# qiskit-community/aqc-research

Hardware: AMD Instinct MI355X
Metric: objective+gradient evals/sec (higher is better)
Workload: dtype f64; 1 GPU; 16-qubit, 40-block cx spin ansatz, state-vector objective+gradient; n_qubits=16, num_thetas=208, gate_groups=56, batch_per_gpu=1024, columns=1, transport=none, records_gathered=1024, launcher=none

## Files before the change

aqc_research_amd/csrc/aqc_api.cpp:

```cpp
#include "aqc_ws.h"

using namespace aqc;

namespace {
thread_local std::string g_error;
}

namespace aqc {

int fail(const char* fmt, ...) {
    char buf[1024];
    va_list ap;
    va_start(ap, fmt);
    vsnprintf(buf, sizeof buf, fmt, ap);
    va_end(ap);
    g_error = buf;
    return 1;
}
int set_error(const std::string& msg) { g_error = msg; return 1; }

int check_buf(const aqc_ws* ws, int buf) {
    if (!ws) return fail("null workspace");
    if (buf < 0 || buf >= AQC_NUM_BUFS) return fail("invalid buffer id %d", buf);
    return 0;
}

int check_block_range(const aqc_ws* ws, int block_from, int block_to) {
    const int nb = ws->ctx->prog.num_blocks;
    if (block_from < 0 || nb == 0) return 0;
    if (!(block_from < block_to && block_to <= nb)) return fail("invalid block_range [%d, %d)", block_from, block_to);
    return 0;
}

int ensure_coef(aqc_ws* ws) {
    if (ws->coef_valid) return 0;
    return fail("thetas have not been uploaded (aqc_ws_set_thetas)");
}

int copy_in(aqc_ws* ws, double2* dst, const double* src, size_t rows) {
    if (ws->pitch == ws->ncols) {
        HIP_OK(hipMemcpyAsync(dst, src, rows * ws->ncols * sizeof(double2), hipMemcpyHostToDevice, ws->stream));
    } else {
        HIP_OK(hipMemsetAsync(dst, 0, rows * ws->pitch * sizeof(double2), ws->stream));
        HIP_OK(hipMemcpy2DAsync(dst, (size_t)ws->pitch * sizeof(double2), src, (size_t)ws->ncols * sizeof(double2),
                                (size_t)ws->ncols * sizeof(double2), rows, hipMemcpyHostToDevice, ws->stream));
    }
    HIP_OK(hipStreamSynchronize(ws->stream));
    return 0;
}
int copy_out(aqc_ws* ws, double* dst, const double2* src, size_t rows) {
    if (ws->pitch == ws->ncols) {
        HIP_OK(hipMemcpyAsync(dst, src, rows * ws->ncols * sizeof(double2), hipMemcpyDeviceToHost, ws->stream));
    } else {
        HIP_OK(hipMemcpy2DAsync(dst, (size_t)ws->ncols * sizeof(double2), src, (size_t)ws->pitch * sizeof(double2),
                                (size_t)ws->ncols * sizeof(double2), rows, hipMemcpyDeviceToHost, ws->stream));
    }
    HIP_OK(hipStreamSynchronize(ws->stream));
    return 0;
}

int results_guard(aqc_ws* ws) {
    if (ws->copy_pending && !ws->capturing) {
        HIP_OK(hipStreamWaitEvent(ws->stream, ws->ev_copied, 0));
        ws->copy_pending = false;
    }
    return 0;
}


}

extern "C" {

const char* aqc_version(void) { return "aqc_hip 0.1.0 (gfx950)"; }
const char* aqc_last_error(void) { return g_error.c_str(); }

int aqc_live_buffers(int64_t* device, int64_t* pinned) {
    if (device) *device = g_live_device.load();
    if (pinned) *pinned = g_live_pinned.load();
    return 0;
}

int aqc_device_count(void) {
    int ndev = 0;
    return hipGetDeviceCount(&ndev) == hipSuccess ? ndev : 0;
}

int aqc_create(int num_qubits, int entangler, const int32_t* blocks, int num_blocks, int trotter, int second_order,
               aqc_ctx** out) {
    if (!out) return fail("out pointer is null");
    *out = nullptr;
    aqc_ctx* ctx = new aqc_ctx();
    const std::string err = build_program(num_qubits, entangler, blocks, num_blocks, trotter != 0, second_order != 0, ctx->prog);
    if (!err.empty()) {
        delete ctx;
        return fail("%s", err.c_str());
    }
    *out = ctx;
    return 0;
}

int aqc_destroy(aqc_ctx* ctx) {
    if (!ctx) return 0;
    for (auto& kv : ctx->oneshot) aqc_ws_destroy(kv.second);
    delete ctx;
    return 0;
}

int aqc_num_thetas(const aqc_ctx* ctx) { return ctx ? ctx->prog.num_thetas() : -1; }
int aqc_num_gate_groups(const aqc_ctx* ctx) { return ctx ? (int)ctx->prog.groups.size() : -1; }

int aqc_plan_query(aqc_ctx* ctx, int ncols, int which, int tile_bits, int low_bits, int stage, int* num_stages,
                   int* bits_out, int* num_bits, int* ops_out, int* num_ops) {
    if (!ctx) return fail("null context");
    if (ncols < 1) return fail("ncols must be positive");
    const int col_bits = ceil_log2(ncols);
    if (tile_bits <= 0) tile_bits = which == 1 ? 12 : 13;
    if (low_bits < 0) low_bits = 3;
    Plan plan = make_plan(ctx->prog, col_bits, tile_bits, low_bits, which == 0);
    if (which == 3) {
        split_substages(ctx->prog, plan, 4, 1 << 20);
        plan = mirror_plan(plan);
    }
    const std::string err = check_plan(ctx->prog, plan);
    if (!err.empty()) return fail("planner produced an invalid plan: %s", err.c_str());
    if (num_stages) *num_stages = (int)plan.stages.size();
    if (stage >= 0) {
        if (stage >= (int)plan.stages.size()) return fail("stage index out of range");
        const Stage& st = plan.stages[stage];
        if (num_bits) *num_bits = (int)st.bits.size();
        if (num_ops) *num_ops = (int)st.ops.size();
        if (bits_out) for (size_t i = 0; i < st.bits.size(); ++i) bits_out[i] = st.bits[i];
        if (ops_out) for (size_t i = 0; i < st.ops.size(); ++i) ops_out[i] = st.ops[i];
    }
    return 0;
}

int aqc_plan_projected(aqc_ctx* ctx, int tile_bits, int low_bits, int32_t* info) {
    if (!ctx || !info) return fail("null argument");
    if (tile_bits <= 0) tile_bits = 12;
    if (low_bits < 0) low_bits = 3;
    const Program& prog = ctx->prog;
    tile_bits = std::min(std::max(tile_bits, 8), std::min(12, prog.n));
    aqc_ws tmp;
    tmp.ctx = ctx;
    tmp.ncols = 1; tmp.col_bits = 0; tmp.nbits = prog.n;
    Plan best = make_plan(prog, 0, tile_bits, low_bits, false);
    for (int lb = low_bits - 1; lb >= 2; --lb) {
        Plan cand = make_plan(prog, 0, tile_bits, lb, false);
        if (cand.stages.size() < best.stages.size()) best = cand;
    }
    lower_plan(prog, best, tmp.sweep, 4, true, true);
    tmp.sparse_enabled = true;
    tmp.inv_mirrored = tmp.sweep.v3 && tmp.sweep.plan.stages.size() >= 2;
    proj_plan(&tmp, low_bits);
    const int rc = aqc_ws_projected_info(&tmp, info);
    tmp.ctx = nullptr;
    return rc;
}

int aqc_plan_substages(aqc_ctx* ctx, int ncols, int which, int tile_bits, int low_bits, int stage, int* num_subs, int* subs_out, int max_subs) {
    if (!ctx || !num_subs) return fail("null argument");
    if (ncols < 1) return fail("ncols must be positive");
    const int col_bits = ceil_log2(ncols);
    if (tile_bits <= 0) tile_bits = 12;
    if (low_bits < 0) low_bits = 3;
    Plan plan = make_plan(ctx->prog, col_bits, tile_bits, low_bits, which == 0);
    split_substages(ctx->prog, plan, 4, 1 << 20);
    if (which == 3) plan = mirror_plan(plan);
    const std::string err = check_plan(ctx->prog, plan);
    if (!err.empty()) return fail("planner produced an invalid plan: %s", err.c_str());
    if (stage < 0 || stage >= (int)plan.stages.size()) return fail("stage index out of range");
    const Stage& st = plan.stages[stage];
    *num_subs = (int)st.subs.size();
    if (subs_out)
        for (int i = 0; i < (int)st.subs.size() && i < max_subs; ++i) {
            for (int j = 0; j < 4; ++j) subs_out[5 * i + j] = j < (int)st.subs[i].bits.size() ? st.subs[i].bits[j] : -1;
            subs_out[5 * i + 4] = (int)st.subs[i].ops.size();
        }
    return 0;
}


static int ws_decide(aqc_ws* ws, int tile_bits_apply, int tile_bits_sweep) {
    aqc_ctx* ctx = ws->ctx;
    const Program& prog = ctx->prog;
    const int batch = ws->batch;
    const int low_bits = env_int("AQC_LOW_BITS", 3);
    int ka = tile_bits_apply > 0 ? tile_bits_apply : env_int("AQC_TILE_BITS_APPLY", 0);
    int ks = tile_bits_sweep > 0 ? tile_bits_sweep : env_int("AQC_TILE_BITS_SWEEP", 0);
    const int family = env_int("AQC_KERNEL_FAMILY", env_int("AQC_KERNEL_V2", -1) >= 0 ? env_int("AQC_KERNEL_V2", -1) + 1 : 0);
    if (family < 0 || family > 3) return fail("AQC_KERNEL_FAMILY must be 1 (per-group), 2 (register-blocked) or 3 (matrix cores)");
    const bool want_v3 = (family == 3 || family == 0) && ws->nbits >= 8;
    const int force_v2 = family == 3 ? 0 : (family ? family - 1 : -1);
    const size_t big_tiles = (size_t)batch << std::max(0, ws->nbits - 12);
    const bool want_v2 = force_v2 >= 0 ? force_v2 != 0 : big_tiles >= 512;
    auto pick = [&](int kmax) {
        if (want_v3) {
            int k = std::min(12, ws->nbits);
            while (k > 10 && ((size_t)batch << (ws->nbits - k)) < 256) --k;
            const int kmin = std::max(8, prog.n + std::min(ws->col_bits, 3));
            while (ws->col_bits > 0 && k > kmin && ((size_t)batch << (ws->nbits - k)) < 256) --k;
            return k;
        }
        if (want_v2) return std::min(kmax, ws->nbits);
        int k = std::min(11, ws->nbits);
        while (k > 10 && ((size_t)batch << (ws->nbits - k)) < 512) --k;
        return k;
    };
    if (ka <= 0) ka = pick(13);
    if (ks <= 0) ks = pick(12);
    ka = std::min(std::min(ka, 13), ws->nbits);
    ks = std::min(std::min(ks, 12), ws->nbits);
    ws->threads = env_int("AQC_THREADS", 0);
    if (ws->threads <= 0) ws->threads = std::min(256, std::max(64, 1 << (std::min(ka, ks) - 2)));
    if (ws->threads < 64 || ws->threads > 512 || ws->threads % 64) return fail("AQC_THREADS must be a multiple of 64 in [64, 512]");

    auto best_plan = [&](int k, bool inverse) {
        Plan best = make_plan(prog, ws->col_bits, k, low_bits, inverse);
        for (int lb = low_bits - 1; lb >= 2; --lb) {
            Plan cand = make_plan(prog, ws->col_bits, k, lb, inverse);
            if (cand.stages.size() < best.stages.size()) best = cand;
        }
        return best;
    };
    if (want_v3) { ka = std::min(std::max(ka, 8), 12); ks = std::max(ks, 8); }
    auto cached = [&](const std::vector<int>& key, DevPlan& out, const std::function<void(HostPlan&)>& lower) {
        std::lock_guard<std::recursive_mutex> lock(ctx->mu);
        auto it = ctx->plan_cache.find(key);
        if (it == ctx->plan_cache.end()) {
            HostPlan fresh;
            lower(fresh);
            it = ctx->plan_cache.emplace(key, std::move(fresh)).first;
        }
        out = it->second;
    };
    auto cached_plan = [&](int which, int k, bool inverse, int reg_bits, bool dots, DevPlan& out) {
        cached({which, ws->col_bits, k, low_bits, reg_bits, (int)dots, (int)want_v3}, out,
               [&](HostPlan& fresh) { lower_plan(prog, best_plan(k, inverse), fresh, reg_bits, dots, want_v3); });
    };
    cached_plan(2, ka, false, (want_v2 || want_v3) ? 4 : 0, false, ws->fwd);
    cached_plan(1, ks, false, want_v3 ? 4 : (want_v2 ? (env_int("AQC_SWEEP_REG_BITS", 4) == 3 ? 3 : 4) : 0), true, ws->sweep);
    ws->inv_mirrored = want_v3 && ka == ks && ws->sweep.v3 && ws->sweep.plan.stages.size() >= 2 && env_int("AQC_MIRROR_PLAN", 1) != 0;
    if (ws->inv_mirrored)
        cached({3, ws->col_bits, ks, low_bits, 4, 0, 1}, ws->inv,
               [&](HostPlan& fresh) { lower_plan(prog, mirror_plan(ws->sweep.plan), fresh, 4, false, true, true); });
    else
        cached_plan(0, ka, true, (want_v2 || want_v3) ? 4 : 0, false, ws->inv);
    ws->sparse_enabled = env_int("AQC_SPARSE_SWEEP", 1) != 0;
    ws->sparse_min_items = env_int("AQC_SPARSE_MIN_ITEMS", 512);
    ws->lazy_z_enabled = env_int("AQC_LAZY_Z", 1) != 0;
    ws->r_only_enabled = env_int("AQC_R_ONLY_LAST", 1) != 0;
    ws->r_only_max_subs = env_int("AQC_R_ONLY_MAX_SUBS", 12);
    ws->proj_vdag_enabled = env_int("AQC_PROJECTED_VDAG", 1) != 0;
    ws->proj_fused_enabled = env_int("AQC_PROJECTED_FUSED", 1) != 0;
    ws->proj_pairs_enabled = env_int("AQC_PROJECTED_PAIRS", 1) != 0;
    ws->proj_vdag_min_elems = (long long)env_int("AQC_PROJECTED_VDAG_MIN_ELEMS", 1 << 24);
    ws->skipw_enabled = env_int("AQC_SKIP_ZERO_W", 0) != 0;
    for (DevPlan* p : {&ws->fwd, &ws->inv, &ws->sweep}) {
        const std::string err = check_plan(prog, p->plan);
        if (!err.empty()) return fail("planner produced an invalid plan: %s", err.c_str());
    }
    proj_plan(ws, low_bits);
    if (env_int("AQC_VERBOSE", 0) && want_v3)
        fprintf(stderr, "aqc_hip: matrix-core kernels, tiles 2^%d (V / V^H, %d workgroups per CU) / 2^%d (sweep, %d per CU), sub-stages %zu / %zu / %zu\n",
                ws->inv.k, mfma_occupancy(ws->inv.k, false), ws->sweep.k, mfma_occupancy(ws->sweep.k, true), ws->fwd.h_subs3.size(),
                ws->inv.h_subs3.size(), ws->sweep.h_subs3.size());
    return 0;
}

struct SlotTables {
    std::vector<int> theta_slots, slot_theta, slot_ntiles;
    int partial_tiles = 1;
};
static SlotTables ws_slot_tables(aqc_ws* ws) {
    const Program& prog = ws->ctx->prog;
    const int T = prog.num_thetas();
    const int G = (int)prog.groups.size();
    ws->nslots = G * kSlotsPerGroup;
    SlotTables t;
    t.partial_tiles = ws->sweep.v3 ? 1 : ws->sweep.ntiles;
    t.theta_slots.assign(2 * (size_t)std::max(T, 1), -1);
    t.slot_ntiles.assign((size_t)std::max(ws->nslots, 1), t.partial_tiles);
    auto feed = [&](int theta, int slot) {
        if (t.theta_slots[2 * theta] < 0) t.theta_slots[2 * theta] = slot; else t.theta_slots[2 * theta + 1] = slot;
    };
    for (int gi = 0; gi < G; ++gi) {
        const GateGroup& g = prog.groups[gi];
        if (g.type == GROUP_FRONT) {
            feed(g.theta0 + 2, gi * kSlotsPerGroup + 0);
            feed(g.theta0 + 1, gi * kSlotsPerGroup + 1);
            feed(g.theta0 + 0, gi * kSlotsPerGroup + 2);
        } else {
            for (int d = 0; d < prog.tpb; ++d) feed(g.theta0 + d, gi * kSlotsPerGroup + d);
        }
    }
    t.slot_theta.assign((size_t)std::max(ws->nslots, 1), -1);
    ws->grads_direct = ws->sweep.v3 && T > 0 && env_int("AQC_GRADS_DIRECT", 1) != 0;
    for (int th = 0; th < T; ++th) {
        if (t.theta_slots[2 * th] < 0 || t.theta_slots[2 * th + 1] >= 0) { ws->grads_direct = false; break; }
        t.slot_theta[t.theta_slots[2 * th]] = th;
    }
    return t;
}

static int ws_upload_ujobs(aqc_ws* ws) {
    const Program& prog = ws->ctx->prog;
    std::vector<UJob> jobs, route_jobs;
    size_t n_vdag_sweep = 0;
    DevPlan* vsw = ws->proj.ok ? &ws->proj.vsw : nullptr;
    const int nsw = ws->sweep.v3 ? (int)ws->sweep.h_subs3.size() : 0;
    ws->ujobs_mirror = ws->inv_mirrored && ws->inv.v3 && (int)ws->inv.h_subs3.size() == nsw && env_int("AQC_UBUILD_MIRROR", 1) != 0;
    for (DevPlan* p : {&ws->inv, &ws->sweep, vsw, &ws->fwd})
        if (p && p->v3)
            for (size_t i = 0; i < p->h_subs3.size(); ++i) {
                if (p == &ws->inv && ws->ujobs_mirror) continue;
                UJob j{p->d_subs3 + i, p->d_grps, p->d_umat, (int)i, (int)p->h_subs3.size(), p->plan.inverse ? 1 : 0, prog.entangler, nullptr, 0, 0};
                if (p == &ws->sweep && ws->ujobs_mirror) { j.umat_mirror = ws->inv.d_umat; j.mirror_index = nsw - 1 - (int)i; j.mirror_nsubs = nsw; }
                if (p == vsw) {
                    const int nvs = (int)vsw->h_subs3.size();
                    j.umat_mirror = ws->proj.vinv.d_umat; j.mirror_index = nvs - 1 - (int)i; j.mirror_nsubs = nvs;
                }
                jobs.push_back(j);
                if (p != &ws->fwd) ++n_vdag_sweep;
                if (vsw && ((p == &ws->inv && (int)i >= p->h_stages.back().sub_begin) || (p == &ws->sweep && (int)i < p->h_stages[0].nsubs) || p == vsw))
                    route_jobs.push_back(j);
            }
    if (vsw && !route_jobs.empty() && route_jobs.size() < n_vdag_sweep && env_int("AQC_UBUILD_SUBSET", 1) != 0) {
        if (ws->d_ujobs_route.upload(route_jobs)) return 1;
        ws->n_ujobs_route = (int)route_jobs.size();
    }
    if (!jobs.empty() && ws->d_ujobs.upload(jobs)) return 1;
    return 0;
}

static int ws_device_side(aqc_ws* ws, const SlotTables& t) {
    const Program& prog = ws->ctx->prog;
    const size_t B = (size_t)ws->batch, T1 = (size_t)std::max(prog.num_thetas(), 1), lanes = B * ws->lane_elems;
    HIP_OK(hipStreamCreateWithFlags(&ws->stream, hipStreamNonBlocking));
    HIP_OK(hipEventCreate(&ws->ev0)); HIP_OK(hipEventCreate(&ws->ev1));
    HIP_OK(hipEventCreate(&ws->pev0)); HIP_OK(hipEventCreate(&ws->pev1));
    if (upload_plan(ws->fwd) || upload_plan(ws->inv) || upload_plan(ws->sweep) || proj_alloc(ws)) return 1;
    if (ws->d_thetas_own.alloc(B * T1)) return 1;
    ws->d_thetas = ws->d_thetas_own;
    if (ws->d_coef.alloc(B * (prog.n + prog.num_blocks + 1) * kCoefStride)) return 1;
    for (auto& buf : ws->bufs) {
        if (buf.alloc(lanes)) return 1;
        HIP_OK(hipMemsetAsync(buf, 0, sizeof(double2) * lanes, ws->stream));
    }
    if (ws->d_partial.alloc(B * std::max(ws->nslots, 1) * t.partial_tiles)) return 1;
    for (DevPlan* p : {&ws->fwd, &ws->inv, &ws->sweep})
        if (p->v3 && p->d_umat.alloc(B * std::max<size_t>(p->h_subs3.size(), 1) * 12 * 64)) return 1;
    if (ws_upload_ujobs(ws)) return 1;
    if (ws->sweep.v3 && ws->sweep.d_rpart.alloc(B * std::max<size_t>(ws->sweep.h_subs3.size(), 1) *
                                                sweep3_nparts(ws->sweep.ntiles, ws->batch, ws->sweep.k) * 256)) return 1;
    if (ws->d_grads.alloc(B * T1)) return 1;
    if (ws->d_theta_slots.upload(t.theta_slots) || ws->d_slot_ntiles.upload(t.slot_ntiles) || ws->d_slot_theta.upload(t.slot_theta)) return 1;
    ws->pin_thetas = B * T1;
    ws->pin_grads = 2 * B * T1;
    ws->pin_small = 2 * B * 64;
    if (ws->h_pin.alloc(ws->pin_thetas + ws->pin_grads + ws->pin_small)) return 1;
    ws->vdot_parts = (int)std::min<size_t>(1024, std::max<size_t>(1, ws->lane_elems / 1024));
    if (ws->d_vdot_part.alloc(B * ws->vdot_parts)) return 1;
    HIP_OK(hipStreamSynchronize(ws->stream));
    return 0;
}

int aqc_ws_create(aqc_ctx* ctx, int device, int batch, int ncols, int tile_bits_apply, int tile_bits_sweep, aqc_ws** out) {
    if (!out) return fail("out pointer is null");
    *out = nullptr;
    if (!ctx) return fail("null context");
    if (batch < 1 || batch > 65535) return fail("batch must be in [1, 65535] (lanes are the y dimension of the launch grid)");
    if (ncols < 1) return fail("ncols must be >= 1");
    const Program& prog = ctx->prog;
    int ndev = 0;
    hipError_t e = hipGetDeviceCount(&ndev);
    if (e != hipSuccess || ndev <= 0)
        return fail("no HIP device available (%s): the aqc_hip path needs an AMD GPU and has no CPU fallback",
                    e == hipSuccess ? "device count is 0" : hipGetErrorString(e));
    if (device < 0 || device >= ndev) return fail("device %d out of range (%d visible)", device, ndev);
    HIP_OK(hipSetDevice(device));
    HIP_OK(init_kernels());
    HIP_OK(init_kernels2());
    HIP_OK(init_kernels3());

    struct Destroy { void operator()(aqc_ws* w) const { aqc_ws_destroy(w); } };
    std::unique_ptr<aqc_ws, Destroy> ws(new aqc_ws());
    ws->ctx = ctx;
    ws->device = device;
    ws->batch = batch;
    ws->ncols = ncols;
    ws->col_bits = ceil_log2(ncols);
    ws->pitch = 1 << ws->col_bits;
    ws->nbits = ws->col_bits + prog.n;
    if (ws->nbits > kMaxBits) return fail("2^%d elements per lane is beyond this build's limit", ws->nbits);
    ws->lane_elems = (size_t)1 << ws->nbits;
    if (ws_decide(ws.get(), tile_bits_apply, tile_bits_sweep)) return 1;
    if (ws_device_side(ws.get(), ws_slot_tables(ws.get()))) return 1;
    *out = ws.release();
    return 0;
}

int aqc_ws_destroy(aqc_ws* ws) {
    if (!ws) return 0;
    (void)hipSetDevice(ws->device);
    for (hipStream_t s : {ws->stream, ws->copy_stream, ws->mps_stream}) if (s) (void)hipStreamSynchronize(s);
    drop_graphs(ws);
    for (hipEvent_t ev : {ws->ev0, ws->ev1, ws->pev0, ws->pev1, ws->ev_ready, ws->ev_copied, ws->ev_mps_fork, ws->ev_mps_join})
        if (ev) (void)hipEventDestroy(ev);
    for (hipStream_t s : {ws->copy_stream, ws->mps_stream, ws->stream}) if (s) (void)hipStreamDestroy(s);
    delete ws;
    return 0;
}

int aqc_ws_set_thetas(aqc_ws* ws, const double* thetas) {
    if (!ws || !thetas) return fail("null argument");
    HIP_OK(hipSetDevice(ws->device));
    const Program& prog = ws->ctx->prog;
    const int T = prog.num_thetas();
    HIP_OK(hipMemcpyAsync(ws->d_thetas_own, thetas, sizeof(double) * (size_t)ws->batch * T, hipMemcpyHostToDevice, ws->stream));
    HIP_OK(hipStreamSynchronize(ws->stream));
    return run_coef(ws, ws->d_thetas_own);
}

int aqc_ws_upload(aqc_ws* ws, int buf, const double* src) {
    if (check_buf(ws, buf) || before_write(ws, buf)) return 1;
    if (!src) return fail("null source");
    HIP_OK(hipSetDevice(ws->device));
    return copy_in(ws, ws->bufs[buf], src, (size_t)ws->batch << ws->ctx->prog.n);
}

int aqc_ws_upload_lane(aqc_ws* ws, int buf, int lane, const double* src) {
    if (check_buf(ws, buf)) return 1;
    if (!src) return fail("null source");
    if (lane < 0 || lane >= ws->batch) return fail("lane out of range");
    HIP_OK(hipSetDevice(ws->device));
    if (before_write(ws, buf, true)) return 1;
    return copy_in(ws, ws->bufs[buf] + (size_t)lane * ws->lane_elems, src, (size_t)1 << ws->ctx->prog.n);
}

int aqc_ws_broadcast(aqc_ws* ws, int buf, const double* src) {
    if (check_buf(ws, buf) || before_write(ws, buf)) return 1;
    if (!src) return fail("null source");
    HIP_OK(hipSetDevice(ws->device));
    if (copy_in(ws, ws->bufs[buf], src, (size_t)1 << ws->ctx->prog.n)) return 1;
    for (int b = 1; b < ws->batch; ++b)
        HIP_OK(hipMemcpyAsync(ws->bufs[buf] + (size_t)b * ws->lane_elems, ws->bufs[buf], ws->lane_elems * sizeof(double2),
                              hipMemcpyDeviceToDevice, ws->stream));
    return 0;
}

int aqc_ws_copy_lane(aqc_ws* dst_ws, int dst_buf, int dst_lane, aqc_ws* src_ws, int src_buf, int src_lane) {
    if (check_buf(dst_ws, dst_buf) || check_buf(src_ws, src_buf)) return 1;
    if (dst_ws->device != src_ws->device) return fail("copy_lane: the two workspaces live on different devices");
    if (dst_ws->lane_elems != src_ws->lane_elems) return fail("copy_lane: lane sizes differ");
    if (dst_lane < 0 || dst_lane >= dst_ws->batch || src_lane < 0 || src_lane >= src_ws->batch) return fail("lane out of range");
    if (before_read(src_ws, src_buf) || before_write(dst_ws, dst_buf, true)) return 1;
    HIP_OK(hipSetDevice(dst_ws->device));
    if (src_ws->stream != dst_ws->stream) HIP_OK(hipStreamSynchronize(src_ws->stream));
    HIP_OK(hipMemcpyAsync(dst_ws->bufs[dst_buf] + (size_t)dst_lane * dst_ws->lane_elems, src_ws->bufs[src_buf] + (size_t)src_lane * src_ws->lane_elems,
                          sizeof(double2) * dst_ws->lane_elems, hipMemcpyDeviceToDevice, dst_ws->stream));
    return 0;
}

int aqc_ws_download(aqc_ws* ws, int buf, double* dst) {
    if (check_buf(ws, buf)) return 1;
    if (!dst) return fail("null destination");
    HIP_OK(hipSetDevice(ws->device));
    if (before_read(ws, buf)) return 1;
    return copy_out(ws, dst, ws->bufs[buf], (size_t)ws->batch << ws->ctx->prog.n);
}

int aqc_ws_download_lane(aqc_ws* ws, int buf, int lane, double* dst) {
    if (check_buf(ws, buf)) return 1;
    if (!dst) return fail("null destination");
    if (lane < 0 || lane >= ws->batch) return fail("lane out of range");
    HIP_OK(hipSetDevice(ws->device));
    if (before_read(ws, buf)) return 1;
    return copy_out(ws, dst, ws->bufs[buf] + (size_t)lane * ws->lane_elems, (size_t)1 << ws->ctx->prog.n);
}

int aqc_ws_set_basis(aqc_ws* ws, int buf, const int64_t* index) {
    if (check_buf(ws, buf) || before_write(ws, buf)) return 1;
    if (!index) return fail("null index");
    HIP_OK(hipSetDevice(ws->device));
    const int64_t dim = (int64_t)1 << ws->ctx->prog.n;
    std::vector<long long> elem(ws->batch);
    for (int b = 0; b < ws->batch; ++b) {
        if (index[b] < 0 || index[b] >= dim) return fail("basis index out of range");
        elem[b] = (long long)index[b] << ws->col_bits;
    }
    if (ws->d_basis_index.reserve(ws->batch)) return 1;
    HIP_OK(hipMemcpyAsync(ws->d_basis_index, elem.data(), sizeof(long long) * ws->batch, hipMemcpyHostToDevice, ws->stream));
    HIP_OK(hipStreamSynchronize(ws->stream));
    HIP_OK(hipMemsetAsync(ws->bufs[buf], 0, sizeof(double2) * (size_t)ws->batch * ws->lane_elems, ws->stream));
    {
        ProfScope ps(ws, AQC_K_MISC);
        HIP_OK(launch_scatter_one(ws->bufs[buf], ws->lane_elems, ws->batch, ws->d_basis_index, ws->stream));
    }
    std::vector<long long> supp(2 * (size_t)ws->batch, -1);
    for (int b = 0; b < ws->batch; ++b) supp[2 * (size_t)b] = elem[b];
    if (ws->d_combo_prev[buf].reserve(2 * (size_t)ws->batch)) return 1;
    HIP_OK(hipMemcpyAsync(ws->d_combo_prev[buf], supp.data(), sizeof(long long) * supp.size(), hipMemcpyHostToDevice, ws->stream));
    HIP_OK(hipStreamSynchronize(ws->stream));
    std::vector<double> coef(4 * (size_t)ws->batch, 0.0);
    for (int b = 0; b < ws->batch; ++b) coef[4 * (size_t)b] = 1.0;
    lhs_support_changed(ws, buf, std::move(supp), std::move(coef));
    return 0;
}

int aqc_ws_set_identity(aqc_ws* ws, int buf) {
    if (check_buf(ws, buf) || before_write(ws, buf)) return 1;
    const int dim = 1 << ws->ctx->prog.n;
    if (ws->ncols != dim) return fail("identity needs a square workspace (ncols == 2^n)");
    HIP_OK(hipSetDevice(ws->device));
    HIP_OK(hipMemsetAsync(ws->bufs[buf], 0, sizeof(double2) * (size_t)ws->batch * ws->lane_elems, ws->stream));
    ProfScope ps(ws, AQC_K_MISC);
    HIP_OK(launch_set_identity(ws->bufs[buf], ws->lane_elems, dim, ws->pitch, ws->batch, ws->stream));
    return 0;
}

int aqc_ws_set_combo(aqc_ws* ws, int buf, const int64_t* index, const double* coef) {
    if (check_buf(ws, buf)) return 1;
    if (!index || !coef) return fail("null argument");
    if (buf == AQC_BUF_W || buf == AQC_BUF_ZW || buf == AQC_BUF_Z) return fail("set_combo targets an lhs buffer (X, X2) or Y");
    HIP_OK(hipSetDevice(ws->device));
    const int64_t dim = (int64_t)1 << ws->ctx->prog.n;
    const int B = ws->batch;
    std::vector<long long> elem(2 * (size_t)B);
    for (int b = 0; b < B; ++b) {
        const int64_t i0 = index[2 * b], i1 = index[2 * b + 1];
        if (i0 < 0 || i0 >= dim || i1 >= dim) return fail("basis index out of range");
        if (i1 == i0) return fail("the two basis states of a lane must differ");
        elem[2 * b] = (long long)i0 << ws->col_bits;
        elem[2 * b + 1] = i1 < 0 ? -1 : (long long)i1 << ws->col_bits;
    }
    std::vector<double> cf(coef, coef + 4 * (size_t)B);
    if (ws->combo_valid[buf] && ws->combo_last_elem[buf] == elem && ws->combo_last_coef[buf] == cf) return 0;
    if (ws->d_combo_index.reserve(2 * (size_t)B) || ws->d_combo_coef.reserve(2 * (size_t)B)) return 1;
    if (ws->d_combo_prev[buf].reserve(2 * (size_t)B)) return 1;
    HIP_OK(hipMemcpyAsync(ws->d_combo_index, elem.data(), sizeof(long long) * 2 * B, hipMemcpyHostToDevice, ws->stream));
    HIP_OK(hipMemcpyAsync(ws->d_combo_coef, coef, sizeof(double2) * 2 * B, hipMemcpyHostToDevice, ws->stream));
    HIP_OK(hipStreamSynchronize(ws->stream));
    if (!ws->combo_valid[buf]) {
        HIP_OK(hipMemsetAsync(ws->bufs[buf], 0, sizeof(double2) * (size_t)B * ws->lane_elems, ws->stream));
        HIP_OK(hipMemsetAsync(ws->d_combo_prev[buf], 0xff, sizeof(long long) * 2 * B, ws->stream));
    }
    ProfScope ps(ws, AQC_K_MISC);
    HIP_OK(launch_scatter_two(ws->bufs[buf], ws->lane_elems, B, ws->d_combo_index, ws->d_combo_coef, ws->d_combo_prev[buf], ws->stream));
    lhs_support_changed(ws, buf, std::move(elem), std::move(cf));
    return 0;
}

int aqc_ws_get_grads(aqc_ws* ws, double* grads) {
    if (!ws || !grads) return fail("null argument");
    HIP_OK(hipSetDevice(ws->device));
    HIP_OK(hipMemcpyAsync(grads, ws->d_grads, sizeof(double2) * (size_t)ws->batch * ws->ctx->prog.num_thetas(),
                          hipMemcpyDeviceToHost, ws->stream));
    HIP_OK(hipStreamSynchronize(ws->stream));
    return 0;
}

int aqc_ws_gather(aqc_ws* ws, int buf, const int64_t* index, int count, double* out) {
    if (check_buf(ws, buf)) return 1;
    if (!index || !out || count < 1) return fail("invalid gather arguments");
    HIP_OK(hipSetDevice(ws->device));
    if (before_read(ws, buf)) return 1;
    const int64_t dim = (int64_t)1 << ws->ctx->prog.n;
    std::vector<long long> elem(count);
    for (int i = 0; i < count; ++i) {
        if (index[i] < 0 || index[i] >= dim) return fail("gather index out of range");
        elem[i] = (long long)index[i] << ws->col_bits;
    }
    HIP_OK(hipStreamSynchronize(ws->stream));
    if (ws->d_tmp_index.reserve(count) || ws->d_tmp_small.reserve((size_t)ws->batch * count)) return 1;
    HIP_OK(hipMemcpyAsync(ws->d_tmp_index, elem.data(), sizeof(long long) * count, hipMemcpyHostToDevice, ws->stream));
    HIP_OK(hipStreamSynchronize(ws->stream));
    {
        ProfScope ps(ws, AQC_K_MISC);
        HIP_OK(launch_gather(ws->bufs[buf], ws->lane_elems, ws->d_tmp_index, count, ws->batch, ws->d_tmp_small, ws->stream));
    }
    HIP_OK(hipMemcpyAsync(out, ws->d_tmp_small, sizeof(double2) * (size_t)ws->batch * count, hipMemcpyDeviceToHost, ws->stream));
    HIP_OK(hipStreamSynchronize(ws->stream));
    return 0;
}

int aqc_ws_vdot(aqc_ws* ws, int buf_a, int buf_b, double* out) {
    if (check_buf(ws, buf_a) || check_buf(ws, buf_b)) return 1;
    if (!out) return fail("null output");
    HIP_OK(hipSetDevice(ws->device));
    if (before_read(ws, buf_a) || before_read(ws, buf_b)) return 1;
    HIP_OK(hipStreamSynchronize(ws->stream));
    if (ws->d_tmp_small.reserve(ws->batch)) return 1;
    {
        ProfScope ps(ws, AQC_K_MISC);
        HIP_OK(launch_vdot(ws->bufs[buf_a], ws->bufs[buf_b], ws->lane_elems, ws->lane_elems, ws->batch, ws->d_vdot_part,
                           ws->vdot_parts, ws->d_tmp_small, ws->stream));
    }
    HIP_OK(hipMemcpyAsync(out, ws->d_tmp_small, sizeof(double2) * (size_t)ws->batch, hipMemcpyDeviceToHost, ws->stream));
    HIP_OK(hipStreamSynchronize(ws->stream));
    return 0;
}

int aqc_ws_theta_bank(aqc_ws* ws, const double* thetas, int nsets) {
    if (!ws || !thetas || nsets < 1) return fail("invalid theta bank arguments");
    HIP_OK(hipSetDevice(ws->device));
    const size_t count = (size_t)nsets * ws->batch * std::max(ws->ctx->prog.num_thetas(), 1), bytes = sizeof(double) * count;
    HIP_OK(hipStreamSynchronize(ws->stream));
    if (ws->d_theta_bank.release()) return 1;
    ws->bank_sets = 0;
    ws->d_thetas = ws->d_thetas_own;
    if (ws->d_theta_bank.alloc(count)) return 1;
    HIP_OK(hipMemcpyAsync(ws->d_theta_bank, thetas, bytes, hipMemcpyHostToDevice, ws->stream));
    HIP_OK(hipStreamSynchronize(ws->stream));
    ws->bank_sets = nsets;
    return 0;
}

int aqc_ws_use_theta_set(aqc_ws* ws, int set_index) {
    if (!ws) return fail("null workspace");
    if (set_index < 0 || set_index >= ws->bank_sets) return fail("theta set %d out of range (%d loaded)", set_index, ws->bank_sets);
    HIP_OK(hipSetDevice(ws->device));
    return run_coef(ws, ws->d_theta_bank + (size_t)set_index * ws->batch * ws->ctx->prog.num_thetas());
}

int aqc_ws_gather_setup(aqc_ws* ws, const int64_t* index, int count) {
    if (!ws || !index || count < 1) return fail("invalid gather arguments");
    HIP_OK(hipSetDevice(ws->device));
    const int64_t dim = (int64_t)1 << ws->ctx->prog.n;
    std::vector<long long> elem(count);
    for (int i = 0; i < count; ++i) {
        if (index[i] < 0 || index[i] >= dim) return fail("gather index out of range");
        elem[i] = (long long)index[i] << ws->col_bits;
    }
    HIP_OK(hipStreamSynchronize(ws->stream));
    drop_graphs(ws);
    if (ws->d_index.reserve(count) || ws->d_small.reserve((size_t)ws->batch * count)) return 1;
    if (2 * (size_t)ws->batch * count > ws->pin_small) {
        const size_t want = 2 * (size_t)ws->batch * count;
        PinBuf<double> pin;
        if (pin.alloc(ws->pin_thetas + ws->pin_grads + want)) return 1;
        ws->h_pin = std::move(pin);
        ws->pin_small = want;
    }
    HIP_OK(hipMemcpyAsync(ws->d_index, elem.data(), sizeof(long long) * count, hipMemcpyHostToDevice, ws->stream));
    HIP_OK(hipStreamSynchronize(ws->stream));
    ws->gather_count = count;
    ws->h_gather = elem;
    ++ws->gather_gen;
    return 0;
}

int aqc_ws_gather_launch(aqc_ws* ws, int buf) {
    if (check_buf(ws, buf)) return 1;
    if (ws->gather_count < 1) return fail("aqc_ws_gather_setup has not been called");
// ... 265 lines not shown
```

aqc_research_amd/csrc/aqc_kernels3.hip:

```cpp
#include <hip/hip_runtime.h>

#include <cstring>

#include <type_traits>

#include "aqc_device.h"
#include "aqc_launch.h"
#include "aqc_math.h"

namespace aqc {

typedef double double4_t __attribute__((ext_vector_type(4)));

__host__ __device__ __forceinline__ unsigned swz3(unsigned l) { return l ^ ((l >> 4) & 15u) ^ ((l >> 8) & 15u); }

__device__ __forceinline__ double4_t mfma(double a, double b, double4_t c) {
    return __builtin_amdgcn_mfma_f64_16x16x4f64(a, b, c, 0, 0, 0);
}

struct Acc3 { double4_t k1, k2, k3; };
__device__ __forceinline__ void u_mfma(const cplx (&v)[4], const double (&u0)[4], const double (&u1)[4], const double (&u2)[4], Acc3& t) {
    t.k1 = double4_t{0.0, 0.0, 0.0, 0.0}; t.k2 = t.k1; t.k3 = t.k1;
#pragma unroll
    for (int s = 0; s < 4; ++s) {
        t.k1 = mfma(v[s].x + v[s].y, u0[s], t.k1);
        t.k2 = mfma(v[s].x, u1[s], t.k2);
        t.k3 = mfma(v[s].y, u2[s], t.k3);
    }
}
__device__ __forceinline__ void u_combine(const Acc3& t, cplx (&o)[4]) {
#pragma unroll
    for (int r = 0; r < 4; ++r) {
        o[r].x = t.k1[r] - t.k3[r];
        o[r].y = t.k1[r] + t.k2[r];
    }
}

#ifdef AQC_TUNING
#define AQC_STAMP(slot) do { if (a.stamps && threadIdx.x == 0 && (slot) < kStampSlots) \
    a.stamps[((size_t)blockIdx.y * gridDim.x + blockIdx.x) * kStampSlots + (slot)] = __builtin_amdgcn_s_memtime(); } while (0)
#ifdef AQC_TUNING_NODBG
#define AQC_DBG_AND(x)
#define AQC_DBG_TEST(x) false
#else
#define AQC_DBG_AND(x) && (x)
#define AQC_DBG_TEST(x) (x)
#endif
#else
#define AQC_STAMP(slot) do { } while (0)
#define AQC_DBG_AND(x)
#define AQC_DBG_TEST(x) false
#endif

__host__ __device__ constexpr bool sweep_scratch_double(int k) { return k >= 12 || k <= 9; }
#ifndef AQC_SWEEP_SPREAD
#define AQC_SWEEP_SPREAD 1
#endif
#ifndef AQC_APPLY_SPREAD
#define AQC_APPLY_SPREAD 1
#endif
#ifndef AQC_EXP_APPLY_SKIP
#define AQC_EXP_APPLY_SKIP 0
#endif
constexpr int kApplySkip = AQC_EXP_APPLY_SKIP;
#ifndef AQC_EXP_SWEEP_SKIP
#define AQC_EXP_SWEEP_SKIP 0
#endif
constexpr int kSweepSkip = AQC_EXP_SWEEP_SKIP;
#ifndef AQC_EXP_UBUILD_SKIP
#define AQC_EXP_UBUILD_SKIP 0
#endif
constexpr int kUbuildSkip = AQC_EXP_UBUILD_SKIP;

constexpr int kSweepSpread = AQC_SWEEP_SPREAD, kApplySpread = AQC_APPLY_SPREAD;
template <int K, bool SWEEP = false> struct TileShape {
    static constexpr int kSweepWaves12 = 4;
    static constexpr int kWaves = (SWEEP && K == 12) ? kSweepWaves12 : (K >= 10 ? 4 : (1 << (K - 8)));
    static constexpr int kGroups = 1 << (K - 8);
    static constexpr int kGpw = kGroups / kWaves;
    static constexpr int kLoads = (1 << (K - 6)) / kWaves;
};

struct SubRegs {
    double u0[4], u1[4], u2[4];
    unsigned lane12;
};

template <int GPW>
__device__ __forceinline__ void fetch_sub(SubRegs& x, const DevSub3* subs, const double* umat, int sub_index, int lane, int wave,
                                          int nwaves) {
    const DevSub3* sub = subs + sub_index;
    const double* up = umat + (size_t)sub_index * 12 * 64;
#pragma unroll
    for (int s = 0; s < 4; ++s) {
        x.u0[s] = up[(0 * 4 + s) * 64 + lane];
        x.u1[s] = up[(1 * 4 + s) * 64 + lane];
        x.u2[s] = up[(2 * 4 + s) * 64 + lane];
    }
    x.lane12 = sub->lane12[lane];
}

template <int GPW>
struct SubAddr {
    unsigned a1, a2;
    unsigned k1[GPW][4], k2[GPW][4];
};
typedef unsigned uint8v_t __attribute__((ext_vector_type(8)));
template <int GPW>
__device__ __forceinline__ void fetch_k(SubAddr<GPW>& x, const DevSub3* subs, int sub_index, int wave, int nwaves) {
#pragma unroll
    for (int j = 0; j < GPW; ++j) {
        const uint8v_t kv = *reinterpret_cast<const __attribute__((address_space(4))) uint8v_t*>(
            (const __attribute__((address_space(4))) void*)(const void*)&subs[sub_index].kk[wave + j * nwaves][0]);
#pragma unroll
        for (int s = 0; s < 4; ++s) { x.k1[j][s] = kv[s]; x.k2[j][s] = kv[4 + s]; }
    }
}
template <int GPW>
__device__ __forceinline__ void sub_addr(SubAddr<GPW>& x, const SubRegs& c, unsigned lds_base) {
    x.a1 = ((c.lane12 & 0xffffu) << 4) + lds_base;
    x.a2 = ((c.lane12 >> 16) << 4) + lds_base;
}
typedef double dbl2_t __attribute__((ext_vector_type(2)));
typedef __attribute__((address_space(3))) dbl2_t* lds_cplx_ptr;
__device__ __forceinline__ cplx lds_get(unsigned addr) {
    const dbl2_t v = *reinterpret_cast<lds_cplx_ptr>(addr);
    return make_double2(v.x, v.y);
}
__device__ __forceinline__ void lds_put(unsigned addr, cplx v) { *reinterpret_cast<lds_cplx_ptr>(addr) = dbl2_t{v.x, v.y}; }
__device__ __forceinline__ unsigned lds_address(const void* p) {
    return (unsigned)reinterpret_cast<size_t>((__attribute__((address_space(3))) const char*)p);
}

__device__ __forceinline__ const void* uniform_ptr(const void* p) {
    const unsigned long long v = (unsigned long long)p;
    const unsigned lo = __builtin_amdgcn_readfirstlane((unsigned)v), hi = __builtin_amdgcn_readfirstlane((unsigned)(v >> 32));
    return (const void*)(((unsigned long long)hi << 32) | lo);
}

template <int K, int NV>
__device__ __forceinline__ void load_tiles3(cplx* t0, cplx* t1, const cplx* s0, const cplx* s1, const DevStage& st, unsigned lo, int wave) {
    constexpr int NL = TileShape<K, NV == 2>::kLoads, NW = TileShape<K, NV == 2>::kWaves;
    cplx v0[NL], v1[NL];
#pragma unroll
    for (int i = 0; i < NL; ++i) {
        const unsigned off = lo + st.dhi[wave + i * NW];
        v0[i] = s0[off];
        if (NV == 2) v1[i] = s1[off];
    }
#pragma unroll
    for (int i = 0; i < NL; ++i) {
        const unsigned slot = swz3((unsigned)((wave + i * NW) << 6) | (threadIdx.x & 63u));
        t0[slot] = v0[i];
        if (NV == 2) t1[slot] = v1[i];
    }
}
template <int K, bool SWEEP>
__device__ __forceinline__ void store_tile3(const cplx* tile, cplx* dst, const DevStage& st, unsigned lo, int wave) {
    constexpr int NL = TileShape<K, SWEEP>::kLoads, NW = TileShape<K, SWEEP>::kWaves;
#pragma unroll
    for (int i = 0; i < NL; ++i) {
        const unsigned slot = swz3((unsigned)((wave + i * NW) << 6) | (threadIdx.x & 63u));
        dst[lo + st.dhi[wave + i * NW]] = tile[slot];
    }
}
__device__ __forceinline__ size_t tile_base3(const DevStage& st, unsigned tile) {
    size_t base = 0;
    for (int i0 = 0; i0 < st.nub; i0 += 4) {
        int ub[4];
#pragma unroll
        for (int u = 0; u < 4; ++u) ub[u] = st.ubits[i0 + u];
#pragma unroll
        for (int u = 0; u < 4; ++u)
            if (i0 + u < st.nub) base |= (size_t)((tile >> (i0 + u)) & 1u) << ub[u];
    }
    return base;
}

__device__ __forceinline__ int uniform_load(const int* p) { return __builtin_amdgcn_readfirstlane(*p); }
struct ItemAt { int bl, tile, slot; };
template <bool LIST>
__device__ __forceinline__ ItemAt item_at(const Stage3Args& a, int wi) {
    if (LIST) {
        const TileItem* it = a.items + wi;
        return ItemAt{uniform_load(&it->lane), uniform_load(&it->tile), uniform_load(&it->slot)};
    }
    const int bl = wi / a.ntiles;
    return ItemAt{bl, wi - bl * a.ntiles, 0};
}
template <int K, bool LIST, bool PAIR = false>
__device__ __forceinline__ void apply_mfma_body(const Stage3Args& a0, const Stage3Args& b0, const int wg, const int nwg) {
    using TS = TileShape<K>;
    static_assert(!PAIR || (LIST && K >= 12), "the pair form walks two lists with persistent workgroups");
    extern __shared__ __attribute__((aligned(16))) char smem[];
    const Stage3Args* ca = &a0;
#define a (*ca)
#define st (ca->stage)
    cplx* tw = reinterpret_cast<cplx*>(smem);
    const unsigned lds_base = lds_address(smem);
    if (lds_base & ((16u << K) - 1)) __builtin_trap();
    const int lane = threadIdx.x & 63;
    const int wave = __builtin_amdgcn_readfirstlane((int)(threadIdx.x >> 6));
    constexpr int NL = TS::kLoads, NW = TS::kWaves;
    constexpr bool kPersist = K >= 12;
    int nwork = LIST ? uniform_load(a.nitems) : a.ntiles * a.batch;
    bool second = false;
    if (PAIR && wg >= nwork) { ca = &b0; second = true; nwork = uniform_load(b0.nitems); }
    unsigned lo = st.dlo[lane];
    unsigned lo16 = lo << 4;
    (void)lo16;
    SubRegs cur, nxt;
    SubAddr<TS::kGpw> ad;
    dbl2_t pw[NL];
    int wi = wg + ((kPersist || LIST) ? 0 : (int)blockIdx.y * a.ntiles);
    if (LIST && wi >= nwork) return;
    ItemAt it = item_at<LIST>(a, wi);
    {
        const int bl = it.bl;
        if (st.nsubs > 0) {
            fetch_sub<TS::kGpw>(cur, a.subs, a.umat + (size_t)bl * a.nsubs_total * 12 * 64, st.sub_begin, lane, wave, NW);
            fetch_k<TS::kGpw>(ad, a.subs, st.sub_begin, wave, NW);
        }
        AQC_STAMP(0);
        if (!(kApplySkip & 64)) load_tiles3<K, 1>(tw, nullptr, a.in0 + (size_t)bl * a.lane_stride + tile_base3(st, it.tile), nullptr, st, lo, wave);
    }
    __builtin_amdgcn_s_waitcnt(0x0F70);
    AQC_STAMP(1);
    for (;;) {
    const int bl = it.bl;
    const size_t lane_off = (size_t)bl * a.lane_stride + tile_base3(st, it.tile);
    const double* umat = a.umat + (size_t)bl * a.nsubs_total * 12 * 64;
    int nwi = wi + nwg;
    bool more = kPersist && st.nsubs > 0 && nwi < nwork;
    const Stage3Args* na = ca;
    int nnwork = nwork;
    if (PAIR && !more && !second) {
        na = &b0; nwi = wg; nnwork = uniform_load(b0.nitems);
        more = nwi < nnwork;
    }
    const bool change = PAIR && na != ca;
    const ItemAt nit = more ? item_at<LIST>(*na, nwi) : ItemAt{0, 0, 0};
    const int nbl = nit.bl;
    const size_t next_off = more ? (size_t)nbl * na->lane_stride + tile_base3(na->stage, nit.tile) : 0;
    const unsigned nlo = change ? na->stage.dlo[lane] : lo;
    const unsigned nlo16 = nlo << 4;
    for (int si = 0; si < st.nsubs; ++si) {
        AQC_STAMP(4 + si);
        if (!(kApplySkip & 512)) __syncthreads();
        if (si + 1 < st.nsubs) fetch_sub<TS::kGpw>(nxt, a.subs, umat, st.sub_begin + si + 1, lane, wave, NW);
        else if (more) fetch_sub<TS::kGpw>(nxt, na->subs, na->umat + (size_t)nbl * na->nsubs_total * 12 * 64, na->stage.sub_begin, lane, wave, NW);
        if (kPersist && more && !(kApplySkip & 64)) {
#pragma unroll
            for (int c = 0; c < 4; ++c) {
                if (si == (c < st.nsubs ? c : st.nsubs - 1)) {
#pragma unroll
                    for (int i = c * (NL / 4); i < (c + 1) * (NL / 4); ++i) {
                        const size_t ub = next_off + na->stage.dhi[wave + i * NW];
                        asm volatile("s_nop 4\n\tglobal_load_dwordx4 %0, %1, %2" : "=a"(pw[i]) : "v"(nlo16), "s"(uniform_ptr(na->in0 + ub)) : "memory");
                    }
                }
            }
        }
        sub_addr(ad, cur, lds_base);
        cplx v[2][4];
        Acc3 acc;
#pragma unroll
        for (int s = 0; s < 4; ++s) v[0][s] = lds_get(ad.a1 ^ ad.k1[0][s]);
#pragma unroll
        for (int j = 0; j <= TS::kGpw; ++j) {
            if (j + 1 < TS::kGpw && !(kApplySkip & 2)) {
#pragma unroll
                for (int s = 0; s < 4; ++s) v[(j + 1) & 1][s] = lds_get((kApplySkip & 32) ? ad.a1 : (ad.a1 ^ ad.k1[j + 1][s]));
            }
            __builtin_amdgcn_sched_barrier(0);
            double sv[4];
            cplx o[4];
            if (j < TS::kGpw) {
#pragma unroll
                for (int s = 0; s < 4; ++s) sv[s] = (kApplySkip & (16 | 128)) ? v[j & 1][s].x : v[j & 1][s].x + v[j & 1][s].y;
            }
            if (j > 0) {
                if (kApplySkip & (16 | 256)) {
#pragma unroll
                    for (int r = 0; r < 4; ++r) o[r] = make_double2(acc.k1[r], acc.k2[r]);
                } else u_combine(acc, o);
            }
            unsigned wa[4];
            if (j < TS::kGpw) {
#pragma unroll
                for (int s = 0; s < 4; ++s) asm volatile("" : "+v"(sv[s]));
            }
            if (j > 0) {
#pragma unroll
                for (int r = 0; r < 4; ++r) { wa[r] = (kApplySkip & 32) ? ad.a2 : (ad.a2 ^ ad.k2[j - 1][r]); asm volatile("" : "+v"(wa[r])); }
            }
            __builtin_amdgcn_sched_barrier(0);
            if (j < TS::kGpw) {
                acc.k1 = double4_t{0.0, 0.0, 0.0, 0.0}; acc.k2 = acc.k1; acc.k3 = acc.k1;
#pragma unroll
                for (int s = 0; s < 4; ++s) {
                    if (kApplySkip & 8) continue;
                    acc.k1 = mfma(sv[s], cur.u0[s], acc.k1);
                    acc.k2 = mfma(v[j & 1][s].x, cur.u1[s], acc.k2);
                    acc.k3 = mfma(v[j & 1][s].y, cur.u2[s], acc.k3);
                }
            }
            if (j > 0 && !(kApplySkip & 1)) {
#pragma unroll
                for (int r = 0; r < 4; ++r) lds_put(wa[r], o[r]);
                if (j < TS::kGpw) {
#pragma unroll
                    for (int i = 0; i < 4; ++i) {
                        __builtin_amdgcn_sched_group_barrier(0x008, kApplySpread, 0);
                        __builtin_amdgcn_sched_group_barrier(0x200, 1, 0);
                    }
                }
            }
            __builtin_amdgcn_sched_barrier(0);
        }
        if (si + 1 < st.nsubs || more) {
            cur = nxt;
            if (si + 1 < st.nsubs) fetch_k<TS::kGpw>(ad, a.subs, st.sub_begin + si + 1, wave, NW);
            else fetch_k<TS::kGpw>(ad, na->subs, na->stage.sub_begin, wave, NW);
        }
    }
    AQC_STAMP(4 + st.nsubs);
    __syncthreads();
    AQC_STAMP(2);
    if (!(kApplySkip & 64)) store_tile3<K, false>(tw, a.out0 + lane_off, st, lo, wave);
    AQC_STAMP(3);
    if (!more) break;
    __syncthreads();
    __builtin_amdgcn_s_waitcnt(0x0F70);
#pragma unroll
    for (int i = 0; i < NL; ++i) {
        const unsigned slot = swz3((unsigned)((wave + i * NW) << 6) | (threadIdx.x & 63u));
        asm volatile("ds_write_b128 %0, %1" : : "v"(lds_base + (slot << 4)), "a"(pw[i]) : "memory");
    }
    __builtin_amdgcn_s_waitcnt(0xC07F);
    wi = nwi;
    it = nit;
    if (PAIR) { ca = na; second = second || change; nwork = nnwork; lo = nlo; lo16 = nlo16; }
    }
#undef a
#undef st
}
template <int K, bool LIST = false>
__global__ __launch_bounds__(TileShape<K>::kWaves * 64, 2) void apply_mfma_kernel(const Stage3Args a) {
    apply_mfma_body<K, LIST>(a, a, (int)blockIdx.x, (int)gridDim.x);
}
#ifndef AQC_PAIR_PLAIN_BOUNDARY
#define AQC_PAIR_PLAIN_BOUNDARY 0
#endif
template <int K>
__global__ __launch_bounds__(TileShape<K>::kWaves * 64, 2) void apply_pair_kernel(const Stage3Args a, const Stage3Args b, const int grid_a) {
    if constexpr (K >= 12 && !AQC_PAIR_PLAIN_BOUNDARY) {
        static_assert(sizeof(Stage3Args) % 8 == 0 && alignof(Stage3Args) == 8, "b follows a in the kernel-argument segment without padding");
        const __attribute__((address_space(4))) char* kp = (const __attribute__((address_space(4))) char*)__builtin_amdgcn_kernarg_segment_ptr();
        const Stage3Args* pa = (const Stage3Args*)(const void*)kp;
        const Stage3Args* pb = (const Stage3Args*)(const void*)(kp + sizeof(Stage3Args));
        apply_mfma_body<K, true, true>(*pa, *pb, (int)blockIdx.x, (int)gridDim.x);
    } else if (K >= 12) {
        apply_mfma_body<K, true>(a, a, (int)blockIdx.x, (int)gridDim.x);
        __syncthreads();
        apply_mfma_body<K, true>(b, b, (int)blockIdx.x, (int)gridDim.x);
    } else if ((int)blockIdx.x < grid_a) {
        apply_mfma_body<K, true>(a, a, (int)blockIdx.x, grid_a);
    } else {
        apply_mfma_body<K, true>(b, b, (int)blockIdx.x - grid_a, (int)gridDim.x - grid_a);
    }
}

template <int N>
__device__ __forceinline__ void wait_prefetched(dbl2_t (&pw)[N], dbl2_t (&pz)[N]) {
    asm volatile("s_waitcnt vmcnt(0)" : : : "memory");
#pragma unroll
    for (int i = 0; i < N; ++i) asm volatile("" : "+a"(pw[i]), "+a"(pz[i]));
}
__device__ __forceinline__ unsigned tile_offset3(const DevStage& st, unsigned local) { return st.dlo[local & 63u] | st.dhi[local >> 6]; }
template <int K> struct SweepShape : TileShape<K, true> {};
__device__ __forceinline__ unsigned elem_bit(const DevStage& st, long long e, unsigned local_pos) {
    const unsigned m = local_pos < 6 ? st.dlo[1u << local_pos] : st.dhi[1u << (local_pos - 6)];
    return ((unsigned long long)e & m) ? 1u : 0u;
}
template <int GPW, int NW>
__device__ __forceinline__ void skip_masks(const DevStage& st, unsigned info, long long e0, long long e1, int wave, unsigned& nzmask, unsigned& kneed) {
    nzmask = 0; kneed = 0;
    const unsigned gfresh = info & 15u, kfresh = (info >> 6) & 3u;
#pragma unroll
    for (int k = 0; k < 2; ++k) {
        const long long e = k ? e1 : e0;
        if (e < 0) continue;
        unsigned gb = 0;
#pragma unroll
        for (int i = 0; i < 4; ++i)
            if (gfresh >> i & 1) gb |= elem_bit(st, e, (info >> (8 + 4 * i)) & 15u) << i;
        unsigned kb = 0;
        if (kfresh & 1) kb |= elem_bit(st, e, (info >> 24) & 15u);
        if (kfresh & 2) kb |= elem_bit(st, e, (info >> 28) & 15u) << 1;
#pragma unroll
        for (int j = 0; j < GPW; ++j)
            if ((((unsigned)(wave + j * NW) ^ gb) & gfresh) == 0) nzmask |= 1u << j;
#pragma unroll
        for (unsigned s2 = 0; s2 < 4; ++s2)
            if (((s2 ^ kb) & kfresh) == 0) kneed |= 1u << s2;
    }
}
template <int K, bool LIST, bool SKIPW, bool RLAST>
__device__ __forceinline__ void sweep_mfma_body(const Stage3Args& a, const int wg, const int nwg) {
    using TS = TileShape<K, true>;
    constexpr int kSlots = TS::kWaves > 4 ? 4 : TS::kWaves;
    constexpr unsigned tsize = 1u << K;
    extern __shared__ __attribute__((aligned(16))) char smem[];
    const DevStage& st = a.stage;
    cplx* tw = reinterpret_cast<cplx*>(smem);
    cplx* tz = tw + tsize;
    cplx* scratch = tz + tsize;
    constexpr bool kDouble = sweep_scratch_double(K);
    const unsigned lds_base = lds_address(smem);
    if (lds_base & ((32u << K) - 1)) __builtin_trap();
    const int lane = threadIdx.x & 63;
    const int wave = __builtin_amdgcn_readfirstlane((int)(threadIdx.x >> 6));
    constexpr bool kPersist = K >= 12;
    constexpr int NL = TS::kLoads, NW = TS::kWaves;
    const int nwork = LIST ? uniform_load(a.nitems) : a.ntiles * a.batch;
    const unsigned lo = st.dlo[lane];
    SubRegs cur, nxt;
    SubAddr<TS::kGpw> ad;
    dbl2_t pw[NL], pz[NL];
    unsigned parity = 0;
    AQC_STAMP(0);
    const int chunk = kPersist ? (LIST ? (nwork + nwg - 1) / nwg : a.chunk) : 0;
    const int wi_first = kPersist ? wg * chunk : wg;
    const int wi_end = kPersist ? (wi_first + chunk < nwork ? wi_first + chunk : nwork) : wi_first + 1;
    int wi = wi_first;
    if (wi >= nwork) return;
    const unsigned e16 = threadIdx.x << 4;
    dbl2_t racc;
    static_assert(!kPersist || NL == 4 * TS::kGpw, "the prefetch registers are the first sub-stage's operands");
    const bool reg_first = kPersist && st.nsubs > 0;
    unsigned flo16 = 0;
    ItemAt it = item_at<LIST>(a, wi);
    size_t item_off = (size_t)it.bl * a.lane_stride + tile_base3(st, it.tile);
    {
        const size_t off0 = item_off;
        if (st.nsubs > 0) {
            fetch_sub<TS::kGpw>(cur, a.subs, a.umat + (size_t)it.bl * a.nsubs_total * 12 * 64, st.sub_begin, lane, wave, NW);
            fetch_k<TS::kGpw>(ad, a.subs, st.sub_begin, wave, NW);
        }
        if (reg_first) {
            flo16 = tile_offset3(st, swz3(cur.lane12 & 0xffffu)) << 4;
#pragma unroll
            for (int i = 0; i < ((kSweepSkip & 64) ? 0 : NL); ++i) {
                const size_t ub = off0 + a.first_hi[wave + (i / 4) * NW][i % 4];
                asm volatile("s_nop 4\n\tglobal_load_dwordx4 %0, %1, %2" : "=a"(pw[i]) : "v"(flo16), "s"(uniform_ptr(a.in0 + ub)) : "memory");
                asm volatile("s_nop 4\n\tglobal_load_dwordx4 %0, %1, %2" : "=a"(pz[i]) : "v"(flo16), "s"(uniform_ptr(a.in1 + ub)) : "memory");
            }
        } else {
            load_tiles3<K, 2>(tw, tz, a.in0 + off0, a.in1 + off0, st, lo, wave);
        }
    }
    __builtin_amdgcn_s_waitcnt(0x0F70);
    if (reg_first) wait_prefetched<NL>(pw, pz);
    __syncthreads();
    AQC_STAMP(1);
    for (;;) {
    const int bl = it.bl, tile = it.tile;
    const size_t lane_off = item_off;
    long long se0 = -1, se1 = -1;
    if (SKIPW) {
        const unsigned long long toff = (unsigned long long)tile_base3(st, tile);
        const long long c0 = a.supp[2 * (size_t)bl], c1 = a.supp[2 * (size_t)bl + 1];
        const unsigned lo0 = __builtin_amdgcn_readfirstlane((unsigned)c0), hi0 = __builtin_amdgcn_readfirstlane((unsigned)(c0 >> 32));
        const unsigned lo1 = __builtin_amdgcn_readfirstlane((unsigned)c1), hi1 = __builtin_amdgcn_readfirstlane((unsigned)(c1 >> 32));
        const long long u0 = (long long)(((unsigned long long)hi0 << 32) | lo0), u1 = (long long)(((unsigned long long)hi1 << 32) | lo1);
        if (u0 >= 0 && (((unsigned long long)u0 ^ toff) & st.fresh_nonlocal) == 0) se0 = u0;
        if (u1 >= 0 && (((unsigned long long)u1 ^ toff) & st.fresh_nonlocal) == 0) se1 = u1;
    }
    const double* umat = a.umat + (size_t)bl * a.nsubs_total * 12 * 64;
    const int part = LIST ? it.slot : (kPersist ? wg - (bl * a.ntiles) / chunk : tile);
    const bool seg_first = LIST || !kPersist || wi == wi_first || tile == 0;
    cplx* rpart = a.rpart + (((size_t)bl * a.nsubs_total + st.sub_begin) * a.nparts + part) * 256;
    const int nwi = wi + 1;
    const bool more = reg_first && nwi < wi_end;
    const ItemAt nit = more ? item_at<LIST>(a, nwi) : ItemAt{0, 0, 0};
    const int nbl = nit.bl;
    const size_t next_off = more ? (size_t)nbl * a.lane_stride + tile_base3(st, nit.tile) : 0;
    constexpr unsigned ZOFF = tsize * 16;
    cplx vw[2][4], vz[2][4];
    constexpr bool kEarly = K >= 11;
    if (reg_first) {
        sub_addr(ad, cur, lds_base);
#pragma unroll
        for (int s = 0; s < 4; ++s) { vw[0][s] = make_double2(pw[s].x, pw[s].y); vz[0][s] = make_double2(pz[s].x, pz[s].y); }
    } else if (kEarly && st.nsubs > 0) {
        sub_addr(ad, cur, lds_base);
#pragma unroll
        for (int s = 0; s < 4; ++s) { vw[0][s] = lds_get(ad.a1 ^ ad.k1[0][s]); vz[0][s] = lds_get((ad.a1 | ZOFF) ^ ad.k1[0][s]); }
    }
    auto prefetch = [&](int c) __attribute__((always_inline)) {
#pragma unroll
        for (int i = 0; i < ((kSweepSkip & 64) ? 0 : NL); ++i)
            if (i / (NL / 4) == c) {
                const size_t ub = next_off + a.first_hi[wave + (i / 4) * NW][i % 4];
                asm volatile("s_nop 4\n\tglobal_load_dwordx4 %0, %1, %2" : "=a"(pw[i]) : "v"(flo16), "s"(uniform_ptr(a.in0 + ub)) : "memory");
                asm volatile("s_nop 4\n\tglobal_load_dwordx4 %0, %1, %2" : "=a"(pz[i]) : "v"(flo16), "s"(uniform_ptr(a.in1 + ub)) : "memory");
            }
    };
    const int nmain = RLAST && a.r_only_last && st.nsubs >= 1 && !(kPersist && st.nsubs == 1) ? st.nsubs - 1 : st.nsubs;
    if (!RLAST) {
        for (int si = 0; si < st.nsubs; ++si) {
#define AQC_SS_FROM_REGS (reg_first && si == 0)
#define AQC_SS_RONLY false
#include "aqc_sweep_substage.inc"
#undef AQC_SS_FROM_REGS
#undef AQC_SS_RONLY
        }
    } else {
        if (nmain > 0) {
            const int si = 0;
#define AQC_SS_FROM_REGS reg_first
#define AQC_SS_RONLY false
#include "aqc_sweep_substage.inc"
#undef AQC_SS_FROM_REGS
#undef AQC_SS_RONLY
        }
        for (int si = 1; si < nmain; ++si) {
#define AQC_SS_FROM_REGS false
#define AQC_SS_RONLY false
#include "aqc_sweep_substage.inc"
#undef AQC_SS_FROM_REGS
#undef AQC_SS_RONLY
        }
        if (nmain < st.nsubs) {
            const int si = nmain;
#define AQC_SS_FROM_REGS false
#define AQC_SS_RONLY true
#include "aqc_sweep_substage.inc"
#undef AQC_SS_FROM_REGS
#undef AQC_SS_RONLY
        }
    }
    AQC_STAMP(kStampSlots - 2);
    if (more) wait_prefetched<NL>(pw, pz);
    if (!(kSweepSkip & 64)) {
        if (a.store_out & 1) store_tile3<K, true>(tw, a.out0 + lane_off, st, lo, wave);
        if (a.store_out & 2) store_tile3<K, true>(tz, a.out1 + lane_off, st, lo, wave);
    }
    AQC_STAMP(kStampSlots - 1);
    if (!more) break;
    AQC_STAMP(kStampSlots - 6);
    __syncthreads();
    AQC_STAMP(kStampSlots - 5);
    wi = nwi;
    it = nit;
    item_off = next_off;
    }
    AQC_STAMP(kStampSlots - 4);
}
template <int K, bool LIST = false, bool SKIPW = false, bool RLAST = false>
__global__ __launch_bounds__(SweepShape<K>::kWaves * 64, K >= 12 ? 1 : 2) void sweep_mfma_kernel(const Stage3Args a) {
    sweep_mfma_body<K, LIST, SKIPW, RLAST>(a, (int)blockIdx.x, (int)gridDim.x);
}
template <int K, bool RLAST_A, bool RLAST_B>
__global__ __launch_bounds__(SweepShape<K>::kWaves * 64, K >= 12 ? 1 : 2) void sweep_pair_kernel(const Stage3Args a, const Stage3Args b, const int grid_a) {
    if (K >= 12) {
        sweep_mfma_body<K, true, false, RLAST_A>(a, (int)blockIdx.x, (int)gridDim.x);
        __syncthreads();
        sweep_mfma_body<K, true, false, RLAST_B>(b, (int)blockIdx.x, (int)gridDim.x);
    } else if ((int)blockIdx.x < grid_a) {
        sweep_mfma_body<K, true, false, RLAST_A>(a, (int)blockIdx.x, grid_a);
    } else {
        sweep_mfma_body<K, true, false, RLAST_B>(b, (int)blockIdx.x - grid_a, (int)gridDim.x - grid_a);
    }
}

constexpr int kGrpChunk = 16;
struct Gm {
    cplx c[4], t[4];
    double ec, es;
    double rc[4], rs[4];
    int type, pc, pt, flags, slot0, jblock, o0, o1;
};
__device__ __forceinline__ void m2_mul(const cplx (&a)[4], const cplx (&b)[4], cplx (&o)[4]) {
#pragma unroll
    for (int i = 0; i < 2; ++i)
#pragma unroll
        for (int j = 0; j < 2; ++j) {
            const cplx x = a[2 * i], y = b[j], u = a[2 * i + 1], v = b[2 + j];
            o[2 * i + j] = make_double2(x.x * y.x - x.y * y.y + u.x * v.x - u.y * v.y, x.x * y.y + x.y * y.x + u.x * v.y + u.y * v.x);
        }
}
__device__ __forceinline__ void m2_ry(double c, double s, cplx (&o)[4]) {
    o[0] = make_double2(c, 0.0); o[1] = make_double2(-s, 0.0); o[2] = make_double2(s, 0.0); o[3] = make_double2(c, 0.0);
}
__device__ __forceinline__ void m2_rz(double c, double s, cplx (&o)[4]) {
    o[0] = make_double2(c, -s); o[1] = make_double2(0.0, 0.0); o[2] = make_double2(0.0, 0.0); o[3] = make_double2(c, s);
}
__device__ __forceinline__ void m2_rx(double c, double s, cplx (&o)[4]) {
    o[0] = make_double2(c, 0.0); o[1] = make_double2(0.0, -s); o[2] = make_double2(0.0, -s); o[3] = make_double2(c, 0.0);
}
template <bool DAG, bool TR>
__device__ __forceinline__ void m2_apply(const cplx (&m)[4], cplx& a0, cplx& a1) {
    const cplx m00 = m[0], m01 = (DAG || TR) ? m[2] : m[1], m10 = (DAG || TR) ? m[1] : m[2], m11 = m[3];
    const double sg = DAG ? -1.0 : 1.0;
    const cplx x = a0, y = a1;
    a0 = make_double2(m00.x * x.x - sg * m00.y * x.y + m01.x * y.x - sg * m01.y * y.y, m00.x * x.y + sg * m00.y * x.x + m01.x * y.y + sg * m01.y * y.x);
    a1 = make_double2(m10.x * x.x - sg * m10.y * x.y + m11.x * y.x - sg * m11.y * y.y, m10.x * x.y + sg * m10.y * x.x + m11.x * y.y + sg * m11.y * y.x);
}
__device__ __forceinline__ void stage_groups(Gm* gm, const DevGrp* grps, int begin, int count, const double* th, int ent, int lane) {
    {
        const int gi = lane >> 2, k = lane & 3;
        if (gi < count) {
            const DevGrp d = grps[begin + gi];
            double c = 1.0, s = 0.0;
            if (k < (d.type == 0 ? 3 : 4)) sincos(0.5 * th[d.theta0 + k], &s, &c);
            gm[gi].rc[k] = c; gm[gi].rs[k] = s;
            if (k == 0) {
                double ec = 1.0, es = 0.0;
                if (ent == 2 && d.type != 0) sincos(th[d.theta0 + 4], &es, &ec);
                gm[gi].ec = ec; gm[gi].es = es;
            }
        }
    }
    __builtin_amdgcn_fence(__ATOMIC_SEQ_CST, "wavefront");
    __builtin_amdgcn_wave_barrier();
    if (lane >= count) return;
    const DevGrp d = grps[begin + lane];
    Gm g;
    g.type = d.type; g.pc = d.pc; g.pt = d.pt; g.flags = d.flags; g.slot0 = d.slot0; g.jblock = d.jblock;
    const int mask = 0xF & ~(1 << d.pc) & ~(1 << d.pt);
    g.o0 = __ffs(mask) - 1; g.o1 = __ffs(mask & (mask - 1)) - 1;
    g.ec = gm[lane].ec; g.es = gm[lane].es;
#pragma unroll
    for (int k = 0; k < 4; ++k) { g.rc[k] = gm[lane].rc[k]; g.rs[k] = gm[lane].rs[k]; }
    cplx a[4], b[4], m[4];
    if (d.type == 0) {
        m2_rz(g.rc[0], g.rs[0], a); m2_ry(g.rc[1], g.rs[1], b); m2_mul(a, b, m);
        m2_rz(g.rc[2], g.rs[2], b); m2_mul(m, b, g.c);
        g.t[0] = make_double2(1.0, 0.0); g.t[1] = make_double2(0.0, 0.0); g.t[2] = g.t[1]; g.t[3] = g.t[0];
    } else {
        m2_rz(g.rc[1], g.rs[1], a); m2_ry(g.rc[0], g.rs[0], b); m2_mul(a, b, g.c);
        if (d.flags & 1) { m2_rz(kR, -kR, b); m2_mul(g.c, b, m); g.c[0] = m[0]; g.c[1] = m[1]; g.c[2] = m[2]; g.c[3] = m[3]; }
        if (ent == 0) m2_rx(g.rc[3], g.rs[3], a); else m2_rz(g.rc[3], g.rs[3], a);
        m2_ry(g.rc[2], g.rs[2], b); m2_mul(a, b, g.t);
        if (d.flags & 2) { m2_rz(kR, kR, a); m2_mul(a, g.t, m); g.t[0] = m[0]; g.t[1] = m[1]; g.t[2] = m[2]; g.t[3] = m[3]; }
    }
    gm[lane] = g;
}
__device__ __forceinline__ int grp_index(const Gm& g, int l, int rest) {
    return ((l >> 1) << g.pc) | ((l & 1) << g.pt) | ((rest & 1) << g.o0) | ((rest >> 1) << g.o1);
}
template <int MODE>
__device__ __forceinline__ void grp_apply(const Gm& g, int ent, cplx (&x)[4]) {
    auto entangle = [&](double es) {
        if (g.type == 0) return;
        if (ent == 0) { const cplx t = x[2]; x[2] = x[3]; x[3] = t; }
        else if (ent == 1) x[3] = make_double2(-x[3].x, -x[3].y);
        else x[3] = cmul(x[3], g.ec, es);
    };
    if (MODE == 0) {
        entangle(g.es);
        m2_apply<false, false>(g.t, x[0], x[1]); m2_apply<false, false>(g.t, x[2], x[3]);
        m2_apply<false, false>(g.c, x[0], x[2]); m2_apply<false, false>(g.c, x[1], x[3]);
    } else {
        m2_apply<MODE == 1, MODE == 2>(g.c, x[0], x[2]); m2_apply<MODE == 1, MODE == 2>(g.c, x[1], x[3]);
        m2_apply<MODE == 1, MODE == 2>(g.t, x[0], x[1]); m2_apply<MODE == 1, MODE == 2>(g.t, x[2], x[3]);
        entangle(MODE == 1 ? -g.es : g.es);
    }
}

__global__ __launch_bounds__(64) void ubuild_kernel(const UJob* jobs, const double* thetas, int T, double* thetas_copy) {
    __shared__ cplx u[256];
    __shared__ Gm gm[kGrpChunk];
    const int lane = threadIdx.x, b = blockIdx.y;
    const UJob job = jobs[blockIdx.x];
    const DevSub3 sub = *job.sub;
    const double* th = thetas + (size_t)b * T;
    if (thetas_copy && blockIdx.x == 0)
        for (int i = lane; i < T; i += 64) thetas_copy[(size_t)b * T + i] = th[i];
#pragma unroll
    for (int m = 0; m < 4; ++m) {
        const int e = lane + 64 * m;
        u[e] = make_double2((e >> 4) == (e & 15) ? 1.0 : 0.0, 0.0);
    }
    const int col = lane & 15, rest = lane >> 4;
    for (int base = 0; base < sub.ngrp; base += kGrpChunk) {
        const int count = min(kGrpChunk, sub.ngrp - base);
        __syncthreads();
        stage_groups(gm, job.grps, sub.grp_begin + base, count, th, job.entangler, lane);
        __syncthreads();
        for (int i = 0; i < count; ++i) {
            const Gm& g = gm[i];
            cplx x[4];
            int idx[4];
#pragma unroll
            for (int l = 0; l < 4; ++l) { idx[l] = grp_index(g, l, rest) * 16 + col; x[l] = u[idx[l]]; }
            if (job.inverse) grp_apply<1>(g, job.entangler, x); else grp_apply<0>(g, job.entangler, x);
#pragma unroll
            for (int l = 0; l < 4; ++l) u[idx[l]] = x[l];
            __syncthreads();
        }
    }
    __syncthreads();
    double* out = job.umat + ((size_t)b * job.nsubs + job.index) * 12 * 64;
    if (kUbuildSkip) {
        double acc = 0.0;
        for (int m = 0; m < 4; ++m) acc += u[lane + 64 * m].x * u[lane + 64 * m].y;
        if (acc == 1.0e300) out[lane] = acc;
    }
    if (kUbuildSkip & 1) return;
#pragma unroll
    for (int s = 0; s < 4; ++s) {
        const cplx v = u[(lane & 15) * 16 + 4 * s + (lane >> 4)];
        out[(0 * 4 + s) * 64 + lane] = v.x;
        out[(1 * 4 + s) * 64 + lane] = v.y - v.x;
        out[(2 * 4 + s) * 64 + lane] = v.x + v.y;
    }
    if (job.umat_mirror && !(kUbuildSkip & 2)) {
        double* om = job.umat_mirror + ((size_t)b * job.mirror_nsubs + job.mirror_index) * 12 * 64;
#pragma unroll
        for (int s = 0; s < 4; ++s) {
            const cplx t = u[(4 * s + (lane >> 4)) * 16 + (lane & 15)];
            const double re = t.x, im = -t.y;
            om[(0 * 4 + s) * 64 + lane] = re;
            om[(1 * 4 + s) * 64 + lane] = im - re;
            om[(2 * 4 + s) * 64 + lane] = re + im;
        }
    }
}

template <int LB>
__device__ __forceinline__ void rho_unapply(cplx (&rho)[16], int kind, double c, double s) {
    constexpr int st = LB == 0 ? 1 : 2, other = LB == 0 ? 2 : 1;
#pragma unroll
    for (int q = 0; q < 2; ++q)
#pragma unroll
        for (int b = 0; b < 4; ++b) {
            const int a0 = q * other;
            if (kind == MOP_RY) ry2(rho[a0 * 4 + b], rho[(a0 + st) * 4 + b], c, -s);
            else if (kind == MOP_RZ) rz2(rho[a0 * 4 + b], rho[(a0 + st) * 4 + b], c, -s);
            else rx2(rho[a0 * 4 + b], rho[(a0 + st) * 4 + b], c, -s);
        }
#pragma unroll
    for (int q = 0; q < 2; ++q)
#pragma unroll
        for (int a = 0; a < 4; ++a) {
            const int b0 = q * other;
            if (kind == MOP_RY) ry2(rho[a * 4 + b0], rho[a * 4 + b0 + st], c, -s);
            else if (kind == MOP_RZ) rz2(rho[a * 4 + b0], rho[a * 4 + b0 + st], c, s);
            else rx2(rho[a * 4 + b0], rho[a * 4 + b0 + st], c, s);
        }
}
template <int LB>
__device__ __forceinline__ cplx rho_dot(const cplx (&rho)[16], int kind) {
    constexpr int st = LB == 0 ? 1 : 2, other = LB == 0 ? 2 : 1;
    double re = 0.0, im = 0.0;
#pragma unroll
    for (int q = 0; q < 2; ++q) {
        const int i0 = q * other, i1 = i0 + st;
        if (kind == MOP_RY) { re += rho[i1 * 4 + i0].x - rho[i0 * 4 + i1].x; im += rho[i1 * 4 + i0].y - rho[i0 * 4 + i1].y; }
        else if (kind == MOP_RZ) { re += rho[i0 * 4 + i0].x - rho[i1 * 4 + i1].x; im += rho[i0 * 4 + i0].y - rho[i1 * 4 + i1].y; }
        else { re += rho[i0 * 4 + i1].x + rho[i1 * 4 + i0].x; im += rho[i0 * 4 + i1].y + rho[i1 * 4 + i0].y; }
    }
    return kind == MOP_RY ? make_double2(0.5 * re, 0.5 * im) : make_double2(-0.5 * im, 0.5 * re);
}

#ifdef AQC_TUNING
__device__ unsigned long long g_rgrad_stamps[32 * 8];
#define RG_STAMP(slot) do { if (blockIdx.y == 0 && blockIdx.x < 32 && threadIdx.x == 0) g_rgrad_stamps[blockIdx.x * 8 + (slot)] = __builtin_amdgcn_s_memtime(); } while (0)
#else
#define RG_STAMP(slot) do { } while (0)
#endif
template <int WAVES>
__global__ __launch_bounds__(64 * WAVES) void rgrad_kernel(const DevSub3* subs, const DevGrp* grps, int ent, const double* thetas, int T,
                                                           const cplx* rpart, int ntiles, int nsubs_total, cplx* partial, int nslots,
                                                           int from, int to, int front, const int* slot_theta, cplx* grads, cplx* mirror,
                                                           const GatherJob gj, int tiles_per_lane, int chunk, int sparse_subs,
                                                           const int* lane_parts, int conj_sub, const double* umat, int nsubs_run,
                                                           const RgradSecond second) {
    if ((int)blockIdx.x == nsubs_run + second.count) {
        const cplx* src = static_cast<const cplx*>(gj.buf) + (size_t)blockIdx.y * gj.lane_stride;
        for (int i = threadIdx.x; i < gj.count; i += 64 * WAVES) {
            const cplx v = src[(size_t)gj.elem[i]];
            static_cast<cplx*>(gj.out)[(size_t)blockIdx.y * gj.count + i] = v;
            if (gj.mirror) static_cast<cplx*>(gj.mirror)[(size_t)blockIdx.y * gj.count + i] = v;
        }
        return;
    }
    __shared__ cplx R[16 * 17];
    __shared__ Gm gm[kGrpChunk];
    __shared__ cplx rho_s[kGrpChunk][16];
    __shared__ cplx psum[WAVES > 1 ? WAVES - 1 : 1][WAVES > 1 ? 256 : 1];
    const int lane = threadIdx.x & 63, wave = threadIdx.x >> 6, b = blockIdx.y;
    int si = blockIdx.x;
    if (si >= nsubs_run) {
        si -= nsubs_run;
        subs = second.subs; grps = second.grps; rpart = second.rpart; ntiles = second.nparts; nsubs_total = second.nsubs_total;
        tiles_per_lane = second.nparts; chunk = 0; sparse_subs = second.nsubs_total; lane_parts = second.lane_parts; conj_sub = -1; umat = second.umat;
    }
    RG_STAMP(0);
    const DevSub3 sub = subs[si];
    const double* th = thetas + (size_t)b * T;
    const int nparts_stride = ntiles;
    if (chunk > 0) ntiles = ((b + 1) * tiles_per_lane - 1) / chunk - (b * tiles_per_lane) / chunk + 1;
    if (si < sparse_subs) ntiles = lane_parts[b];
    const cplx* rp = rpart + ((size_t)b * nsubs_total + si) * nparts_stride * 256;
    {
        cplx acc[4] = {make_double2(0.0, 0.0), make_double2(0.0, 0.0), make_double2(0.0, 0.0), make_double2(0.0, 0.0)};
        constexpr int TB = 8;
        for (int t0 = wave; t0 < ntiles; t0 += TB * WAVES) {
            cplx v[TB][4];
#pragma unroll
            for (int u = 0; u < TB; ++u)
#pragma unroll
                for (int r = 0; r < 4; ++r)
                    v[u][r] = t0 + u * WAVES < ntiles ? rp[(size_t)(t0 + u * WAVES) * 256 + 64 * r + lane] : make_double2(0.0, 0.0);
            if (WAVES > 1 && t0 == wave && wave == 0 && sub.ngrp > 0)
                stage_groups(gm, grps, sub.grp_begin + max(0, sub.ngrp - kGrpChunk), min(sub.ngrp, kGrpChunk), th, ent, lane);
#pragma unroll
            for (int u = 0; u < TB; ++u)
#pragma unroll
                for (int r = 0; r < 4; ++r) { acc[r].x += v[u][r].x; acc[r].y += v[u][r].y; }
        }
        if (WAVES > 1) {
            if (wave > 0) {
#pragma unroll
                for (int r = 0; r < 4; ++r) psum[wave - 1][64 * r + lane] = acc[r];
            }
            __syncthreads();
            if (wave > 0) return;
#pragma unroll
            for (int w = 0; w < WAVES - 1; ++w)
#pragma unroll
                for (int r = 0; r < 4; ++r) { const cplx p = psum[w][64 * r + lane]; acc[r].x += p.x; acc[r].y += p.y; }
        }
#pragma unroll
        for (int r = 0; r < 4; ++r)
            R[(4 * r + (lane >> 4)) * 17 + (lane & 15)] = acc[r];
    }
    if (si == conj_sub) {
        cplx* const Us = &rho_s[0][0];
        const double* up = umat + ((size_t)b * nsubs_total + si) * 12 * 64;
        __syncthreads();
#pragma unroll
        for (int s2 = 0; s2 < 4; ++s2) {
            const double re = up[(0 * 4 + s2) * 64 + lane], im = up[(1 * 4 + s2) * 64 + lane] + re;
            Us[(lane & 15) * 16 + 4 * s2 + (lane >> 4)] = make_double2(re, im);
        }
        __syncthreads();
        const int i0 = lane & 15, j0 = lane >> 4;
        cplx acc[4];
#pragma unroll
        for (int m = 0; m < 4; ++m) {
            const int j = j0 + 4 * m;
            double re = 0.0, im = 0.0;
            for (int k = 0; k < 16; ++k) {
                const cplx u = Us[j * 16 + k], r = R[k * 17 + i0];
                re += u.x * r.x - u.y * r.y; im += u.x * r.y + u.y * r.x;
            }
            acc[m] = make_double2(re, im);
        }
        __syncthreads();
#pragma unroll
        for (int m = 0; m < 4; ++m) R[(j0 + 4 * m) * 17 + i0] = acc[m];
        __syncthreads();
#pragma unroll
        for (int m = 0; m < 4; ++m) {
            const int j = j0 + 4 * m;
            double re = 0.0, im = 0.0;
            for (int k = 0; k < 16; ++k) {
                const cplx t = R[j * 17 + k], u = Us[i0 * 16 + k];
                re += t.x * u.x + t.y * u.y; im += t.y * u.x - t.x * u.y;
            }
            acc[m] = make_double2(re, im);
        }
        __syncthreads();
#pragma unroll
        for (int m = 0; m < 4; ++m) R[(j0 + 4 * m) * 17 + i0] = acc[m];
        __syncthreads();
    }
    RG_STAMP(1);
    cplx* out = partial + (size_t)b * nslots;
    auto put = [&](int slot, cplx v) {
        out[slot] = v;
        if (slot_theta) {
            const int t = slot_theta[slot];
            if (t >= 0) {
                grads[(size_t)b * T + t] = v;
                if (mirror) mirror[(size_t)b * T + t] = v;
            }
        }
    };
    const int lo = lane & 15, hi = lane >> 4;
    for (int top = sub.ngrp; top > 0; top -= kGrpChunk) {
        const int base = max(0, top - kGrpChunk), count = top - base;
        __syncthreads();
        if (WAVES == 1 || top != sub.ngrp) stage_groups(gm, grps, sub.grp_begin + base, count, th, ent, lane);
        __syncthreads();
        RG_STAMP(2);
        for (int i = count - 1; i >= 0; --i) {
            const Gm& g = gm[i];
            {
                const int a = lane >> 4, bb = (lane >> 2) & 3, o = lane & 3;
                cplx v = R[grp_index(g, a, o) * 17 + grp_index(g, bb, o)];
                v.x += dpp_mov<0xB1, 0xf>(v.x); v.y += dpp_mov<0xB1, 0xf>(v.y);
                v.x += dpp_mov<0x4E, 0xf>(v.x); v.y += dpp_mov<0x4E, 0xf>(v.y);
                if (o == 0) rho_s[i][a * 4 + bb] = v;
            }
            cplx x[4];
            int idx[4];
#pragma unroll
            for (int l = 0; l < 4; ++l) { idx[l] = grp_index(g, l, hi) * 17 + lo; x[l] = R[idx[l]]; }
            grp_apply<1>(g, ent, x);
#pragma unroll
            for (int l = 0; l < 4; ++l) R[idx[l]] = x[l];
            __syncthreads();
#pragma unroll
            for (int l = 0; l < 4; ++l) { idx[l] = lo * 17 + grp_index(g, l, hi); x[l] = R[idx[l]]; }
            grp_apply<2>(g, ent, x);
#pragma unroll
            for (int l = 0; l < 4; ++l) R[idx[l]] = x[l];
            __syncthreads();
        }
        RG_STAMP(3);
        if (lane < count) {
            const Gm& g = gm[lane];
            const bool on = g.jblock < 0 ? (front != 0) : (g.jblock >= from && g.jblock < to);
            if (on && g.slot0 >= 0) {
                cplx rho[16];
#pragma unroll
                for (int e = 0; e < 16; ++e) rho[e] = rho_s[lane][e];
                if (g.type == 0) {
                    put(g.slot0 + 2, rho_dot<1>(rho, MOP_RZ));
                    rho_unapply<1>(rho, MOP_RZ, g.rc[0], g.rs[0]);
                    put(g.slot0 + 1, rho_dot<1>(rho, MOP_RY));
                    rho_unapply<1>(rho, MOP_RY, g.rc[1], g.rs[1]);
                    put(g.slot0 + 0, rho_dot<1>(rho, MOP_RZ));
                } else {
                    const int ks = ent == 0 ? MOP_RX : MOP_RZ;
                    if (g.flags & 2) rho_unapply<0>(rho, MOP_RZ, kR, kR);
                    put(g.slot0 + 3, rho_dot<0>(rho, ks));
                    rho_unapply<0>(rho, ks, g.rc[3], g.rs[3]);
                    put(g.slot0 + 2, rho_dot<0>(rho, MOP_RY));
                    put(g.slot0 + 1, rho_dot<1>(rho, MOP_RZ));
                    rho_unapply<1>(rho, MOP_RZ, g.rc[1], g.rs[1]);
                    put(g.slot0 + 0, rho_dot<1>(rho, MOP_RY));
                    if (ent == 2) {
                        rho_unapply<0>(rho, MOP_RY, g.rc[2], g.rs[2]);
                        rho_unapply<1>(rho, MOP_RY, g.rc[0], g.rs[0]);
                        put(g.slot0 + 4, make_double2(rho[15].y, -rho[15].x));
                    }
                }
            } else if (slot_theta && g.slot0 >= 0) {
                for (int k = 0; k < 5; ++k) put(g.slot0 + k, make_double2(0.0, 0.0));
            }
        }
        RG_STAMP(4);
    }
}
#ifdef AQC_TUNING
void rgrad_print_stamps(int nsubs) {
    unsigned long long h[32 * 8];
    if (hipMemcpyFromSymbol(h, HIP_SYMBOL(g_rgrad_stamps), sizeof h) != hipSuccess) return;
    double a = 0, b = 0, c = 0, d = 0;
    const int n = nsubs < 32 ? nsubs : 32;
    for (int i = 0; i < n; ++i) { a += h[i * 8 + 1] - h[i * 8]; b += h[i * 8 + 2] - h[i * 8 + 1]; c += h[i * 8 + 3] - h[i * 8 + 2]; d += h[i * 8 + 4] - h[i * 8 + 3]; }
    fprintf(stderr, "aqc_hip stamps: gradient walk (lane 0, %d sub-stages): tile sum %.0f + group decode %.0f + R walk %.0f + rho walk %.0f cycles\n", n, a / n, b / n, c / n, d / n);
}
#endif

void stage3_first_offsets(Stage3Args& a, const DevSub3& first_sub) {
    for (int g = 0; g < 16; ++g)
        for (int s = 0; s < 4; ++s) {
            const unsigned local = swz3(first_sub.kk[g][s] >> 4);
            a.first_hi[g][s] = a.stage.dlo[local & 63u] | a.stage.dhi[local >> 6];
        }
}

int mfma_threads(int k, bool sweep) { return (sweep && k == 12) ? 64 * SweepShape<12>::kWaves : 64 * std::min(4, 1 << std::max(0, k - 8)); }
size_t apply3_lds_bytes(int k) { return (size_t)16 << k; }
size_t sweep3_lds_bytes(int k) {
    return ((size_t)32 << k) + (size_t)(sweep_scratch_double(k) ? 2 : 1) * std::min(4, mfma_threads(k, true) / 64) * 256 * sizeof(cplx);
}

template <typename F>
static hipError_t with_tile_size(int k, F&& f) {
    switch (k) {
        case 8: return f(std::integral_constant<int, 8>{});
        case 9: return f(std::integral_constant<int, 9>{});
        case 10: return f(std::integral_constant<int, 10>{});
        case 11: return f(std::integral_constant<int, 11>{});
        case 12: return f(std::integral_constant<int, 12>{});
        default: return hipErrorInvalidValue;
    }
}
using Stage3Kernel = void (*)(Stage3Args);
using Pair3Kernel = void (*)(Stage3Args, Stage3Args, int);
template <int K> static Stage3Kernel apply_variant(bool list) { return list ? apply_mfma_kernel<K, true> : apply_mfma_kernel<K, false>; }
template <int K> static Stage3Kernel sweep_variant(bool list, bool skipw, bool rlast) {
    if (list) return rlast ? sweep_mfma_kernel<K, true, false, true> : sweep_mfma_kernel<K, true, false, false>;
    if (skipw) return sweep_mfma_kernel<K, false, true, false>;
    return rlast ? sweep_mfma_kernel<K, false, false, true> : sweep_mfma_kernel<K, false, false, false>;
}
template <int K> static Pair3Kernel apply_pair_variant() { return apply_pair_kernel<K>; }
template <int K> static Pair3Kernel sweep_pair_variant(bool rlast_a) { return rlast_a ? sweep_pair_kernel<K, true, false> : sweep_pair_kernel<K, false, false>; }

template <typename F>
static hipError_t big_lds(F kernel) {
    return hipFuncSetAttribute(reinterpret_cast<const void*>(kernel), hipFuncAttributeMaxDynamicSharedMemorySize, 160 * 1024);
}
hipError_t init_kernels3() {
    hipError_t e = hipSuccess;
    for (int k = 8; k <= 12 && e == hipSuccess; ++k)
        e = with_tile_size(k, [](auto kk) {
            constexpr int K = decltype(kk)::value;
            hipError_t e = big_lds(apply_pair_variant<K>());
            for (int f = 0; f < 2 && e == hipSuccess; ++f) e = big_lds(apply_variant<K>(f));
            for (int f = 0; f < 2 && e == hipSuccess; ++f) e = big_lds(sweep_pair_variant<K>(f));
            for (int f = 0; f < 8 && e == hipSuccess; ++f) e = big_lds(sweep_variant<K>(f & 1, f & 2, f & 4));
            return e;
        });
    return e;
}
template <typename... Args>
static hipError_t launch3(void (*kernel)(Args...), dim3 grid, int k, bool sweep, hipStream_t s, const Args&... args) {
    kernel<<<grid, mfma_threads(k, sweep), sweep ? sweep3_lds_bytes(k) : apply3_lds_bytes(k), s>>>(args...);
    return hipGetLastError();
}
int mfma_occupancy(int k, bool sweep) {
    int n = 0;
    const hipError_t e = with_tile_size(k, [&](auto kk) {
        constexpr int K = decltype(kk)::value;
        return sweep ? hipOccupancyMaxActiveBlocksPerMultiprocessor(&n, sweep_variant<K>(false, false, false), mfma_threads(k, true), sweep3_lds_bytes(k))
                     : hipOccupancyMaxActiveBlocksPerMultiprocessor(&n, apply_variant<K>(false), mfma_threads(k, false), apply3_lds_bytes(k));
    });
    return e == hipSuccess ? n : -1;
}
static long persistent_sweep_grid() {
    static int cus[64] = {0};
    int dev = 0;
    if (hipGetDevice(&dev) != hipSuccess || dev < 0 || dev >= 64) return 256;
    if (cus[dev] == 0) {
        int n = 0;
        cus[dev] = (hipDeviceGetAttribute(&n, hipDeviceAttributeMultiprocessorCount, dev) == hipSuccess && n > 0) ? n : 256;
    }
    if (const char* e = getenv("AQC_SWEEP_GRID")) { const long v = atol(e); if (v > 0) return v; }
    return cus[dev];
}
static long apply_persist() {
    static const long persist = []() { const char* e = getenv("AQC_APPLY_PERSIST"); return e ? atol(e) : 2L; }();
    return persist;
}
static bool stage3_launchable(int k, const Stage3Args& a, bool need_list, bool need_subs) {
    if (a.items ? (!a.nitems || a.max_items < 1) : need_list) return false;
    if (k < 12) return true;
    if (need_subs && a.stage.nsubs <= 0) return false;
    for (int l = 0; l < 64; ++l)
        if (a.stage.dlo[l] >= (1u << 28)) return false;
    return true;
}
hipError_t launch_apply3(int k, hipStream_t s, const Stage3Args& a) {
    const bool list = a.items != nullptr;
    const long persist = apply_persist();
    if (!stage3_launchable(k, a, false, list) || (list && k >= 12 && persist <= 0)) return hipErrorInvalidValue;
    const long nwork = list ? (long)a.max_items : (long)a.ntiles * a.batch;
    const dim3 grid = (k >= 12 && persist > 0 && a.stage.nsubs > 0) ? dim3((unsigned)std::min<long>(nwork, persist * persistent_sweep_grid()))
                                                                     : ((k >= 12 || list) ? dim3((unsigned)nwork) : dim3(a.ntiles, a.batch));
    return with_tile_size(k, [&](auto kk) { return launch3(apply_variant<decltype(kk)::value>(list), grid, k, false, s, a); });
}
static_assert(2 * sizeof(Stage3Args) + 16 <= 3840, "two argument blocks must fit the kernel-argument segment");
hipError_t launch_apply3_pair(int k, hipStream_t s, const Stage3Args& a, const Stage3Args& b) {
    const long persist = apply_persist();
    if (!stage3_launchable(k, a, true, true) || !stage3_launchable(k, b, true, true) || (k >= 12 && persist <= 0)) return hipErrorInvalidValue;
    const long longer = std::max(a.max_items, b.max_items);
    const dim3 grid((unsigned)(k >= 12 ? std::min<long>(longer, persist * persistent_sweep_grid()) : (long)a.max_items + b.max_items));
    return with_tile_size(k, [&](auto kk) { return launch3(apply_pair_variant<decltype(kk)::value>(), grid, k, false, s, a, b, a.max_items); });
}
int sweep3_chunk(int ntiles, int batch, int k) {
    if (k < 12) return 0;
    const long nwork = (long)ntiles * batch, g = std::min<long>(nwork, persistent_sweep_grid());
    return (int)((nwork + g - 1) / g);
}
int sweep3_nparts(int ntiles, int batch, int k) {
    const int chunk = sweep3_chunk(ntiles, batch, k);
    return chunk > 0 ? std::min(ntiles, (ntiles + chunk - 1) / chunk + 1) : ntiles;
}
hipError_t launch_sweep3(int k, hipStream_t s, const Stage3Args& a) {
    const bool list = a.items != nullptr;
    if (!stage3_launchable(k, a, false, true)) return hipErrorInvalidValue;
    if (a.nparts < 1 || (!list && (a.nparts != sweep3_nparts(a.ntiles, a.batch, k) || a.chunk != sweep3_chunk(a.ntiles, a.batch, k)))) return hipErrorInvalidValue;
    const long nwork = list ? (long)a.max_items : (long)a.ntiles * a.batch;
    const dim3 grid((unsigned)(k >= 12 ? (list ? std::min<long>(nwork, persistent_sweep_grid()) : (nwork + a.chunk - 1) / a.chunk) : nwork));
    const bool skipw = !list && a.supp != nullptr;
    const bool rlast = !skipw && a.r_only_last != 0;
    return with_tile_size(k, [&](auto kk) { return launch3(sweep_variant<decltype(kk)::value>(list, skipw, rlast), grid, k, true, s, a); });
}

hipError_t launch_sweep3_pair(int k, hipStream_t s, const Stage3Args& a, const Stage3Args& b) {
    if (!stage3_launchable(k, a, true, true) || !stage3_launchable(k, b, true, true)) return hipErrorInvalidValue;
    if (a.nparts < 1 || b.nparts < 1 || a.supp || b.supp || b.r_only_last) return hipErrorInvalidValue;
    const long longer = std::max(a.max_items, b.max_items);
    const dim3 grid((unsigned)(k >= 12 ? std::min<long>(longer, persistent_sweep_grid()) : (long)a.max_items + b.max_items));
    return with_tile_size(k, [&](auto kk) { return launch3(sweep_pair_variant<decltype(kk)::value>(a.r_only_last != 0), grid, k, true, s, a, b, a.max_items); });
}

__device__ __forceinline__ int tile_of_elem(const DevStage& st, long long e) {
    int t = 0;
    for (int i = 0; i < st.nub; ++i) t |= (int)((e >> st.ubits[i]) & 1) << i;
    return t;
}
__device__ __forceinline__ int lane_tiles(const DevStage& st, const long long* supp, int per_lane, const long long* extra, int nextra, int b,
                                          int (&tiles)[kMaxTileCands]) {
    int n = 0;
    auto add = [&](long long e) {
        if (e < 0) return;
        const int t = tile_of_elem(st, e);
        for (int i = 0; i < n; ++i)
            if (tiles[i] == t) return;
        tiles[n++] = t;
    };
    for (int k = 0; supp && k < per_lane; ++k) add(supp[(size_t)b * per_lane + k]);
    for (int k = 0; extra && k < nextra; ++k) add(extra[k]);
    return n;
}
__global__ __launch_bounds__(1024) void tile_items_kernel(const DevStage st, const long long* supp, int per_lane, const long long* extra, int nextra,
                                                          int batch, TileItem* items, int* nitems, int* lane_parts, int* prev_tiles,
                                                          TileItem* clear_items, int* nclear) {
    __shared__ int scan_a[1024], scan_b[1024];
    const int tid = threadIdx.x, per = (batch + 1023) / 1024;
    const int b0 = tid * per, b1 = min(batch, b0 + per);
    int tiles[kMaxTileCands];
    int mine = 0, mine_clear = 0;
    for (int b = b0; b < b1; ++b) {
        const int n = lane_tiles(st, supp, per_lane, extra, nextra, b, tiles);
        mine += n;
        if (prev_tiles)
            for (int k = 0; k < 2; ++k) {
                const int pt = prev_tiles[2 * b + k];
                bool stale = pt >= 0;
                for (int i = 0; i < n; ++i) stale = stale && tiles[i] != pt;
                mine_clear += stale ? 1 : 0;
            }
    }
    scan_a[tid] = mine; scan_b[tid] = mine_clear;
    __syncthreads();
    for (int d = 1; d < 1024; d <<= 1) {
        const int va = tid >= d ? scan_a[tid - d] : 0, vb = tid >= d ? scan_b[tid - d] : 0;
        __syncthreads();
        scan_a[tid] += va; scan_b[tid] += vb;
        __syncthreads();
    }
    int at = scan_a[tid] - mine, at_clear = scan_b[tid] - mine_clear;
    if (tid == 1023) { *nitems = scan_a[tid]; if (nclear) *nclear = scan_b[tid]; }
    for (int b = b0; b < b1; ++b) {
        const int n = lane_tiles(st, supp, per_lane, extra, nextra, b, tiles);
        if (lane_parts) lane_parts[b] = n;
        if (prev_tiles) {
            for (int k = 0; k < 2; ++k) {
                const int pt = prev_tiles[2 * b + k];
                bool stale = pt >= 0;
                for (int i = 0; i < n; ++i) stale = stale && tiles[i] != pt;
                if (stale) clear_items[at_clear++] = TileItem{b, pt, 0, 0};
            }
            prev_tiles[2 * b] = n > 0 ? tiles[0] : -1;
            prev_tiles[2 * b + 1] = n > 1 ? tiles[1] : -1;
        }
        for (int i = 0; i < n; ++i) items[at++] = TileItem{b, tiles[i], i, 0};
    }
}
hipError_t launch_tile_items(const DevStage& stage, const long long* supp, int per_lane, const long long* extra, int nextra, int batch,
                             TileItem* items, int* nitems, int* lane_parts, int* prev_tiles, TileItem* clear_items, int* nclear, hipStream_t s) {
    if ((supp ? per_lane : 0) + (extra ? nextra : 0) > kMaxTileCands || batch < 1) return hipErrorInvalidValue;
    if (prev_tiles && ((supp ? per_lane : 0) > 2 || (extra && nextra > 0) || !clear_items || !nclear)) return hipErrorInvalidValue;
    tile_items_kernel<<<1, 1024, 0, s>>>(stage, supp, per_lane, extra, nextra, batch, items, nitems, lane_parts, prev_tiles, clear_items, nclear);
    return hipGetLastError();
}
__global__ __launch_bounds__(256) void clear_tiles_kernel(const DevStage st, cplx* buf, size_t lane_stride, const TileItem* clear_items, const int* nclear) {
    if ((int)blockIdx.x >= *nclear) return;
    const TileItem it = clear_items[blockIdx.x];
    cplx* dst = buf + (size_t)it.lane * lane_stride + tile_base3(st, (unsigned)it.tile);
    for (unsigned l = threadIdx.x; l < (1u << st.k); l += 256) dst[tile_offset3(st, l)] = make_double2(0.0, 0.0);
}
hipError_t launch_clear_tiles(const DevStage& stage, void* buf, size_t lane_stride, const TileItem* clear_items, const int* nclear, int max_items,
                              hipStream_t s) {
    if (max_items < 1) return hipSuccess;
    clear_tiles_kernel<<<max_items, 256, 0, s>>>(stage, static_cast<cplx*>(buf), lane_stride, clear_items, nclear);
    return hipGetLastError();
}
hipError_t launch_ubuild(const UJob* jobs, int njobs, const double* thetas, int T, int batch, hipStream_t s, double* thetas_copy) {
    if (njobs < 1) return hipSuccess;
    ubuild_kernel<<<dim3(njobs, batch), 64, 0, s>>>(jobs, thetas, T, thetas_copy);
    return hipGetLastError();
}
hipError_t launch_rgrad(const DevSub3* subs, const DevGrp* grps, int entangler, const double* thetas, int T, const void* rpart,
                        int ntiles, int nsubs_total, void* partial, int nslots, int from, int to, int front, int batch, hipStream_t s,
                        const int* slot_theta, void* grads, void* mirror, GatherJob gather, int nparts, int chunk, int sparse_subs,
                        const int* lane_parts, int conj_sub, const double* umat, int nsubs_run, const RgradSecond* second_plan) {
    if (nsubs_total < 1) return hipSuccess;
    if (nsubs_run < 0 || nsubs_run > nsubs_total) nsubs_run = nsubs_total;
    RgradSecond second;
    memset(&second, 0, sizeof second);
    if (second_plan) second = *second_plan;
    const int extra = (gather.count > 0 && gather.buf ? 1 : 0) + second.count;
    if (nsubs_run + extra < 1) return hipSuccess;
    const int tiles_per_lane = ntiles;
    if (nparts <= 0) nparts = ntiles;
    ntiles = nparts;
    if (nparts >= 32 && second.count == 0)
        rgrad_kernel<4><<<dim3(nsubs_run + extra, batch), 256, 0, s>>>(subs, grps, entangler, thetas, T, static_cast<const cplx*>(rpart), ntiles,
                                                                  nsubs_total, static_cast<cplx*>(partial), nslots, from, to, front, slot_theta,
                                                                  static_cast<cplx*>(grads), static_cast<cplx*>(mirror), gather, tiles_per_lane, chunk, sparse_subs, lane_parts, conj_sub, umat, nsubs_run, second);
    else
        rgrad_kernel<1><<<dim3(nsubs_run + extra, batch), 64, 0, s>>>(subs, grps, entangler, thetas, T, static_cast<const cplx*>(rpart), ntiles,
                                                                 nsubs_total, static_cast<cplx*>(partial), nslots, from, to, front, slot_theta,
                                                                 static_cast<cplx*>(grads), static_cast<cplx*>(mirror), gather, tiles_per_lane, chunk, sparse_subs, lane_parts, conj_sub, umat, nsubs_run, second);
    return hipGetLastError();
}

}
```

aqc_research_amd/csrc/aqc_launch.h:

```cpp
#pragma once
#include <string>
#include <hip/hip_runtime.h>

#include <algorithm>
#include <cstddef>

#include "aqc_device.h"
#include "aqc_mps_walk.h"

namespace aqc {

struct StageArgs {
    const DevStage* stage;
    const DevOp* ops;
    const DevSub* subs;
    const DevMop* mops;
    const double* coef;
    int ncoef;
    const double2* in0;
    const double2* in1;
    double2* out0;
    double2* out1;
    size_t lane_stride;
    double2* partial;
    int nslots, ntiles_max;
    int from, to, front;
    int final_stage;
    int debug;
};

size_t apply_lds_bytes(int k);
size_t sweep_lds_bytes(int k, int threads);
hipError_t init_kernels();
hipError_t launch_apply(int ent, bool inverse, int ntiles, int batch, int threads, int k, hipStream_t s, const StageArgs& a);
hipError_t launch_sweep(int ent, int ntiles, int batch, int threads, int k, hipStream_t s, const StageArgs& a);
hipError_t launch_coef(const double* thetas, double* coef, int n, int nblocks, int tpb, int tail, int batch, hipStream_t s);
hipError_t launch_finalize(const void* partial, const int* theta_slots, const int* slot_ntiles, void* grads, int T,
                           int nslots, int ntiles_max, int n, int tpb, int from, int to, int front, int batch,
                           hipStream_t s, void* mirror = nullptr);
hipError_t launch_scatter_one(void* buf, size_t lane_stride, int batch, const long long* elem, hipStream_t s);
hipError_t launch_scatter_two(void* buf, size_t lane_stride, int batch, const long long* elem, const void* coef, long long* prev, hipStream_t s);
hipError_t launch_set_identity(void* buf, size_t lane_stride, int dim, int pitch, int batch, hipStream_t s);
hipError_t launch_gather(const void* buf, size_t lane_stride, const long long* elem, int count, int batch, void* out,
                         hipStream_t s, void* mirror = nullptr);
hipError_t launch_vdot(const void* a, const void* b, size_t lane_stride, size_t count, int batch, void* part, int nparts,
                       void* out, hipStream_t s);

hipError_t init_kernels2();
hipError_t launch_apply2(int ent, int ntiles, int batch, int k, hipStream_t s, const StageArgs& a);
hipError_t launch_sweep2(int ent, int ntiles, int batch, int k, int reg_bits, hipStream_t s, const StageArgs& a);

struct TileItem { int lane, tile, slot, pad; };
struct Stage3Args {
    DevStage stage;
    const DevSub3* subs;
    const double* umat;
    int nsubs_total;
    const double2* in0;
    const double2* in1;
    double2* out0;
    double2* out1;
    size_t lane_stride;
    double2* rpart;
    int ntiles;
    int batch;
    int chunk, nparts;
    int store_out;
    int r_only_last;
    const long long* supp;
    const TileItem* items;
    const int* nitems;
    int max_items;
    unsigned first_hi[16][4];
    int debug;
    unsigned long long* stamps;
};
constexpr int kStampSlots = 40;
void stage3_first_offsets(Stage3Args& a, const DevSub3& first_sub);
hipError_t init_kernels3();
int mfma_threads(int k, bool sweep);
int mfma_occupancy(int k, bool sweep);
hipError_t launch_apply3(int k, hipStream_t s, const Stage3Args& a);
hipError_t launch_sweep3(int k, hipStream_t s, const Stage3Args& a);
hipError_t launch_apply3_pair(int k, hipStream_t s, const Stage3Args& a, const Stage3Args& b);
hipError_t launch_sweep3_pair(int k, hipStream_t s, const Stage3Args& a, const Stage3Args& b);
void rgrad_print_stamps(int nsubs);
int sweep3_chunk(int ntiles, int batch, int k);
int sweep3_nparts(int ntiles, int batch, int k);
struct ProjMap { const unsigned* tab; int shift; };
struct ProjArgs {
    const double2* y;
    const double2* s;
    double2* out;
    int s_virtual, out_virtual;
    int staged;
    int keep_bits, k_bits, cb;
    ProjMap y_keep, y_k, s_k, s_c, o_keep, o_c;
    size_t lane_stride;
    const TileItem* items;
    const int* nitems;
    const int* lane_parts;
    int nub0, ubits0[32];
    unsigned ff_mask, cb_mask, tf_mask;
    int nvp;
    const unsigned* off_t;
    const unsigned* off_cb;
    const unsigned* it_of_c;
    const unsigned* off_us;
    int us_bits;
    size_t part_stride;
    double2* cpart;
    int cpart_shares;
    int t, ntiles_v;
    double2* vm;
    TileItem* vitems;
    int* vcount;
    int* vlane_parts;
    int batch;
};
hipError_t launch_project_init(const ProjArgs& a, hipStream_t s);
hipError_t launch_project_fused(const ProjArgs& a, const void* mend, void* ctile, void* yout, hipStream_t s);
hipError_t launch_project_amps(const ProjArgs& a, const long long* gather, int ngather, const long long* supp, void* small, const void* vy, const void* z,
                               hipStream_t s);
hipError_t launch_project(const ProjArgs& a, hipStream_t s);
struct UJob {
    const DevSub3* sub;
    const DevGrp* grps;
    double* umat;
    int index, nsubs;
    int inverse, entangler;
    double* umat_mirror;
    int mirror_index, mirror_nsubs;
};
hipError_t launch_ubuild(const UJob* jobs, int njobs, const double* thetas, int T, int batch, hipStream_t s, double* thetas_copy = nullptr);
struct GatherJob {
    const void* buf; size_t lane_stride; const long long* elem; int count; void* out; void* mirror;
};
struct RgradSecond {
    const DevSub3* subs;
    const DevGrp* grps;
    const double2* rpart;
    const int* lane_parts;
    const double* umat;
    int nparts, nsubs_total, count;
};
hipError_t launch_rgrad(const DevSub3* subs, const DevGrp* grps, int entangler, const double* thetas, int T, const void* rpart,
                        int ntiles, int nsubs_total, void* partial, int nslots, int from, int to, int front, int batch, hipStream_t s,
                        const int* slot_theta = nullptr, void* grads = nullptr, void* mirror = nullptr,
                        GatherJob gather = GatherJob{nullptr, 0, nullptr, 0, nullptr, nullptr},
                        int nparts = 0, int chunk = 0,
                        int sparse_subs = 0, const int* lane_parts = nullptr,
                        int conj_sub = -1, const double* umat = nullptr,
                        int nsubs_run = -1,
                        const RgradSecond* second_plan = nullptr);
constexpr int kMaxTileCands = 72;
hipError_t launch_tile_items(const DevStage& stage, const long long* supp, int per_lane, const long long* extra, int nextra, int batch,
                             TileItem* items, int* nitems, int* lane_parts, int* prev_tiles, TileItem* clear_items, int* nclear, hipStream_t s);
hipError_t launch_clear_tiles(const DevStage& stage, void* buf, size_t lane_stride, const TileItem* clear_items, const int* nclear, int max_items,
                              hipStream_t s);

struct LbState {
    int B, T, S, memory;
    double *x, *g, *f;
    double *d, *slope, *step;
    double *x_new;
    double *Smem, *Ymem, *rho;
    int *active, *done;
    long long* nit;
    double *weight, *fidelity;
    int* max_no;
    double2 *cur_hs, *cur_g0;
    double2 *acc_hs, *acc_g0;
};
hipError_t lb_prepare(const LbState& st, const void* hs, int update, double* f_out, void* raw_hs, void* x2, size_t lane_stride,
                      const long long* index, long long* prev, hipStream_t s);
hipError_t lb_take(const LbState& st, const void* grads, double* g_out, void* raw_g, hipStream_t s);
hipError_t lb_probe(const LbState& st, const void* hs, int* flags, hipStream_t s);
hipError_t lb_commit0(const LbState& st, const void* hs, const void* raw_g, double* f_out, double* g_out, hipStream_t s);
hipError_t lb_active(const LbState& st, double gtol, double fid_thr, int* flags, hipStream_t s);
hipError_t lb_direction(const LbState& st, int count, hipStream_t s);
hipError_t lb_trial(const LbState& st, double* thetas, hipStream_t s);
hipError_t lb_armijo(const LbState& st, double c1, const double* thetas, const double* ft, const void* raw_hs_t, const void* raw_g0_t,
                     int* flags, hipStream_t s);
hipError_t lb_copy_raw(const LbState& st, hipStream_t s);
hipError_t lb_history(const LbState& st, int count, double ftol, const double* f_acc, const double* g_acc, hipStream_t s);
struct LbMat {
    int k;
    double gtol, fobj_thr, fid_thr;
    double *gmax;
    double *ft, *gt, *gmax_t, *fid_t;
    double *f_acc, *g_acc, *gmax_acc, *fid_acc;
    int* status;
    int* flags;
};
enum { kLbNotDone = 1, kLbAnyActive = 2 };
enum { kLbNonFinite = 1 };
hipError_t lb_mat_value(const LbState& st, const LbMat& m, const void* trace, const void* grads, int init, hipStream_t s);
hipError_t lb_mat_direction(const LbState& st, const LbMat& m, int count, hipStream_t s);
hipError_t lb_mat_armijo(const LbState& st, const LbMat& m, double c1, const double* thetas, hipStream_t s);
hipError_t lb_mat_history(const LbState& st, const LbMat& m, int count, double ftol, int last, hipStream_t s);

hipError_t launch_mps_scale(void* g, const double* lam, int rows, int cols, hipStream_t s);
hipError_t launch_zgemm(bool conj_t, bool accum, int M, int N, int K, const void* A, int lda, const void* B, int ldb,
                        void* C, int ldc, hipStream_t s);
hipError_t launch_zgemm_bh(bool conj_t, bool accum, int M, int N, int K, const void* A, int lda, const void* B, int ldb,
                           void* C, int ldc, hipStream_t s);
hipError_t launch_mps_env_dot(const void* e, const void* rc, size_t count, void* out, hipStream_t s);
hipError_t launch_zgemm_batched(bool conj_t, bool accum, int M, int N, int K, const void* A, int lda, const void* B, int ldb,
                                void* C, int ldc, size_t stride_a, size_t stride_b, size_t stride_c, int nbatch, hipStream_t s);
hipError_t launch_zgemm_tables(int M, int N, int K, const void* const* a_tab, int lda, const void* const* b_tab, int ldb, void* const* c_tab, int ldc,
                               size_t stride_a, size_t stride_b, size_t stride_c, int outer, int inner, hipStream_t s, int b_transposed = 0);
hipError_t launch_mps_product(const void* const* t_tab, void* const* out_tab, int n, int count, hipStream_t s);
struct MpsSites {
    int n;
    size_t total;
    size_t offset[65];
    int lam_offset[64];
    int cols[64];
};
hipError_t launch_mps_scale_all(void* t, const double* lam, const MpsSites& sites, hipStream_t s);

int cd_num_parts(size_t npairs);
hipError_t launch_cd_dot(const void* w, const void* z, size_t npairs, int hbit, int kind, void* part, hipStream_t s);
hipError_t launch_cd_update(void* w, void* z, size_t npairs, int hbit, int kind, const void* part, int nparts,
                            const double* theta_in, double* theta_out, int tindex, double dim, hipStream_t s);
hipError_t launch_cd_entangle(void* w, void* z, size_t ngroups, int cbit, int tbit, int ent, hipStream_t s);
struct CdSegHost { int32_t ha, hb, ent, nrot, kind[4], on_b[4], tindex[4]; };
size_t cd_persistent_lds_bytes(int nbits, int T);
struct CdRule {
    int* status;
    int* nit;
    double* best_f;
    double* best_thetas;
    double* profile;
    double fobj_thr, dtheta_thr;
    int maxiter;
};
hipError_t launch_cd_persistent(const void* prog, int nsegs, int nbits, int col_bits, const void* target, size_t lane_stride, double* thetas,
                                int T, double* fobj, int nsweeps, int max_steps, int batch, hipStream_t s, const CdRule* rule = nullptr);
struct CdWide {
    void* w; void* z;
    size_t lane_stride;
    int ngroups, nparts;
    int ha, hb, ent;
    int kind, on_b, tindex;
    int next_kind, next_on_b;
    int T;
    const double* theta_in;
    double* theta_out;
    double* dmax;
    const int* status;
    const double* part_in;
    double* part_out;
    double inv_d2n;
};
int cd_wide_parts(size_t lane_elems);
hipError_t launch_cd_wide_open(const CdWide& a, int batch, hipStream_t s);
hipError_t launch_cd_wide_step(const CdWide& a, int batch, hipStream_t s);
struct CdClose {
    CdRule rule;
    const double2* trace;
    double* dmax;
    double* theta_own;
    const double* theta_cur;
    int T;
    double inv_d2n;
};
hipError_t launch_cd_close(const CdClose& a, int batch, hipStream_t s);
hipError_t launch_cd_count(int* status, int batch, int mark, int* running, hipStream_t s);


hipError_t launch_gate1q(const void* src, void* dst, int n, size_t ncols, int q, const double* g, hipStream_t s);
hipError_t launch_gate2q(const void* src, void* dst, int n, size_t ncols, int qc, int qt, const double* g, hipStream_t s);
int gate_dot_parts(int n, size_t ncols, int kind);
hipError_t launch_gate_dot(const void* w, const void* z, int n, size_t ncols, int kind, int q0, int q1, void* partial, void* out,
                           hipStream_t s);


int set_error(const std::string& msg);

hipError_t launch_svd_identity(void* V, int cols, hipStream_t s);
hipError_t launch_jacobi_round(void* W, int rows, void* V, int cols, const void* pairs, int npairs, double tol, const double* fro2, int* rotations,
                               hipStream_t s);
hipError_t launch_svd_fro2(const void* W, size_t n, double* out, hipStream_t s);
hipError_t launch_svd_load(const void* a, int m, int n, int mode, void* work, hipStream_t s);
hipError_t launch_svd_assemble(const void* W, const void* V, const int* ord, const double* sigma, int m, int n, int k, int mode, void* u, void* vh,
                               double* s_sorted, hipStream_t s);
bool svd_fits_small(int rows, int cols);
hipError_t launch_jacobi_small(void* W, int rows, void* V, int cols, double tol, int max_sweeps, int* sweeps_out, double* sigma_out,
                               hipStream_t s);
bool svd_fits_block(int rows, int cols);
int svd_block_size();
hipError_t launch_jacobi_block(void* W, int rows, void* V, int cols, const void* bpairs, int rounds, int per_round, double tol, int max_sweeps,
                               const double* fro2, int* rot, unsigned* bar, int* status, hipStream_t s);
hipError_t launch_svd_norms(const void* W, int rows, int cols, double* sigma, hipStream_t s);
hipError_t launch_mps_theta(const void* theta0, const double* lam_left, int chil, int chir, const double* g16, int mode, void* work, hipStream_t s);
size_t svd_batch_work_elems(int count, int m, int n);
size_t svd_batch_v_elems(int count, int m, int n);
hipError_t launch_svd_batch(int count, int m, int n, const int* d_rows, const int* d_cols, const void* d_a, void* d_u, double* d_s, void* d_vh,
                            int* d_sweeps, int* d_status, void* work, void* vmat, hipStream_t s);
constexpr int kLaneCap = 32;
constexpr int kLaneSite = 2 * kLaneCap * kLaneCap;
constexpr int kLaneEnv = kLaneCap * kLaneCap;
constexpr int kLaneNoConv = 1, kLaneOverflow = 2, kLaneZero = 4, kLaneLdsShort = 8;
struct LaneMps { void* T; double* lam; int* dims; double* discarded; int n, pad; };
hipError_t launch_lanes_gate1(const LaneMps& a, const LaneMps* b, const LaneOp1* ops, int nops, const LaneOp1& one, const double* thetas, int T, int lanes,
                              int bond_hint, hipStream_t s);
hipError_t launch_lanes_gate2(const LaneMps& m, const LaneMps* m2, const LaneOp2* ops, int nops, const LaneOp2& one, const double* thetas, int T,
                              double trunc_thr, int max_bond, int* status, int* peak, int lanes, int bond_hint, hipStream_t s,
                              unsigned long long* jstats = nullptr);
hipError_t launch_lanes_env_left(const LaneMps& w, const LaneMps& z, int p, const void* in, size_t in_stride, void* out, size_t out_stride,
                                 const double* gh8, int lanes, hipStream_t s);
hipError_t launch_lanes_env_right(const LaneMps& w, const LaneMps& z, int p, const void* in, size_t in_stride, void* out, size_t out_stride, int lanes,
                                  hipStream_t s);
hipError_t launch_lanes_env_dot(const LaneMps& w, const LaneMps& z, int hi, const void* e, size_t e_stride, const void* rc, size_t rc_stride, void* vals,
                                int nvals, int slot, int lanes, hipStream_t s);
struct LaneSteps { LaneGate1 g[3]; double gh[3][8]; int count, pad; };
hipError_t launch_lanes_grad_step(const LaneMps& w, const LaneMps& z, int q, const LaneSteps& steps, const double* thetas, int T, const void* env_l,
                                  size_t l_stride, const void* env_r, size_t r_stride, void* scratch, void* vals, int nvals, int slot, int lanes, hipStream_t s);
hipError_t launch_lanes_basis(const LaneMps& m, const unsigned char* bits , int lanes, hipStream_t s);
hipError_t launch_lanes_bank_dot(const LaneMps& bank, int count, const LaneMps& vh, int lanes, void* vals, int nvals, int slot0, int* status,
                                 int bond_hint, hipStream_t s);
hipError_t launch_lanes_env_init(void* env_l, size_t l_stride, void* env_r_last, size_t r_stride, int lanes, hipStream_t s);
bool mps_env_fits_small(int xa, int ua, int yb, int vb);
hipError_t launch_mps_env_left(const void* in, const void* A, const void* B, int xa, int ua, int yb, int vb, const double* gh8, void* out, hipStream_t s);
hipError_t launch_mps_env_right(const void* rc, const void* A, const void* B, int xa, int ua, int yb, int vb, void* out, hipStream_t s);
hipError_t launch_mps_theta_fused(const void* tq, const void* tq1, const double* lam_left, int chil, int chim, int chir, const double* g16, int mode,
                                  void* work, hipStream_t s);
hipError_t launch_mps_split(const void* W, const void* V, const int* ord, const double* sigma, const double* lam_left, int chil, int chir,
                            int k, int mode, double rescale, void* tq, void* tq1, const double* lam_new, double* lam_dst, hipStream_t s);
hipError_t launch_mps_colscale(void* t, const double* lam, size_t rows, int cols, int mul, hipStream_t s);

int sk_qr_slabs(int d);
hipError_t launch_sk_qr(void* a, void* scratch, size_t lane_stride, int lda, int d, int k, int batch, double abs_floor, void* partial, void* rinv, int* status,
                        hipStream_t s);
hipError_t launch_sk_alt(void* x, void* y, size_t lane_stride, int pitch, int d, int k, const void* u, size_t u_stride, const int* idx, int batch,
                         hipStream_t s);
hipError_t launch_sk_omega(void* out, size_t lane_stride, int pitch, int d, int k, unsigned long long seed, unsigned long long stream,
                           unsigned long long iteration, int normal, int batch, hipStream_t s);
hipError_t launch_sk_sub(void* a, const void* b, size_t lane_stride, int pitch, int d, int k, int batch, hipStream_t s);
struct SkAdam {
    int B, T, k, profile_stride;
    double* thetas;
    const double2* trace;
    const double2* grads;
    double *m, *v, *best_x;
    double *best_f, *profile;
    const double* lr;
    int *t, *nit, *flag;
    double beta1, beta2, eps, tol;
};
hipError_t launch_sk_adam(const SkAdam& st, int col, int do_update, hipStream_t s);

}
```

aqc_research_amd/csrc/aqc_ws.h:

```cpp
#pragma once
#include <hip/hip_runtime_api.h>

#include <cmath>
#include <cstdarg>
#include <cstdio>
#include <cstdlib>
#include <cstring>
#include <functional>
#include <initializer_list>
#include <map>
#include <memory>
#include <mutex>
#include <string>
#include <type_traits>
#include <vector>

#include "../../include/aqc_hip.h"
#include "aqc_devbuf.h"
#include "aqc_device.h"
#include "aqc_launch.h"
#include "aqc_plan.h"

namespace aqc {

int fail(const char* fmt, ...) __attribute__((format(printf, 1, 2)));

#define HIP_OK(expr)                                                                              \
    do {                                                                                          \
        hipError_t e_ = (expr);                                                                   \
        if (e_ != hipSuccess) return ::aqc::fail("%s failed: %s (%s:%d)", #expr, hipGetErrorString(e_), __FILE__, __LINE__); \
    } while (0)

inline int env_int(const char* name, int dflt) {
    const char* v = getenv(name);
    return (v && *v) ? atoi(v) : dflt;
}

inline int ceil_log2(int v) {
    int b = 0;
    while ((1 << b) < v) ++b;
    return b;
}

enum ULevel { kUNone = 0, kURoute = 1, kUAll = 2 };

struct HostPlan {
    Plan plan;
    std::vector<DevStage> h_stages;
    std::vector<DevOp> h_ops;
    std::vector<DevSub> h_subs;
    std::vector<DevMop> h_mops;
    int k = 0, ntiles = 0, reg_bits = 0;
    bool v2 = false;
    bool v3 = false;
    std::vector<DevSub3> h_subs3;
    std::vector<DevGrp> h_grps;
    int family() const { return v3 ? 3 : (v2 ? 2 : 1); }
};
static_assert(std::is_copy_constructible<HostPlan>::value && std::is_copy_assignable<HostPlan>::value,
              "a cached plan is copied out of the cache: it owns no device memory (a buffer member would make it move-only)");

struct DevPlan : HostPlan {
    DevBuf<DevStage> d_stages;
    DevBuf<DevOp> d_ops;
    DevBuf<DevSub> d_subs;
    DevBuf<DevMop> d_mops;
    DevBuf<DevSub3> d_subs3;
    DevBuf<DevGrp> d_grps;
    DevBuf<double> d_umat;
    DevBuf<double2> d_rpart;
    int u_level = kUNone;
    DevPlan& operator=(const HostPlan& host) { HostPlan::operator=(host); return *this; }
};

struct ListKey {
    static constexpr int kUnknown = -2, kGatherOnly = -1;
    int buf = kUnknown;
    unsigned long long supp = 0, gather = 0;
    bool operator==(const ListKey& o) const { return buf != kUnknown && buf == o.buf && supp == o.supp && gather == o.gather; }
};

struct EvalRoute {
    int x_buf = AQC_BUF_X;
    bool vdag = false;
    bool new_thetas = false;
    bool gather = false;
    bool gather_rides = false;
    bool grads = false;
    bool support_in_gather_set = false;
    bool sparse = false;
    enum VdagKind { kStages, kRestricted, kProjected } vdag_kind = kStages;
    bool skip_zero_w = false;
    int key_bits() const {
        static_assert(AQC_NUM_BUFS <= 8, "x_buf takes the low three bits");
        return x_buf | (vdag ? 8 : 0) | (gather ? 16 : 0) | (gather_rides ? 32 : 0) | (grads ? 64 : 0) | (sparse ? 128 : 0) |
               (support_in_gather_set ? 256 : 0) | (skip_zero_w ? 512 : 0) | ((int)vdag_kind << 10);
    }
};

struct ProjRoute {
    bool ok = false;
    int t = 0, cb = 0, us = 0, nv = 0, nvp = 0, kv = 0, ntiles_v = 0;
    int first_subs = 0;
    Program vprog;
    std::vector<int> rest;
    DevPlan vsw;
    DevPlan vinv;
    DevBuf<double2> vm;
    DevBuf<double2> vy;
    DevBuf<double2> vme;
    DevBuf<double2> cpart;
    int cpart_shares = 0;
    int vy_copies = 1;
    unsigned l0_mask = 0;
    DevBuf<unsigned> d_tab;
    std::vector<unsigned> h_tab;
    unsigned ff_mask = 0, cb_mask = 0, tf_mask = 0;
    DevBuf<TileItem> d_items;
    DevBuf<int> d_count;
    DevBuf<int> d_lane_parts;
    ListKey init_key;
};

void lower_plan(const Program& prog, const Plan& plan, HostPlan& out, int reg_bits, bool with_dots, bool mfma = false, bool presplit = false, int beam_width = 64);
int upload_plan(DevPlan& p);
Plan mirror_plan(const Plan& plan);

}

using aqc::DevBuf; using aqc::DevPlan; using aqc::HostPlan; using aqc::PinBuf; using aqc::Program; using aqc::UJob;

struct aqc_ctx {
    Program prog;
    std::recursive_mutex mu;
    std::map<std::vector<int>, HostPlan> plan_cache;
    std::map<int, aqc_ws*> oneshot;
};

struct aqc_ws {
    aqc_ctx* ctx = nullptr;
    int device = 0, batch = 1, ncols = 1, pitch = 1, col_bits = 0, nbits = 0, threads = 256;
    size_t lane_elems = 0;
    hipStream_t stream = nullptr;
    DevPlan fwd, inv, sweep;
    double* d_thetas = nullptr;
    DevBuf<double> d_thetas_own;
    DevBuf<double> d_theta_bank;
    int bank_sets = 0, gather_count = 0;
    DevBuf<double> d_coef;
    DevBuf<double2> bufs[AQC_NUM_BUFS];
    PinBuf<double> h_pin;
    size_t pin_thetas = 0, pin_grads = 0, pin_small = 0;
    DevBuf<double2> d_partial;
    DevBuf<double2> d_grads;
    double* mirror_grads = nullptr;
    double* mirror_small = nullptr;
    DevBuf<double2> d_small;
    DevBuf<double2> d_vdot_part;
    DevBuf<double2> d_vdot_out;
    DevBuf<long long> d_index;
    DevBuf<long long> d_tmp_index;
    DevBuf<double2> d_tmp_small;
    DevBuf<long long> d_basis_index;
    DevBuf<long long> d_combo_prev[AQC_NUM_BUFS];
    bool combo_valid[AQC_NUM_BUFS] = {false, false, false, false, false, false};
    std::vector<long long> combo_last_elem[AQC_NUM_BUFS];
    std::vector<double> combo_last_coef[AQC_NUM_BUFS];
    DevBuf<char> d_sur;
    PinBuf<char> h_sur;
    int sur_states = 0;
    DevBuf<double> d_sur_real;
    DevBuf<long long> d_combo_index;
    DevBuf<double2> d_combo_coef;
    DevBuf<int> d_theta_slots;
    DevBuf<int> d_slot_theta;
    bool grads_direct = false;
    DevBuf<int> d_slot_ntiles;
    int nslots = 0, vdot_parts = 0;
    bool coef_valid = false;
    bool need_coef = false;
    std::map<std::vector<long long>, hipGraphExec_t> graphs;
    bool capturing = false;
    DevBuf<UJob> d_ujobs;
    bool ujobs_mirror = false;
    DevBuf<UJob> d_ujobs_route;
    int n_ujobs_route = 0;
    struct MpsSlot {
        std::vector<int> dims;
        std::vector<size_t> offset;
        DevBuf<double2> d_t;
    } mps[AQC_MPS_SLOTS];
    DevBuf<double> d_mps_lam;
    DevBuf<double2> d_mps_scratch;
    struct MpsTabs { std::vector<const void*> host; DevBuf<const void*> dev; unsigned long long tick = 0; };
    DevBuf<aqc::CdSegHost> d_cd_prog;
    int cd_nsteps = 0;
    DevBuf<double> d_cd_thetas;
    DevBuf<double> d_cd_fobj;
    DevBuf<double> d_cd_best;
    DevBuf<double> d_cd_real;
    DevBuf<int> d_cd_int;
    DevBuf<double> d_cd_profile;
    DevBuf<double> d_cd_part;
    MpsTabs mps_tabs[32];
    unsigned long long mps_tabs_tick = 0;
    hipEvent_t ev0 = nullptr, ev1 = nullptr, pev0 = nullptr, pev1 = nullptr;
    hipStream_t copy_stream = nullptr;
    hipEvent_t ev_ready = nullptr, ev_copied = nullptr;
    hipStream_t mps_stream = nullptr;
    hipEvent_t ev_mps_fork = nullptr, ev_mps_join = nullptr;
    bool copy_pending = false;
    const double* theta_host = nullptr;
    bool inv_mirrored = false;
    bool ckpt_valid = false;
    bool w_clean = true;
    bool sparse_enabled = true;
    bool r_only_enabled = true;
    int r_only_max_subs = 12;
    bool skipw_enabled = false;
    long sparse_min_items = 512;
    unsigned long long supp_version[AQC_NUM_BUFS] = {0, 0, 0, 0, 0, 0};
    DevBuf<aqc::TileItem> d_sw_items;
    DevBuf<aqc::TileItem> d_sw_clear;
    DevBuf<int> d_sw_counts;
    DevBuf<int> d_sw_lane_parts;
    DevBuf<int> d_sw_prev_tiles;
    int sw_lists_built = 0;
    aqc::ListKey sw_items_key;
    DevBuf<double2> w2;
    DevBuf<double2> zw2;
    bool lazy_z_enabled = true;
    bool z_full = true;
    DevBuf<aqc::TileItem> d_vd_items;
    unsigned long long gather_gen = 0;
    aqc::ListKey vd_key;
    aqc::ListKey z_key;
    aqc::ProjRoute proj;
    bool proj_vdag_enabled = true;
    long long proj_vdag_min_elems = 1ll << 24;
    bool proj_fused_enabled = true;
    bool proj_pairs_enabled = true;
    bool proj_y0_ready = false;
    bool z_from_y = false;
    std::vector<long long> h_gather;
    aqc::ListKey projb_key;
    bool projb_ok = false;
    struct Sketch {
        DevBuf<double2> target;
        bool shared = false;
        DevBuf<double2> qr_part;
        DevBuf<double2> qr_rinv;
        DevBuf<double2> tmp;
        DevBuf<int> status;
        DevBuf<int> idx;
        DevBuf<double> adam;
        DevBuf<int> adam_i;
        DevBuf<double> profile;
        bool adam_started = false;
    } sk;
    bool profile = false;
    int64_t prof_count[AQC_NUM_KINDS] = {};
    double prof_ms[AQC_NUM_KINDS] = {};
    std::vector<std::pair<int, float>> prof_log;
};

namespace aqc {

struct ProfScope {
    aqc_ws* ws;
    int kind;
    ProfScope(aqc_ws* w, int k) : ws(w), kind(k) {
        if (ws->profile) (void)hipEventRecord(ws->pev0, ws->stream);
    }
    ~ProfScope() {
        if (!ws->profile) return;
        float ms = 0.f;
        if (hipEventRecord(ws->pev1, ws->stream) == hipSuccess && hipEventSynchronize(ws->pev1) == hipSuccess &&
            hipEventElapsedTime(&ms, ws->pev0, ws->pev1) == hipSuccess) {
            ws->prof_count[kind] += 1;
            ws->prof_ms[kind] += ms;
            if (ws->prof_log.size() < 100000) ws->prof_log.emplace_back(kind, ms);
        }
    }
};

inline int wait_result_copies(aqc_ws* ws) {
    if (!ws->copy_pending) return 0;
    HIP_OK(hipStreamSynchronize(ws->copy_stream));
    ws->copy_pending = false;
    return 0;
}
struct MirrorScope {
    aqc_ws* w;
    MirrorScope(aqc_ws* w_, double* grads, double* small) : w(w_) { w->mirror_grads = grads; w->mirror_small = small; }
    ~MirrorScope() { w->mirror_grads = nullptr; w->mirror_small = nullptr; w->theta_host = nullptr; }
};
inline bool direct_thetas(const aqc_ws* ws, bool zero_copy) {
    return zero_copy && ws->fwd.v3 && ws->inv.v3 && ws->sweep.v3 && !ws->need_coef;
}

int check_buf(const aqc_ws* ws, int buf);
int check_block_range(const aqc_ws* ws, int block_from, int block_to);
int ensure_coef(aqc_ws* ws);
int copy_in(aqc_ws* ws, double2* dst, const double* src, size_t rows);
int copy_out(aqc_ws* ws, double* dst, const double2* src, size_t rows);
int results_guard(aqc_ws* ws);
int before_read(aqc_ws* ws, int buf);
int before_gather(aqc_ws* ws, int buf);
int before_write(aqc_ws* ws, int buf, bool some_lanes = false);
void lhs_support_changed(aqc_ws* ws, int buf, std::vector<long long> elem = {}, std::vector<double> coef = {});
int run_coef(aqc_ws* ws, double* d_thetas);
void thetas_changed(aqc_ws* ws, double* d_thetas);
ListKey key_of(const aqc_ws* ws, int lhs_buf, bool gather);
bool built_for(const aqc_ws* ws, const ListKey& slot, const ListKey& key);
void record_key(const aqc_ws* ws, ListKey& slot, const ListKey& key);
void replay_state_after(aqc_ws* ws);
int eval_route(aqc_ws* ws, EvalRoute& route);
int enqueue_vdag(aqc_ws* ws, const EvalRoute& route);
int enqueue_gather(aqc_ws* ws, const EvalRoute& route);
void route_state_after(aqc_ws* ws, const EvalRoute& route);
int run_graph(aqc_ws* ws, const EvalRoute& route, std::initializer_list<long long> call, const std::function<int()>& enqueue);
void vdag_projected_state_after(aqc_ws* ws, int x_buf);
int grad_from_impl(aqc_ws* ws, const EvalRoute& route, int block_from, int block_to, int front_layer);
int sweep_r_only_sub(const aqc_ws* ws);
int ensure_umat(aqc_ws* ws, DevPlan& p, int need = kUAll);
int run_apply(aqc_ws* ws, bool inverse, int src_buf, int dst_buf);
Stage3Args stage3_args(aqc_ws* ws, const DevPlan& p, size_t s);
void stage3_first_list(const aqc_ws* ws, Stage3Args& a);
void stage3_sweep_fields(Stage3Args& a, const DevPlan& p, int nparts, int chunk);
void drop_graphs(aqc_ws* ws);
void proj_plan(aqc_ws* ws, int low_bits);
int proj_alloc(aqc_ws* ws);
bool sweep_route_projected(const aqc_ws* ws, bool sparse);
bool projected_pairs(const aqc_ws* ws);
Stage3Args virtual_stage3_args(aqc_ws* ws, const DevPlan& v, size_t s);
Stage3Args projected_sweep_stage(aqc_ws* ws, size_t s);
int run_projected_stages(aqc_ws* ws);
aqc::RgradSecond projected_rgrad_plan(aqc_ws* ws);
bool vdag_route_projected(aqc_ws* ws, int x_buf);
int run_vdag_projected(aqc_ws* ws, int x_buf);
int proj_fix_amplitudes(aqc_ws* ws, int x_buf);
int ensure_sweep_items(aqc_ws* ws, int x_buf);

}
```

aqc_research_amd/csrc/aqc_ws_project.cpp:

```cpp
#include "aqc_ws.h"

#include <algorithm>

using namespace aqc;

namespace aqc {

namespace {
int popc(uint64_t v) { return __builtin_popcountll(v); }
unsigned deposit_bits(unsigned v, const std::vector<int>& bits) {
    unsigned o = 0;
    for (size_t j = 0; j < bits.size(); ++j)
        if (v >> j & 1) o |= 1u << bits[j];
    return o;
}
}

void proj_plan(aqc_ws* ws, int low_bits) {
    ProjRoute& pr = ws->proj;
    pr.ok = false;
    const Program& prog = ws->ctx->prog;
    const DevPlan& p = ws->sweep;
    if (env_int("AQC_PROJECTED", 1) == 0 || !ws->sparse_enabled || !ws->inv_mirrored || !p.v3 || ws->col_bits != 0 || ws->ncols != 1 ||
        p.plan.stages.size() < 2 || prog.n > 30)
        return;
    const int n = prog.n;
    uint64_t L0 = 0, T = 0;
    for (int b : p.plan.stages[0].bits) L0 |= 1ull << b;
    pr.rest.clear();
    for (size_t s = 1; s < p.plan.stages.size(); ++s)
        for (int gi : p.plan.stages[s].ops) {
            const GateGroup& g = prog.groups[gi];
            pr.rest.push_back(gi);
            T |= 1ull << g.q0;
            if (g.q1 >= 0) T |= 1ull << g.q1;
        }
    if (pr.rest.empty()) return;
    const uint64_t all = (1ull << n) - 1, F = all & ~L0, Cb = T & L0, Us = L0 & ~T;
    pr.t = popc(T); pr.cb = popc(Cb); pr.us = popc(Us);
    pr.nv = pr.t + pr.cb;
    if ((Us & 15) != 15 || pr.t < 4 || pr.cb > 6 || pr.nv + 2 > n || pr.nv > 20) return;
    pr.nvp = std::max(pr.nv, 8);
    pr.kv = std::min(pr.nvp, p.k);
    pr.ntiles_v = 1 << (pr.nvp - pr.kv);
    pr.first_subs = p.h_stages[0].nsubs;
    std::vector<int> tbits, cbits, usbits;
    std::vector<int> vq(n, -1);
    for (int b = 0; b < n; ++b) {
        if (T >> b & 1) { vq[b] = (int)tbits.size(); tbits.push_back(b); }
        if (Cb >> b & 1) cbits.push_back(b);
        if (Us >> b & 1) usbits.push_back(b);
    }
    pr.vprog = prog;
    for (int gi : pr.rest) {
        GateGroup& g = pr.vprog.groups[gi];
        g.q0 = vq[g.q0];
        if (g.q1 >= 0) g.q1 = vq[g.q1];
    }
    Plan best;
    for (int lb = std::max(low_bits, 2); lb >= 2; --lb) {
        Plan cand = make_plan(pr.vprog, 0, pr.kv, lb, false, &pr.rest, pr.nvp);
        if (best.stages.empty() || cand.stages.size() < best.stages.size()) best = cand;
    }
    lower_plan(pr.vprog, best, pr.vsw, 4, true, true, false, env_int("AQC_PROJECTED_BEAM", 8));
    if (!pr.vsw.v3 || !check_plan(pr.vprog, pr.vsw.plan, &pr.rest).empty()) return;
    lower_plan(pr.vprog, mirror_plan(pr.vsw.plan), pr.vinv, 4, false, true, true);
    if (!pr.vinv.v3 || pr.vinv.h_subs3.size() != pr.vsw.h_subs3.size()) return;
    for (DevPlan* q : {&pr.vsw, &pr.vinv})
        for (DevStage& ds : q->h_stages) {
            if (ds.nub >= 32) return;
            ds.ubits[ds.nub++] = pr.nvp;
            ds.ntiles *= 2;
        }
    pr.l0_mask = (unsigned)L0;
    pr.ff_mask = (unsigned)(F & ~T);
    pr.cb_mask = (unsigned)Cb;
    pr.tf_mask = (unsigned)(T & F);
    pr.h_tab.clear();
    for (unsigned i = 0; i < (1u << pr.t); ++i) pr.h_tab.push_back(deposit_bits(i, tbits));
    for (unsigned k = 0; k < (1u << pr.us); ++k) pr.h_tab.push_back(deposit_bits(k, usbits));
    for (unsigned c = 0; c < (1u << pr.cb); ++c) pr.h_tab.push_back(deposit_bits(c, cbits));
    for (unsigned c = 0; c < (1u << pr.cb); ++c) {
        const unsigned addr = deposit_bits(c, cbits);
        unsigned it = 0;
        for (size_t j = 0; j < tbits.size(); ++j)
            if (addr >> tbits[j] & 1) it |= 1u << j;
        pr.h_tab.push_back(it);
    }
    pr.ok = true;
    if (env_int("AQC_VERBOSE", 0))
        fprintf(stderr, "aqc_hip: projected route: the sweep's stages after the first run on %d virtual qubits (%d touched, %d shared with the first "
                "stage) instead of %d: %zu stage(s) of 2^%d tiles, %zu sub-stages\n", pr.nv, pr.t, pr.cb, n, pr.vsw.h_stages.size(), pr.kv,
                pr.vsw.h_subs3.size());
}

int proj_alloc(aqc_ws* ws) {
    ProjRoute& pr = ws->proj;
    if (!pr.ok) return 0;
    const size_t B = (size_t)ws->batch;
    if (upload_plan(pr.vsw) || upload_plan(pr.vinv)) return 1;
    const size_t nsubs = std::max<size_t>(pr.vsw.h_subs3.size(), 1);
    if (pr.vsw.d_umat.alloc(B * nsubs * 12 * 64) || pr.vinv.d_umat.alloc(B * nsubs * 12 * 64)) return 1;
    if (pr.vsw.d_rpart.alloc(B * nsubs * (2 * (size_t)pr.ntiles_v) * 256)) return 1;
    const size_t velems = B * (2ull << pr.nvp), vbytes = sizeof(double2) * velems;
    pr.vy_copies = pr.us > 8 && pr.us <= 10 && pr.cb <= 4 ? 1 << (pr.us - 8) : 1;
    if (pr.vm.alloc(velems) || pr.vy.alloc(velems * pr.vy_copies)) return 1;
    HIP_OK(hipMemsetAsync(pr.vm, 0, vbytes, ws->stream));
    HIP_OK(hipMemsetAsync(pr.vy, 0, vbytes * pr.vy_copies, ws->stream));
    pr.cpart_shares = 0;
    const long want_wgs = env_int("AQC_PROJECTED_FUSED_WGS", 512);
    if (pr.us <= 10 && pr.cb <= 4 && (long)B < want_wgs) {
        int shares = 1;
        const int cap = env_int("AQC_PROJECTED_FUSED_MAX_SHARES", 64);
        while ((long)B * pr.vy_copies * shares < want_wgs && 2 * shares <= (1 << (pr.t - 4)) && 2 * shares <= cap) shares *= 2;
        if (shares > 1) {
            if (pr.cpart.alloc((size_t)shares * 2 * B * (16ull << pr.us))) return 1;
            pr.cpart_shares = shares;
        }
    }
    if (pr.vme.alloc(velems)) return 1;
    HIP_OK(hipMemsetAsync(pr.vme, 0, vbytes, ws->stream));
    if (pr.d_tab.upload(pr.h_tab) || pr.d_items.alloc(2 * B * pr.ntiles_v) || pr.d_count.alloc(1) || pr.d_lane_parts.alloc(B)) return 1;
    HIP_OK(hipMemsetAsync(pr.d_count, 0, sizeof(int), ws->stream));
    HIP_OK(hipMemsetAsync(pr.d_lane_parts, 0, sizeof(int) * B, ws->stream));
    return 0;
}

bool sweep_route_projected(const aqc_ws* ws, bool sparse) { return sparse && ws->proj.ok; }

static ProjArgs proj_args(aqc_ws* ws);
static int ensure_pattern(aqc_ws* ws, const ProjArgs& a) {
    ProjRoute& pr = ws->proj;
    if (pr.vsw.h_stages.size() == 1 && built_for(ws, pr.init_key, ws->sw_items_key)) return 0;
    ProfScope ps(ws, AQC_K_MISC);
    HIP_OK(launch_project_init(a, ws->stream));
    record_key(ws, pr.init_key, ws->sw_items_key);
    return 0;
}

static ProjArgs proj_args(aqc_ws* ws) {
    ProjRoute& pr = ws->proj;
    ProjArgs a;
    memset(&a, 0, sizeof a);
    a.lane_stride = ws->lane_elems;
    a.items = ws->d_sw_items;
    a.nitems = ws->d_sw_counts;
    a.lane_parts = ws->d_sw_lane_parts;
    const DevStage& s0 = ws->sweep.h_stages[0];
    a.nub0 = s0.nub;
    for (int i = 0; i < s0.nub; ++i) a.ubits0[i] = s0.ubits[i];
    a.ff_mask = pr.ff_mask; a.cb_mask = pr.cb_mask; a.tf_mask = pr.tf_mask;
    a.nvp = pr.nvp;
    a.off_t = pr.d_tab;
    a.off_cb = pr.d_tab + (1u << pr.t) + (1u << pr.us);
    a.it_of_c = a.off_cb + (1u << pr.cb);
    a.off_us = pr.d_tab + (1u << pr.t);
    a.us_bits = pr.us;
    a.t = pr.t; a.cb = pr.cb; a.ntiles_v = pr.ntiles_v;
    a.vm = pr.vm;
    a.vitems = pr.d_items; a.vcount = pr.d_count; a.vlane_parts = pr.d_lane_parts;
    a.batch = ws->batch;
    return a;
}

static ProjArgs y_product(aqc_ws* ws, ProjArgs a, const double2* y) {
    const ProjRoute& pr = ws->proj;
    a.y = y;
    a.s = ws->bufs[AQC_BUF_W];
    a.out = pr.vy;
    a.s_virtual = 0; a.out_virtual = 1;
    a.staged = 1;
    a.keep_bits = pr.t; a.k_bits = pr.us;
    a.y_keep = ProjMap{a.off_t, 0};
    a.y_k = ProjMap{a.off_us, 0};
    a.s_k = ProjMap{a.off_us, 0};
    a.s_c = ProjMap{a.off_cb, 0};
    a.o_keep = ProjMap{nullptr, 0};
    a.o_c = ProjMap{nullptr, pr.t};
    return a;
}

int run_projected_stages(aqc_ws* ws) {
    ProjRoute& pr = ws->proj;
    if (!ws->proj_y0_ready) {
        const ProjArgs a = proj_args(ws);
        if (ensure_pattern(ws, a)) return 1;
        ProfScope ps(ws, AQC_K_PROJECT);
        HIP_OK(launch_project(y_product(ws, a, ws->bufs[AQC_BUF_ZW]), ws->stream));
    }
    for (size_t s = 0; s < pr.vsw.h_stages.size(); ++s) {
        const Stage3Args a = projected_sweep_stage(ws, s);
        ProfScope ps(ws, AQC_K_SWEEP_VIRTUAL);
        HIP_OK(launch_sweep3(pr.kv, ws->stream, a));
    }
    return 0;
}

Stage3Args virtual_stage3_args(aqc_ws* ws, const DevPlan& v, size_t s) {
    const ProjRoute& pr = ws->proj;
    Stage3Args a = stage3_args(ws, v, s);
    a.lane_stride = 2ull << pr.nvp;
    a.ntiles = 2 * pr.ntiles_v;
    a.items = pr.d_items; a.nitems = pr.d_count; a.max_items = 2 * ws->batch * pr.ntiles_v;
    return a;
}
Stage3Args projected_sweep_stage(aqc_ws* ws, size_t s) {
    const ProjRoute& pr = ws->proj;
    Stage3Args a = virtual_stage3_args(ws, pr.vsw, s);
    a.in0 = pr.vm; a.in1 = pr.vy; a.out0 = pr.vm; a.out1 = pr.vy;
    a.store_out = s + 1 < pr.vsw.h_stages.size() ? 3 : 0;
    stage3_sweep_fields(a, pr.vsw, a.ntiles, 0);
    return a;
}

bool projected_pairs(const aqc_ws* ws) {
    const ProjRoute& pr = ws->proj;
    return pr.ok && ws->proj_pairs_enabled && !ws->capturing && pr.vsw.h_stages.size() == 1 && pr.vinv.h_stages.size() == 1 &&
           ws->sweep.k == pr.kv && ws->inv.k == pr.kv;
}

RgradSecond projected_rgrad_plan(aqc_ws* ws) {
    ProjRoute& pr = ws->proj;
    DevPlan& v = pr.vsw;
    RgradSecond r;
    memset(&r, 0, sizeof r);
    r.subs = v.d_subs3; r.grps = v.d_grps; r.rpart = v.d_rpart; r.lane_parts = pr.d_lane_parts; r.umat = v.d_umat;
    r.nparts = 2 * pr.ntiles_v;
    r.nsubs_total = r.count = (int)v.h_subs3.size();
    return r;
}

bool vdag_route_projected(aqc_ws* ws, int x_buf) {
    ProjRoute& pr = ws->proj;
    if (!pr.ok || !ws->proj_vdag_enabled || ws->capturing || (long long)ws->lane_elems * ws->batch < ws->proj_vdag_min_elems) return false;
    const ListKey key = key_of(ws, x_buf, true);
    if (ws->projb_key == key) return ws->projb_ok;
    ws->projb_key = key;
    ws->projb_ok = false;
    const std::vector<long long>& el = ws->combo_last_elem[x_buf];
    const std::vector<double>& cf = ws->combo_last_coef[x_buf];
    const size_t B = (size_t)ws->batch;
    if (el.size() != 2 * B || cf.size() != 4 * B || (ws->gather_count > 0 && ws->h_gather.size() != (size_t)ws->gather_count)) return false;
    const unsigned fmask = ~pr.l0_mask & (unsigned)((1ull << ws->ctx->prog.n) - 1);
    for (size_t b = 0; b < B; ++b) {
        if (el[2 * b] < 0 || el[2 * b + 1] >= 0 || cf[4 * b] != 1.0 || cf[4 * b + 1] != 0.0) return false;
        const unsigned e = (unsigned)el[2 * b];
        for (long long gl : ws->h_gather) {
            const unsigned d = e ^ (unsigned)gl;
            if ((d & fmask) == 0) continue;
            if ((d & pr.l0_mask) != 0 || (d & pr.ff_mask) != 0) return false;
        }
    }
    ws->projb_ok = true;
    return true;
}

struct VirtualRun { const DevPlan& plan; const double2* src; double2* dst; };
static Stage3Args virtual_apply_stage(aqc_ws* ws, const VirtualRun& v, size_t s) {
    Stage3Args a = virtual_stage3_args(ws, v.plan, s);
    a.in0 = s == 0 ? v.src : v.dst;
    a.out0 = v.dst;
    return a;
}
static int enqueue_couple(aqc_ws* ws, int k, const Stage3Args* real, const VirtualRun* v) {
    if (real && v) {
        ProfScope ps(ws, AQC_K_APPLY_VIRTUAL);
        HIP_OK(launch_apply3_pair(k, ws->stream, *real, virtual_apply_stage(ws, *v, 0)));
    } else if (real) {
        ProfScope ps(ws, AQC_K_APPLY_LIST);
        HIP_OK(launch_apply3(k, ws->stream, *real));
    } else {
        for (size_t s = 0; s < v->plan.h_stages.size(); ++s) {
            ProfScope ps(ws, AQC_K_APPLY_VIRTUAL);
            HIP_OK(launch_apply3(ws->proj.kv, ws->stream, virtual_apply_stage(ws, *v, s)));
        }
    }
    return 0;
}

int run_vdag_projected(aqc_ws* ws, int x_buf) {
    ProjRoute& pr = ws->proj;
    const DevPlan& p = ws->sweep;
    const DevPlan& iv = ws->inv;
    if (ensure_umat(ws, ws->inv, kURoute)) return 1;
    if (!ws->d_sw_items || !ws->w_clean) return fail("objective by projection without the sparse route's preparation");
    if (ensure_sweep_items(ws, x_buf)) return 1;
    Stage3Args psi = stage3_args(ws, p, 0);
    psi.in0 = ws->bufs[x_buf];
    psi.out0 = ws->bufs[AQC_BUF_W];
    stage3_first_list(ws, psi);
    Stage3Args last = stage3_args(ws, iv, iv.h_stages.size() - 1);
    last.in0 = ws->bufs[AQC_BUF_ZW];
    last.out0 = ws->bufs[AQC_BUF_Z];
    stage3_first_list(ws, last);
    const VirtualRun mend{pr.vsw, pr.vm, pr.vme};
    const VirtualRun y0{pr.vinv, pr.vy, pr.vy};
    const ProjArgs a = proj_args(ws);
    const bool pairs = projected_pairs(ws);

    if (!pairs && enqueue_couple(ws, p.k, &psi, nullptr)) return 1;
    if (ensure_pattern(ws, a)) return 1;
    if (enqueue_couple(ws, p.k, pairs ? &psi : nullptr, &mend)) return 1;
    if (ws->proj_fused_enabled && pr.us <= 10 && pr.cb <= 4 && (pr.us <= 8 || pr.vy_copies == 1 << (pr.us - 8))) {
        ProjArgs q = a;
        q.part_stride = (size_t)ws->batch * (2ull << pr.nvp);
        q.cpart = pr.cpart; q.cpart_shares = pr.cpart_shares;
        q.y = ws->bufs[AQC_BUF_Y]; q.s = ws->bufs[AQC_BUF_W];
        ProfScope ps(ws, AQC_K_PROJECT);
        HIP_OK(launch_project_fused(q, pr.vme, ws->bufs[AQC_BUF_ZW], pr.vy, ws->stream));
    } else {
        {
            ProfScope ps(ws, AQC_K_PROJECT);
            HIP_OK(launch_project(y_product(ws, a, ws->bufs[AQC_BUF_Y]), ws->stream));
        }
        ProjArgs q = a;
        q.y = ws->bufs[AQC_BUF_Y]; q.s = pr.vme; q.out = ws->bufs[AQC_BUF_ZW];
        q.s_virtual = 1; q.out_virtual = 0; q.staged = 0;
        q.keep_bits = pr.us; q.k_bits = pr.t;
        q.y_keep = ProjMap{a.off_us, 0}; q.y_k = ProjMap{a.off_t, 0};
        q.s_k = ProjMap{nullptr, 0}; q.s_c = ProjMap{nullptr, pr.t};
        q.o_keep = ProjMap{a.off_us, 0}; q.o_c = ProjMap{a.off_cb, 0};
        ProfScope ps(ws, AQC_K_PROJECT);
        HIP_OK(launch_project(q, ws->stream));
    }
    if (!pairs && enqueue_couple(ws, iv.k, nullptr, &y0)) return 1;
    if (enqueue_couple(ws, iv.k, &last, pairs ? &y0 : nullptr)) return 1;
    vdag_projected_state_after(ws, x_buf);
    return 0;
}

int proj_fix_amplitudes(aqc_ws* ws, int x_buf) {
    ProjRoute& pr = ws->proj;
    if (results_guard(ws)) return 1;
    ProfScope ps(ws, AQC_K_MISC);
    ProjArgs a = proj_args(ws);
    HIP_OK(launch_project_amps(a, ws->d_index, ws->gather_count, ws->d_combo_prev[x_buf], ws->d_small, pr.vy, ws->bufs[AQC_BUF_Z], ws->stream));
    return 0;
}

}
```

aqc_research_amd/csrc/aqc_ws_sweep.cpp:

```cpp
#include "aqc_ws.h"

#include <algorithm>

using namespace aqc;

namespace aqc {


void thetas_changed(aqc_ws* ws, double* d_thetas) {
    ws->d_thetas = d_thetas;
    ws->coef_valid = true;
    ws->fwd.u_level = ws->inv.u_level = ws->sweep.u_level = kUNone;
    ws->ckpt_valid = false;
    ws->z_from_y = false;
    ws->proj_y0_ready = false;
}

static void umat_state_after(aqc_ws* ws, const DevPlan& p, int level = kUAll) {
    if (!p.v3) return;
    if (&p == &ws->fwd) ws->fwd.u_level = kUAll;
    else ws->inv.u_level = ws->sweep.u_level = std::max(ws->sweep.u_level, level);
}
static int route_level(const aqc_ws* ws) { return ws->d_ujobs_route ? kURoute : kUAll; }

// ... 190 lines not shown
            a.out0 = s + 1 == m ? ws->bufs[dst_buf] : ws->bufs[mid];
#ifdef AQC_TUNING
            const size_t nwg = (size_t)p.ntiles * ws->batch;
            if (stamps_begin(ws, a, nwg)) return 1;
#endif
            {
                ProfScope ps(ws, AQC_K_APPLY);
                HIP_OK(launch_apply3(p.k, ws->stream, a));
            }
#ifdef AQC_TUNING
            if (stamps_apply(ws, a, s, nwg)) return 1;
#endif
        }
        apply_state_after(ws, inverse, src_buf, dst_buf);
        return 0;
    }
    for (size_t s = 0; s < p.h_stages.size(); ++s) {
        StageArgs a = stage_args(ws, p, s);
        a.in0 = s == 0 ? ws->bufs[src_buf] : ws->bufs[dst_buf];
        a.out0 = ws->bufs[dst_buf];
        a.final_stage = (s + 1 == p.h_stages.size()) ? 1 : 0;
        ProfScope ps(ws, AQC_K_APPLY);
        if (p.v2) HIP_OK(launch_apply2(prog.entangler, p.ntiles, ws->batch, p.k, ws->stream, a));
        else HIP_OK(launch_apply(prog.entangler, inverse, p.ntiles, ws->batch, ws->threads, p.k, ws->stream, a));
    }
    apply_state_after(ws, inverse, src_buf, dst_buf);
    return 0;
}

static bool vdag_route_restricted(const aqc_ws* ws) {
    return ws->lazy_z_enabled && 2 + ws->gather_count <= kMaxTileCands;
}
static Stage3Args last_vdag_stage(aqc_ws* ws) {
    DevPlan& p = ws->inv;
    Stage3Args a = stage3_args(ws, p, p.h_stages.size() - 1);
    a.in0 = ws->bufs[AQC_BUF_ZW];
    a.out0 = ws->bufs[AQC_BUF_Z];
    return a;
}
static void vdag_restricted_state_after(aqc_ws* ws, int x_buf, int level = kUAll) {
    apply_state_after(ws, true, AQC_BUF_Y, AQC_BUF_Z, level);
    ws->z_full = false;
    ws->z_key = key_of(ws, x_buf, true);
}
void vdag_projected_state_after(aqc_ws* ws, int x_buf) {
    vdag_restricted_state_after(ws, x_buf, route_level(ws));
    ws->z_key.gather = 0;
    ws->ckpt_valid = false;
    ws->z_from_y = true;
    ws->proj_y0_ready = true;
}
static int run_vdag_restricted(aqc_ws* ws, int x_buf, bool support_in_gather_set) {
    DevPlan& p = ws->inv;
    if (ensure_umat(ws, p)) return 1;
    const size_t m = p.h_stages.size();
    const size_t per_lane = 2 + (size_t)ws->gather_count;
    if (ws->d_vd_items.capacity() < per_lane * ws->batch) return fail("objective V^H inside a captured graph without its preparation");
    for (size_t s = 0; s + 1 < m; ++s) {
        Stage3Args a = stage3_args(ws, p, s);
        a.in0 = s == 0 ? ws->bufs[AQC_BUF_Y] : ws->bufs[AQC_BUF_ZW];
        a.out0 = ws->bufs[AQC_BUF_ZW];
        ProfScope ps(ws, AQC_K_APPLY);
        HIP_OK(launch_apply3(p.k, ws->stream, a));
    }
    const bool gather_only = support_in_gather_set && ws->gather_count > 0;
    const ListKey key = key_of(ws, gather_only ? ListKey::kGatherOnly : x_buf, true);
    if (!built_for(ws, ws->vd_key, key)) {
        ProfScope ps(ws, AQC_K_MISC);
        HIP_OK(launch_tile_items(p.h_stages[m - 1], gather_only ? nullptr : ws->d_combo_prev[x_buf], 2, ws->gather_count > 0 ? ws->d_index : nullptr,
                                 ws->gather_count, ws->batch, ws->d_vd_items, ws->d_sw_counts + 2, nullptr, nullptr, nullptr, nullptr, ws->stream));
        record_key(ws, ws->vd_key, key);
    }
    Stage3Args a = last_vdag_stage(ws);
    a.items = ws->d_vd_items;
    a.nitems = ws->d_sw_counts + 2;
    a.max_items = (int)(per_lane * ws->batch);
    ws->sw_lists_built |= 2;
    {
        ProfScope ps(ws, AQC_K_APPLY_LIST);
        HIP_OK(launch_apply3(p.k, ws->stream, a));
    }
    vdag_restricted_state_after(ws, x_buf);
    return 0;
}
static int ensure_z_full(aqc_ws* ws, bool reader) {
    if (ws->z_full) return 0;
    if (ws->capturing) return fail("BUF_Z is partial inside a captured graph");
    if (ws->ckpt_valid && ws->inv.u_level != kUNone) {
        if (ensure_umat(ws, ws->inv)) return 1;
        Stage3Args a = last_vdag_stage(ws);
        ProfScope ps(ws, AQC_K_APPLY);
        HIP_OK(launch_apply3(ws->inv.k, ws->stream, a));
        ws->z_full = true;
        return 0;
    }
    if (!reader) return 0;
    if (ws->z_from_y && ws->inv.u_level != kUNone) {
        ws->z_full = true;
        return run_apply(ws, true, AQC_BUF_Y, AQC_BUF_Z);
    }
    return fail("BUF_Z holds V^H y only on the tiles the last one-call evaluation read, and the thetas (or ZW) have changed since: "
                "run aqc_ws_apply(inverse) for the whole vector");
}

void drop_graphs(aqc_ws* ws) {
    for (auto& kv : ws->graphs) (void)hipGraphExecDestroy(kv.second);
    ws->graphs.clear();
}

static bool sweep_route_sparse(const aqc_ws* ws, int x_buf, bool will_vdag) {
    const DevPlan& p = ws->sweep;
    if (!ws->sparse_enabled || !p.v3 || !ws->inv_mirrored || p.h_stages.size() < 2) return false;
    if (!ws->combo_valid[x_buf] || !ws->d_combo_prev[x_buf]) return false;
    if (!(will_vdag ? keeps_checkpoint(ws, true, AQC_BUF_Y, AQC_BUF_Z) : (ws->ckpt_valid || ws->proj_y0_ready))) return false;
    return (long)p.ntiles * ws->batch >= ws->sparse_min_items;
}
int sweep_r_only_sub(const aqc_ws* ws) {
    const DevPlan& p = ws->sweep;
    if (!p.v3 || !ws->r_only_enabled || p.h_stages.empty()) return -1;
    const DevStage& last = p.h_stages.back();
    if (last.nsubs < 1 || last.nsubs > ws->r_only_max_subs || (p.k >= 12 && last.nsubs == 1)) return -1;
    return last.sub_begin + last.nsubs - 1;
}
static bool sweep_skips_zero_w(const aqc_ws* ws, int x_buf) {
    return ws->skipw_enabled && ws->sweep.v3 && ws->combo_valid[x_buf] && ws->d_combo_prev[x_buf] != nullptr;
}
static int sweep_sparse_prepare(aqc_ws* ws) {
    const DevPlan& p = ws->sweep;
    const int B = ws->batch;
    if (!ws->d_sw_items) {
        if (ws->d_sw_items.alloc(2 * (size_t)B) || ws->d_sw_clear.alloc(2 * (size_t)B) || ws->d_sw_counts.alloc(4)) return 1;
        HIP_OK(hipMemsetAsync(ws->d_sw_counts, 0, sizeof(int) * 4, ws->stream));
        if (ws->d_sw_lane_parts.alloc(B) || ws->d_sw_prev_tiles.alloc(2 * (size_t)B)) return 1;
        ws->w_clean = false;
    }
    if (p.h_stages.size() >= 3 && !ws->w2 && !ws->proj.ok) {
        if (ws->w2.alloc((size_t)B * ws->lane_elems) || ws->zw2.alloc((size_t)B * ws->lane_elems)) return 1;
    }
    const size_t vd_need = (2 + (size_t)ws->gather_count) * B;
    if (ws->lazy_z_enabled && ws->d_vd_items.capacity() < vd_need) {
        HIP_OK(hipStreamSynchronize(ws->stream));
        if (ws->d_vd_items.reserve(vd_need)) return 1;
        ws->vd_key = ListKey{};
    }
    if (!ws->w_clean) {
        HIP_OK(hipMemsetAsync(ws->bufs[AQC_BUF_W], 0, sizeof(double2) * (size_t)B * ws->lane_elems, ws->stream));
        HIP_OK(hipMemsetAsync(ws->d_sw_prev_tiles, 0xff, sizeof(int) * 2 * B, ws->stream));
        ws->w_clean = true;
        ws->sw_items_key = ListKey{};
    }
    return 0;
}
static void sweep_state_after(aqc_ws* ws, bool sparse) {
    umat_state_after(ws, ws->sweep, sweep_route_projected(ws, sparse) ? route_level(ws) : kUAll);
    ws->proj_y0_ready = false;
    if (!sparse) {
        ws->w_clean = false;
        ws->ckpt_valid = false;
    }
}

int eval_route(aqc_ws* ws, EvalRoute& r) {
    r.sparse = r.grads && (r.vdag || !r.new_thetas) && sweep_route_sparse(ws, r.x_buf, r.vdag);
    r.skip_zero_w = r.grads && sweep_skips_zero_w(ws, r.x_buf);
    r.vdag_kind = EvalRoute::kStages;
    if (r.sparse && sweep_sparse_prepare(ws)) return 1;
    if (!(r.sparse && r.vdag && vdag_route_restricted(ws))) return 0;
    const bool projected = !r.gather_rides && !r.support_in_gather_set && vdag_route_projected(ws, r.x_buf);
    r.vdag_kind = projected ? EvalRoute::kProjected : EvalRoute::kRestricted;
    return 0;
}
int enqueue_vdag(aqc_ws* ws, const EvalRoute& r) {
    if (r.vdag_kind == EvalRoute::kProjected) return run_vdag_projected(ws, r.x_buf);
    if (r.vdag_kind == EvalRoute::kRestricted) return run_vdag_restricted(ws, r.x_buf, r.support_in_gather_set);
    return run_apply(ws, true, AQC_BUF_Y, AQC_BUF_Z);
}
int enqueue_gather(aqc_ws* ws, const EvalRoute& r) {
    return r.vdag_kind == EvalRoute::kProjected ? proj_fix_amplitudes(ws, r.x_buf) : aqc_ws_gather_launch(ws, AQC_BUF_Z);
}
void route_state_after(aqc_ws* ws, const EvalRoute& r) {
    if (r.vdag && r.vdag_kind == EvalRoute::kProjected) vdag_projected_state_after(ws, r.x_buf);
    else if (r.vdag && r.vdag_kind == EvalRoute::kRestricted) vdag_restricted_state_after(ws, r.x_buf);
    else if (r.vdag) apply_state_after(ws, true, AQC_BUF_Y, AQC_BUF_Z);
    if (r.support_in_gather_set) lhs_support_changed(ws, r.x_buf);
    if (r.grads) sweep_state_after(ws, r.sparse);
}
static std::vector<long long> graph_key(const aqc_ws* ws, const EvalRoute& r, std::initializer_list<long long> call) {
    std::vector<long long> key;
    key.reserve(call.size() + 5);
    key.insert(key.end(), call.begin(), call.end());
    key.push_back(r.key_bits());
    for (const void* addr : {(const void*)ws->d_small, (const void*)ws->h_pin, (const void*)ws->d_combo_prev[r.x_buf], (const void*)ws->d_vd_items})
        key.push_back((long long)(size_t)addr);
    return key;
}

int run_graph(aqc_ws* ws, const EvalRoute& route, std::initializer_list<long long> call, const std::function<int()>& enqueue) {
    const std::vector<long long> key = graph_key(ws, route, call);
    auto it = ws->graphs.find(key);
    if (it == ws->graphs.end()) {
        hipGraph_t graph = nullptr;
        hipGraphExec_t exec = nullptr;
        HIP_OK(hipStreamSynchronize(ws->stream));
        HIP_OK(hipStreamBeginCapture(ws->stream, hipStreamCaptureModeThreadLocal));
        ws->capturing = true;
        const int rc = enqueue();
        ws->capturing = false;
        const hipError_t e = hipStreamEndCapture(ws->stream, &graph);
        if (rc != 0) { if (graph) (void)hipGraphDestroy(graph); return 1; }
        if (e != hipSuccess || !graph) return fail("hipStreamEndCapture failed: %s", hipGetErrorString(e));
        const hipError_t ei = hipGraphInstantiate(&exec, graph, nullptr, nullptr, 0);
        (void)hipGraphDestroy(graph);
        if (ei != hipSuccess) return fail("hipGraphInstantiate failed: %s", hipGetErrorString(ei));
        if (ws->graphs.size() >= 16) drop_graphs(ws);
        it = ws->graphs.emplace(key, exec).first;
    }
    thetas_changed(ws, ws->d_thetas_own);
    route_state_after(ws, route);
    replay_state_after(ws);
    HIP_OK(hipGraphLaunch(it->second, ws->stream));
    return 0;
}

int ensure_sweep_items(aqc_ws* ws, int x_buf) {
    const DevPlan& p = ws->sweep;
    const ListKey key = key_of(ws, x_buf, false);
    if (!built_for(ws, ws->sw_items_key, key)) {
        ProfScope ps(ws, AQC_K_MISC);
        HIP_OK(launch_tile_items(p.h_stages[0], ws->d_combo_prev[x_buf], 2, nullptr, 0, ws->batch, ws->d_sw_items, ws->d_sw_counts,
                                 ws->d_sw_lane_parts, ws->d_sw_prev_tiles, ws->d_sw_clear, ws->d_sw_counts + 1, ws->stream));
        HIP_OK(launch_clear_tiles(p.h_stages[0], ws->bufs[AQC_BUF_W], ws->lane_elems, ws->d_sw_clear, ws->d_sw_counts + 1, 2 * ws->batch, ws->stream));
        record_key(ws, ws->sw_items_key, key);
        ws->sw_lists_built |= 1;
    }
    return 0;
}

static int sweep_mfma(aqc_ws* ws, const EvalRoute& route, int block_from, int block_to, int front_layer) {
    const Program& prog = ws->ctx->prog;
    DevPlan& p = ws->sweep;
    const int x_buf = route.x_buf;
    const int nsubs = (int)p.h_subs3.size();
    const size_t m = p.h_stages.size();
    const int nparts = sweep3_nparts(p.ntiles, ws->batch, p.k), chunk = sweep3_chunk(p.ntiles, ws->batch, p.k);
    const bool sparse = route.sparse, skipw = route.skip_zero_w;
    const bool projected = sweep_route_projected(ws, sparse);
    if (ensure_umat(ws, p, projected ? kURoute : kUAll)) return 1;
    int r_only_sub = skipw || projected ? -1 : sweep_r_only_sub(ws);
    const bool first_stage_r_only = projected && ws->proj_y0_ready && ws->r_only_enabled && p.h_stages[0].nsubs >= 2 &&
                                    p.h_stages[0].nsubs <= ws->r_only_max_subs;
    if (first_stage_r_only) r_only_sub = p.h_stages[0].sub_begin + p.h_stages[0].nsubs - 1;
    bool pair_virtual = projected && ws->proj_y0_ready && projected_pairs(ws);
#ifdef AQC_TUNING
    if (env_int("AQC_STAMPS", 0) != 0) pair_virtual = false;
#endif
    if (!ws->z_full && !(sparse && ((route.support_in_gather_set && ws->z_key.gather == ws->gather_gen) ||
                                    (ws->z_key.buf == x_buf && ws->z_key.supp == ws->supp_version[x_buf]))) && ensure_z_full(ws, true))
        return 1;
    if (sparse) {
        if (!ws->d_sw_items || !ws->w_clean || (m >= 3 && !ws->w2 && !projected)) return fail("sparse sweep inside a captured graph without its preparation");
        if (ensure_sweep_items(ws, x_buf)) return 1;
    }
    for (size_t s = 0; s < (projected ? 1 : m); ++s) {
        Stage3Args a = stage3_args(ws, p, s);
        if (sparse) {
            double2* w2 = m >= 3 ? ws->w2 : nullptr;
            double2* z2 = m >= 3 ? ws->zw2 : nullptr;
            a.in0 = s == 0 ? ws->bufs[x_buf] : (s == 1 ? ws->bufs[AQC_BUF_W] : w2);
            a.in1 = s == 0 ? ws->bufs[AQC_BUF_Z] : (s == 1 ? ws->bufs[AQC_BUF_ZW] : z2);
            a.out0 = s == 0 ? ws->bufs[AQC_BUF_W] : w2;
            a.out1 = s == 0 ? nullptr : z2;
            a.store_out = s + 1 < m ? (s == 0 ? 1 : 3) : 0;
            if (s == 0) stage3_first_list(ws, a);
            if (s == 0 && first_stage_r_only) { a.r_only_last = 1; a.store_out = 0; }
        } else {
            a.in0 = s == 0 ? ws->bufs[x_buf] : ws->bufs[AQC_BUF_W];
            a.in1 = s == 0 ? ws->bufs[AQC_BUF_Z] : ws->bufs[AQC_BUF_ZW];
            a.out0 = ws->bufs[AQC_BUF_W];
            a.out1 = ws->bufs[AQC_BUF_ZW];
            a.store_out = s + 1 < m ? 3 : 0;
        }
        if (skipw && !a.items) a.supp = ws->d_combo_prev[x_buf];
        if (s + 1 == m && r_only_sub >= 0) a.r_only_last = 1;
        stage3_sweep_fields(a, p, nparts, chunk);
#ifdef AQC_TUNING
        const size_t nwg = (size_t)p.ntiles * ws->batch;
        a.debug = env_int("AQC_DEBUG_SKIP", 0);
        if (stamps_begin(ws, a, nwg)) return 1;
#endif
        if (pair_virtual) {
            const Stage3Args b = projected_sweep_stage(ws, 0);
            ProfScope ps(ws, AQC_K_SWEEP_LIST);
            HIP_OK(launch_sweep3_pair(p.k, ws->stream, a, b));
        } else {
            ProfScope ps(ws, a.items ? AQC_K_SWEEP_LIST : AQC_K_SWEEP);
            HIP_OK(launch_sweep3(p.k, ws->stream, a));
        }
#ifdef AQC_TUNING
        if (stamps_sweep(ws, a, s, nwg)) return 1;
#endif
    }
    if (projected && !pair_virtual && run_projected_stages(ws)) return 1;
    sweep_state_after(ws, sparse);
    ProfScope ps(ws, AQC_K_FINALIZE);
    RgradSecond vwalk;
    if (projected) vwalk = projected_rgrad_plan(ws);
    HIP_OK(launch_rgrad(p.d_subs3, p.d_grps, prog.entangler, ws->d_thetas, prog.num_thetas(), p.d_rpart, p.ntiles, nsubs, ws->d_partial,
                        ws->nslots, block_from, block_to, front_layer ? 1 : 0, ws->batch, ws->stream,
                        ws->grads_direct ? ws->d_slot_theta : nullptr, ws->d_grads, ws->mirror_grads,
                        route.gather_rides ? GatherJob{ws->bufs[AQC_BUF_Z], ws->lane_elems, ws->d_index, ws->gather_count, ws->d_small, ws->mirror_small}
                                         : GatherJob{nullptr, 0, nullptr, 0, nullptr, nullptr},
                        nparts, chunk,
                        sparse ? p.h_stages[0].nsubs : 0, sparse ? ws->d_sw_lane_parts : nullptr, r_only_sub, p.d_umat,
                        projected ? p.h_stages[0].nsubs : -1, projected ? &vwalk : nullptr));
#ifdef AQC_TUNING
    if (env_int("AQC_STAMPS", 0) != 0) { HIP_OK(hipStreamSynchronize(ws->stream)); rgrad_print_stamps(nsubs); }
#endif
    if (!ws->grads_direct)
        HIP_OK(launch_finalize(ws->d_partial, ws->d_theta_slots, ws->d_slot_ntiles, ws->d_grads, prog.num_thetas(), ws->nslots,
                               1, prog.n, prog.tpb, block_from, block_to, front_layer ? 1 : 0, ws->batch, ws->stream, ws->mirror_grads));
    return 0;
}

static int sweep_valu(aqc_ws* ws, int x_buf, int block_from, int block_to, int front_layer) {
    const Program& prog = ws->ctx->prog;
    DevPlan& p = ws->sweep;
    if (before_read(ws, AQC_BUF_Z)) return 1;
    for (size_t s = 0; s < p.h_stages.size(); ++s) {
        StageArgs a = stage_args(ws, p, s);
        a.in0 = s == 0 ? ws->bufs[x_buf] : ws->bufs[AQC_BUF_W];
        a.in1 = s == 0 ? ws->bufs[AQC_BUF_Z] : ws->bufs[AQC_BUF_ZW];
        a.out0 = ws->bufs[AQC_BUF_W];
        a.out1 = ws->bufs[AQC_BUF_ZW];
        a.partial = ws->d_partial; a.nslots = ws->nslots; a.ntiles_max = p.ntiles;
#ifdef AQC_TUNING
        a.debug = env_int("AQC_DEBUG_SKIP", 0);
#endif
        a.from = block_from; a.to = block_to; a.front = front_layer ? 1 : 0;
        ProfScope ps(ws, AQC_K_SWEEP);
        if (p.v2) HIP_OK(launch_sweep2(prog.entangler, p.ntiles, ws->batch, p.k, p.reg_bits, ws->stream, a));
        else HIP_OK(launch_sweep(prog.entangler, p.ntiles, ws->batch, ws->threads, p.k, ws->stream, a));
    }
    sweep_state_after(ws, false);
    ProfScope ps(ws, AQC_K_FINALIZE);
    HIP_OK(launch_finalize(ws->d_partial, ws->d_theta_slots, ws->d_slot_ntiles, ws->d_grads, prog.num_thetas(), ws->nslots,
                           p.ntiles, prog.n, prog.tpb, block_from, block_to, front_layer ? 1 : 0, ws->batch, ws->stream, ws->mirror_grads));
    return 0;
}

static int sweep_refused(aqc_ws* ws, int x_buf, int block_from, int block_to) {
    if (check_buf(ws, x_buf)) return 1;
    if (x_buf == AQC_BUF_W || x_buf == AQC_BUF_ZW || x_buf == AQC_BUF_Z) return fail("lhs buffer must not be Z, W or ZW");
    return ensure_coef(ws) || check_block_range(ws, block_from, block_to);
}

int grad_from_impl(aqc_ws* ws, const EvalRoute& route, int block_from, int block_to, int front_layer) {
    const int x_buf = route.x_buf;
    if (sweep_refused(ws, x_buf, block_from, block_to) || results_guard(ws)) return 1;
    if (block_from < 0) { block_from = 0; block_to = ws->ctx->prog.num_blocks; }
    HIP_OK(hipSetDevice(ws->device));
    return ws->sweep.v3 ? sweep_mfma(ws, route, block_from, block_to, front_layer) : sweep_valu(ws, x_buf, block_from, block_to, front_layer);
}

}

extern "C" {

int aqc_ws_apply(aqc_ws* ws, int inverse, int src_buf, int dst_buf) {
    if (check_buf(ws, src_buf) || check_buf(ws, dst_buf)) return 1;
    if (ensure_coef(ws)) return 1;
    HIP_OK(hipSetDevice(ws->device));
    return run_apply(ws, inverse != 0, src_buf, dst_buf);
}

int aqc_ws_sweep_r_only_sub(aqc_ws* ws) { return ws ? sweep_r_only_sub(ws) : -1; }

int aqc_ws_grad(aqc_ws* ws, int block_from, int block_to, int front_layer) {
    return aqc_ws_grad_from(ws, AQC_BUF_X, block_from, block_to, front_layer);
}

int aqc_ws_grad_from(aqc_ws* ws, int x_buf, int block_from, int block_to, int front_layer) {
    if (sweep_refused(ws, x_buf, block_from, block_to)) return 1;
    HIP_OK(hipSetDevice(ws->device));
    EvalRoute route;
    route.x_buf = x_buf; route.grads = true;
    if (eval_route(ws, route)) return 1;
    return grad_from_impl(ws, route, block_from, block_to, front_layer);
}

int aqc_ws_objective_launch(aqc_ws* ws, int x_buf, int block_from, int block_to, int front_layer) {
    if (check_buf(ws, x_buf)) return 1;
    if (x_buf == AQC_BUF_W || x_buf == AQC_BUF_ZW || x_buf == AQC_BUF_Z || x_buf == AQC_BUF_Y) return fail("lhs buffer must be X or X2");
    if (check_block_range(ws, block_from, block_to)) return 1;
    if (ensure_coef(ws)) return 1;
    HIP_OK(hipSetDevice(ws->device));
    EvalRoute route;
    route.x_buf = x_buf; route.vdag = route.grads = true; route.gather = ws->gather_count > 0;
    if (eval_route(ws, route)) return 1;
    if (enqueue_vdag(ws, route)) return 1;
    if (route.gather && enqueue_gather(ws, route)) return 1;
    return grad_from_impl(ws, route, block_from, block_to, front_layer);
}

int aqc_ws_eval(aqc_ws* ws, const double* thetas, int do_vdag, double* gathered, int x_buf, int block_from, int block_to,
                int front_layer, double* grads) {
    if (!ws) return fail("null workspace");
    HIP_OK(hipSetDevice(ws->device));
    if (wait_result_copies(ws)) return 1;
    const Program& prog = ws->ctx->prog;
    const size_t nth = (size_t)ws->batch * prog.num_thetas();
    double* pin_th = ws->h_pin;
    double* pin_gr = ws->h_pin + ws->pin_thetas;
    double* pin_sm = pin_gr + ws->pin_grads;
    size_t nsm = 0;
    if (gathered) {
        if (ws->gather_count < 1) return fail("aqc_ws_gather_setup has not been called");
        nsm = (size_t)ws->batch * ws->gather_count;
        if (2 * nsm > ws->pin_small) return fail("too many gathered amplitudes for the staging buffer");
    }
    if (check_buf(ws, x_buf)) return 1;
    if (grads && check_block_range(ws, block_from, block_to)) return 1;
    if (!thetas && (do_vdag || grads) && ensure_coef(ws)) return 1;
    const bool zero_copy = sizeof(double2) * (nth + nsm) <= 65536;
    MirrorScope mirror_scope(ws, zero_copy ? pin_gr : nullptr, zero_copy ? pin_sm : nullptr);
    if (!do_vdag && (gathered || grads) && before_read(ws, AQC_BUF_Z)) return 1;
    EvalRoute route;
    route.x_buf = x_buf; route.vdag = do_vdag != 0; route.new_thetas = thetas != nullptr;
    route.gather = gathered != nullptr; route.grads = grads != nullptr;
    route.gather_rides = gathered && grads && zero_copy && ws->sweep.v3;
    if (eval_route(ws, route)) return 1;
    auto enqueue = [&]() -> int {
        if (thetas) {
            const bool direct = (do_vdag || grads) && direct_thetas(ws, zero_copy);
            if (!direct) HIP_OK(hipMemcpyAsync(ws->d_thetas_own, pin_th, sizeof(double) * nth, hipMemcpyHostToDevice, ws->stream));
            if (run_coef(ws, ws->d_thetas_own)) return 1;
            ws->theta_host = direct ? pin_th : nullptr;
        }
        if (route.vdag && enqueue_vdag(ws, route)) return 1;
        if (route.gather && !route.gather_rides) {
            if (enqueue_gather(ws, route)) return 1;
            if (!zero_copy) HIP_OK(hipMemcpyAsync(pin_sm, ws->d_small, sizeof(double2) * nsm, hipMemcpyDeviceToHost, ws->stream));
        }
        if (grads) {
            if (grad_from_impl(ws, route, block_from, block_to, front_layer)) return 1;
            if (!zero_copy) HIP_OK(hipMemcpyAsync(pin_gr, ws->d_grads, sizeof(double2) * nth, hipMemcpyDeviceToHost, ws->stream));
        }
        ws->theta_host = nullptr;
        return 0;
    };
    if (thetas) memcpy(pin_th, thetas, sizeof(double) * nth);
    static const bool graphs_on = env_int("AQC_GRAPH", 1) != 0;
    if (thetas && graphs_on && !ws->profile) {
        if (run_graph(ws, route, {0, block_from, block_to, front_layer, (long long)ws->gather_count}, enqueue)) return 1;
    } else if (enqueue()) {
        return 1;
    }
    HIP_OK(hipStreamSynchronize(ws->stream));
    if (gathered) memcpy(gathered, pin_sm, sizeof(double2) * nsm);
    if (grads) memcpy(grads, pin_gr, sizeof(double2) * nth);
    return 0;
}

}
```

Measured before the change: 1.189 million evals/s.

## Cache decoded gate-group matrices from U builder for reuse in gradient walk

The U-build kernel now writes each decoded gate group's matrices and rotation cos/sin into a per-batch 256-byte record table. The gradient walk kernel reads these records instead of re-decoding groups from thetas in shared memory, which removes the stage_groups work and its barriers. It also adds a fast path for summing partial results when there are few tiles, and uses readfirstlane to keep group indices uniform in ubuild. In exchange it costs extra global memory and writes, and adds a dependency on the U builder having run for the current thetas, which is guarded by a runtime check.

```diff
diff --git a/aqc_research_amd/csrc/aqc_api.cpp b/aqc_research_amd/csrc/aqc_api.cpp
--- a/aqc_research_amd/csrc/aqc_api.cpp
+++ b/aqc_research_amd/csrc/aqc_api.cpp
@@ -255,6 +255,7 @@
     ws->proj_vdag_enabled = env_int("AQC_PROJECTED_VDAG", 1) != 0;
     ws->proj_fused_enabled = env_int("AQC_PROJECTED_FUSED", 1) != 0;
     ws->proj_pairs_enabled = env_int("AQC_PROJECTED_PAIRS", 1) != 0;
+    ws->gm_table = env_int("AQC_GM_TABLE", 1) != 0;
     ws->proj_vdag_min_elems = (long long)env_int("AQC_PROJECTED_VDAG_MIN_ELEMS", 1 << 24);
     ws->skipw_enabled = env_int("AQC_SKIP_ZERO_W", 0) != 0;
     for (DevPlan* p : {&ws->fwd, &ws->inv, &ws->sweep}) {
@@ -315,7 +316,8 @@
         if (p && p->v3)
             for (size_t i = 0; i < p->h_subs3.size(); ++i) {
                 if (p == &ws->inv && ws->ujobs_mirror) continue;
-                UJob j{p->d_subs3 + i, p->d_grps, p->d_umat, (int)i, (int)p->h_subs3.size(), p->plan.inverse ? 1 : 0, prog.entangler, nullptr, 0, 0};
+                UJob j{p->d_subs3 + i, p->d_grps, p->d_umat, (int)i, (int)p->h_subs3.size(), p->plan.inverse ? 1 : 0, prog.entangler, nullptr, 0, 0,
+                       p->d_gtab, (int)p->h_grps.size()};
                 if (p == &ws->sweep && ws->ujobs_mirror) { j.umat_mirror = ws->inv.d_umat; j.mirror_index = nsw - 1 - (int)i; j.mirror_nsubs = nsw; }
                 if (p == vsw) {
                     const int nvs = (int)vsw->h_subs3.size();
@@ -351,6 +353,7 @@
     if (ws->d_partial.alloc(B * std::max(ws->nslots, 1) * t.partial_tiles)) return 1;
     for (DevPlan* p : {&ws->fwd, &ws->inv, &ws->sweep})
         if (p->v3 && p->d_umat.alloc(B * std::max<size_t>(p->h_subs3.size(), 1) * 12 * 64)) return 1;
+    if (ws->sweep.v3 && ws->gm_table && ws->sweep.d_gtab.alloc(B * std::max<size_t>(ws->sweep.h_grps.size(), 1))) return 1;
     if (ws_upload_ujobs(ws)) return 1;
     if (ws->sweep.v3 && ws->sweep.d_rpart.alloc(B * std::max<size_t>(ws->sweep.h_subs3.size(), 1) *
                                                 sweep3_nparts(ws->sweep.ntiles, ws->batch, ws->sweep.k) * 256)) return 1;
diff --git a/aqc_research_amd/csrc/aqc_kernels3.hip b/aqc_research_amd/csrc/aqc_kernels3.hip
--- a/aqc_research_amd/csrc/aqc_kernels3.hip
+++ b/aqc_research_amd/csrc/aqc_kernels3.hip
@@ -71,6 +71,10 @@
 #define AQC_EXP_UBUILD_SKIP 0
 #endif
 constexpr int kUbuildSkip = AQC_EXP_UBUILD_SKIP;
+#ifndef AQC_EXP_SMALL_OFF
+#define AQC_EXP_SMALL_OFF 0
+#endif
+constexpr int kSmallOff = AQC_EXP_SMALL_OFF;
 
 constexpr int kSweepSpread = AQC_SWEEP_SPREAD, kApplySpread = AQC_APPLY_SPREAD;
 template <int K, bool SWEEP = false> struct TileShape {
@@ -608,7 +612,12 @@
     a0 = make_double2(m00.x * x.x - sg * m00.y * x.y + m01.x * y.x - sg * m01.y * y.y, m00.x * x.y + sg * m00.y * x.x + m01.x * y.y + sg * m01.y * y.x);
     a1 = make_double2(m10.x * x.x - sg * m10.y * x.y + m11.x * y.x - sg * m11.y * y.y, m10.x * x.y + sg * m10.y * x.x + m11.x * y.y + sg * m11.y * y.x);
 }
-__device__ __forceinline__ void stage_groups(Gm* gm, const DevGrp* grps, int begin, int count, const double* th, int ent, int lane) {
+__device__ __forceinline__ void gm_to_rec(const Gm& g, GmRec& r) {
+#pragma unroll
+    for (int k = 0; k < 4; ++k) { r.c[k] = g.c[k]; r.t[k] = g.t[k]; r.rc[k] = g.rc[k]; r.rs[k] = g.rs[k]; }
+    r.ec = g.ec; r.es = g.es;
+}
+__device__ __forceinline__ void stage_groups(Gm* gm, const DevGrp* grps, int begin, int count, const double* th, int ent, int lane, GmRec* rec = nullptr) {
     {
         const int gi = lane >> 2, k = lane & 3;
         if (gi < count) {
@@ -647,6 +656,7 @@
         if (d.flags & 2) { m2_rz(kR, kR, a); m2_mul(a, g.t, m); g.t[0] = m[0]; g.t[1] = m[1]; g.t[2] = m[2]; g.t[3] = m[3]; }
     }
     gm[lane] = g;
+    if (rec) gm_to_rec(g, rec[lane]);
 }
 __device__ __forceinline__ int grp_index(const Gm& g, int l, int rest) {
     return ((l >> 1) << g.pc) | ((l & 1) << g.pt) | ((rest & 1) << g.o0) | ((rest >> 1) << g.o1);
@@ -669,6 +679,14 @@
         entangle(MODE == 1 ? -g.es : g.es);
     }
 }
+__device__ __forceinline__ void gm_from_rec(Gm& g, const GmRec& r, const DevGrp& d) {
+#pragma unroll
+    for (int k = 0; k < 4; ++k) { g.c[k] = r.c[k]; g.t[k] = r.t[k]; }
+    g.ec = r.ec; g.es = r.es;
+    g.type = d.type; g.pc = d.pc; g.pt = d.pt; g.flags = d.flags; g.slot0 = d.slot0; g.jblock = d.jblock;
+    const int mask = 0xF & ~(1 << d.pc) & ~(1 << d.pt);
+    g.o0 = __ffs(mask) - 1; g.o1 = __ffs(mask & (mask - 1)) - 1;
+}
 
 __global__ __launch_bounds__(64) void ubuild_kernel(const UJob* jobs, const double* thetas, int T, double* thetas_copy) {
     __shared__ cplx u[256];
@@ -688,10 +706,15 @@
     for (int base = 0; base < sub.ngrp; base += kGrpChunk) {
         const int count = min(kGrpChunk, sub.ngrp - base);
         __syncthreads();
-        stage_groups(gm, job.grps, sub.grp_begin + base, count, th, job.entangler, lane);
+        stage_groups(gm, job.grps, sub.grp_begin + base, count, th, job.entangler, lane,
+                     job.gtab ? job.gtab + (size_t)b * job.gtab_ngrp + sub.grp_begin + base : nullptr);
         __syncthreads();
         for (int i = 0; i < count; ++i) {
-            const Gm& g = gm[i];
+            Gm g = gm[i];
+            if (!(kSmallOff & 1)) {
+                g.type = __builtin_amdgcn_readfirstlane(g.type); g.pc = __builtin_amdgcn_readfirstlane(g.pc); g.pt = __builtin_amdgcn_readfirstlane(g.pt);
+                g.o0 = __builtin_amdgcn_readfirstlane(g.o0); g.o1 = __builtin_amdgcn_readfirstlane(g.o1);
+            }
             cplx x[4];
             int idx[4];
 #pragma unroll
@@ -772,13 +795,15 @@
 #else
 #define RG_STAMP(slot) do { } while (0)
 #endif
-template <int WAVES>
-__global__ __launch_bounds__(64 * WAVES) void rgrad_kernel(const DevSub3* subs, const DevGrp* grps, int ent, const double* thetas, int T,
+template <int WAVES, bool TABLE>
+__global__ __launch_bounds__(64 * WAVES) void rgrad_kernel(const DevSub3* subs, const DevGrp* __restrict__ grps, int ent, const double* thetas, int T,
                                                            const cplx* rpart, int ntiles, int nsubs_total, cplx* partial, int nslots,
                                                            int from, int to, int front, const int* slot_theta, cplx* grads, cplx* mirror,
                                                            const GatherJob gj, int tiles_per_lane, int chunk, int sparse_subs,
                                                            const int* lane_parts, int conj_sub, const double* umat, int nsubs_run,
-                                                           const RgradSecond second) {
+                                                           const RgradSecond second,
+                                                           const GmRec* __restrict__ gtab, int gtab_ngrp, const GmRec* __restrict__ gtab2,
+                                                           const DevGrp* __restrict__ grps2) {
     if ((int)blockIdx.x == nsubs_run + second.count) {
         const cplx* src = static_cast<const cplx*>(gj.buf) + (size_t)blockIdx.y * gj.lane_stride;
         for (int i = threadIdx.x; i < gj.count; i += 64 * WAVES) {
@@ -789,15 +814,16 @@
         return;
     }
     __shared__ cplx R[16 * 17];
-    __shared__ Gm gm[kGrpChunk];
+    __shared__ Gm gm[TABLE ? 1 : kGrpChunk];
     __shared__ cplx rho_s[kGrpChunk][16];
     __shared__ cplx psum[WAVES > 1 ? WAVES - 1 : 1][WAVES > 1 ? 256 : 1];
     const int lane = threadIdx.x & 63, wave = threadIdx.x >> 6, b = blockIdx.y;
     int si = blockIdx.x;
     if (si >= nsubs_run) {
         si -= nsubs_run;
-        subs = second.subs; grps = second.grps; rpart = second.rpart; ntiles = second.nparts; nsubs_total = second.nsubs_total;
+        subs = second.subs; grps = grps2; rpart = second.rpart; ntiles = second.nparts; nsubs_total = second.nsubs_total;
         tiles_per_lane = second.nparts; chunk = 0; sparse_subs = second.nsubs_total; lane_parts = second.lane_parts; conj_sub = -1; umat = second.umat;
+        gtab = gtab2; gtab_ngrp = second.gtab_ngrp;
     }
     RG_STAMP(0);
     const DevSub3 sub = subs[si];
@@ -809,6 +835,15 @@
     {
         cplx acc[4] = {make_double2(0.0, 0.0), make_double2(0.0, 0.0), make_double2(0.0, 0.0), make_double2(0.0, 0.0)};
         constexpr int TB = 8;
+        if (ntiles <= WAVES && !(kSmallOff & 2)) {
+            cplx v[4];
+#pragma unroll
+            for (int r = 0; r < 4; ++r) v[r] = wave < ntiles ? rp[(size_t)wave * 256 + 64 * r + lane] : make_double2(0.0, 0.0);
+            if (!TABLE && WAVES > 1 && wave == 0 && ntiles > 0 && sub.ngrp > 0)
+                stage_groups(gm, grps, sub.grp_begin + max(0, sub.ngrp - kGrpChunk), min(sub.ngrp, kGrpChunk), th, ent, lane);
+#pragma unroll
+            for (int r = 0; r < 4; ++r) { acc[r].x += v[r].x; acc[r].y += v[r].y; }
+        } else
         for (int t0 = wave; t0 < ntiles; t0 += TB * WAVES) {
             cplx v[TB][4];
 #pragma unroll
@@ -816,7 +851,7 @@
 #pragma unroll
                 for (int r = 0; r < 4; ++r)
                     v[u][r] = t0 + u * WAVES < ntiles ? rp[(size_t)(t0 + u * WAVES) * 256 + 64 * r + lane] : make_double2(0.0, 0.0);
-            if (WAVES > 1 && t0 == wave && wave == 0 && sub.ngrp > 0)
+            if (!TABLE && WAVES > 1 && t0 == wave && wave == 0 && sub.ngrp > 0)
                 stage_groups(gm, grps, sub.grp_begin + max(0, sub.ngrp - kGrpChunk), min(sub.ngrp, kGrpChunk), th, ent, lane);
 #pragma unroll
             for (int u = 0; u < TB; ++u)
@@ -893,67 +928,93 @@
         }
     };
     const int lo = lane & 15, hi = lane >> 4;
+    auto peel = [&](const Gm& g, int i) {
+        {
+            const int a = lane >> 4, bb = (lane >> 2) & 3, o = lane & 3;
+            cplx v = R[grp_index(g, a, o) * 17 + grp_index(g, bb, o)];
+            v.x += dpp_mov<0xB1, 0xf>(v.x); v.y += dpp_mov<0xB1, 0xf>(v.y);
+            v.x += dpp_mov<0x4E, 0xf>(v.x); v.y += dpp_mov<0x4E, 0xf>(v.y);
+            if (o == 0) rho_s[i][a * 4 + bb] = v;
+        }
+        cplx x[4];
+        int idx[4];
+#pragma unroll
+        for (int l = 0; l < 4; ++l) { idx[l] = grp_index(g, l, hi) * 17 + lo; x[l] = R[idx[l]]; }
+        grp_apply<1>(g, ent, x);
+#pragma unroll
+        for (int l = 0; l < 4; ++l) R[idx[l]] = x[l];
+        __syncthreads();
+#pragma unroll
+        for (int l = 0; l < 4; ++l) { idx[l] = lo * 17 + grp_index(g, l, hi); x[l] = R[idx[l]]; }
+        grp_apply<2>(g, ent, x);
+#pragma unroll
+        for (int l = 0; l < 4; ++l) R[idx[l]] = x[l];
+        __syncthreads();
+    };
+    auto walk_rho = [&](const Gm& g) {
+        const bool on = g.jblock < 0 ? (front != 0) : (g.jblock >= from && g.jblock < to);
+        if (on && g.slot0 >= 0) {
+            cplx rho[16];
+#pragma unroll
+            for (int e = 0; e < 16; ++e) rho[e] = rho_s[lane][e];
+            if (g.type == 0) {
+                put(g.slot0 + 2, rho_dot<1>(rho, MOP_RZ));
+                rho_unapply<1>(rho, MOP_RZ, g.rc[0], g.rs[0]);
+                put(g.slot0 + 1, rho_dot<1>(rho, MOP_RY));
+                rho_unapply<1>(rho, MOP_RY, g.rc[1], g.rs[1]);
+                put(g.slot0 + 0, rho_dot<1>(rho, MOP_RZ));
+            } else {
+                const int ks = ent == 0 ? MOP_RX : MOP_RZ;
+                if (g.flags & 2) rho_unapply<0>(rho, MOP_RZ, kR, kR);
+                put(g.slot0 + 3, rho_dot<0>(rho, ks));
+                rho_unapply<0>(rho, ks, g.rc[3], g.rs[3]);
+                put(g.slot0 + 2, rho_dot<0>(rho, MOP_RY));
+                put(g.slot0 + 1, rho_dot<1>(rho, MOP_RZ));
+                rho_unapply<1>(rho, MOP_RZ, g.rc[1], g.rs[1]);
+                put(g.slot0 + 0, rho_dot<1>(rho, MOP_RY));
+                if (ent == 2) {
+                    rho_unapply<0>(rho, MOP_RY, g.rc[2], g.rs[2]);
+                    rho_unapply<1>(rho, MOP_RY, g.rc[0], g.rs[0]);
+                    put(g.slot0 + 4, make_double2(rho[15].y, -rho[15].x));
+                }
+            }
+        } else if (slot_theta && g.slot0 >= 0) {
+            for (int k = 0; k < 5; ++k) put(g.slot0 + k, make_double2(0.0, 0.0));
+        }
+    };
+    const GmRec* const tab = TABLE ? gtab + (size_t)b * gtab_ngrp + sub.grp_begin : nullptr;
+    const DevGrp* const dgrp = grps + sub.grp_begin;
     for (int top = sub.ngrp; top > 0; top -= kGrpChunk) {
         const int base = max(0, top - kGrpChunk), count = top - base;
         __syncthreads();
-        if (WAVES == 1 || top != sub.ngrp) stage_groups(gm, grps, sub.grp_begin + base, count, th, ent, lane);
-        __syncthreads();
+        if (!TABLE) {
+            if (WAVES == 1 || top != sub.ngrp) stage_groups(gm, grps, sub.grp_begin + base, count, th, ent, lane);
+            __syncthreads();
+        }
         RG_STAMP(2);
         for (int i = count - 1; i >= 0; --i) {
-            const Gm& g = gm[i];
-            {
-                const int a = lane >> 4, bb = (lane >> 2) & 3, o = lane & 3;
-                cplx v = R[grp_index(g, a, o) * 17 + grp_index(g, bb, o)];
-                v.x += dpp_mov<0xB1, 0xf>(v.x); v.y += dpp_mov<0xB1, 0xf>(v.y);
-                v.x += dpp_mov<0x4E, 0xf>(v.x); v.y += dpp_mov<0x4E, 0xf>(v.y);
-                if (o == 0) rho_s[i][a * 4 + bb] = v;
-            }
-            cplx x[4];
-            int idx[4];
-#pragma unroll
-            for (int l = 0; l < 4; ++l) { idx[l] = grp_index(g, l, hi) * 17 + lo; x[l] = R[idx[l]]; }
-            grp_apply<1>(g, ent, x);
-#pragma unroll
-            for (int l = 0; l < 4; ++l) R[idx[l]] = x[l];
-            __syncthreads();
-#pragma unroll
-            for (int l = 0; l < 4; ++l) { idx[l] = lo * 17 + grp_index(g, l, hi); x[l] = R[idx[l]]; }
-            grp_apply<2>(g, ent, x);
-#pragma unroll
-            for (int l = 0; l < 4; ++l) R[idx[l]] = x[l];
-            __syncthreads();
+            if (TABLE) {
+                int gi = base + i;
+                if (kSmallOff & 1) asm volatile("" : "+v"(gi));
+                Gm g;
+                gm_from_rec(g, tab[gi], dgrp[gi]);
+                peel(g, i);
+            } else {
+                peel(gm[i], i);
+            }
         }
         RG_STAMP(3);
         if (lane < count) {
-            const Gm& g = gm[lane];
-            const bool on = g.jblock < 0 ? (front != 0) : (g.jblock >= from && g.jblock < to);
-            if (on && g.slot0 >= 0) {
-                cplx rho[16];
-#pragma unroll
-                for (int e = 0; e < 16; ++e) rho[e] = rho_s[lane][e];
-                if (g.type == 0) {
-                    put(g.slot0 + 2, rho_dot<1>(rho, MOP_RZ));
-                    rho_unapply<1>(rho, MOP_RZ, g.rc[0], g.rs[0]);
-                    put(g.slot0 + 1, rho_dot<1>(rho, MOP_RY));
-                    rho_unapply<1>(rho, MOP_RY, g.rc[1], g.rs[1]);
-                    put(g.slot0 + 0, rho_dot<1>(rho, MOP_RZ));
-                } else {
-                    const int ks = ent == 0 ? MOP_RX : MOP_RZ;
-                    if (g.flags & 2) rho_unapply<0>(rho, MOP_RZ, kR, kR);
-                    put(g.slot0 + 3, rho_dot<0>(rho, ks));
-                    rho_unapply<0>(rho, ks, g.rc[3], g.rs[3]);
-                    put(g.slot0 + 2, rho_dot<0>(rho, MOP_RY));
-                    put(g.slot0 + 1, rho_dot<1>(rho, MOP_RZ));
-                    rho_unapply<1>(rho, MOP_RZ, g.rc[1], g.rs[1]);
-                    put(g.slot0 + 0, rho_dot<1>(rho, MOP_RY));
-                    if (ent == 2) {
-                        rho_unapply<0>(rho, MOP_RY, g.rc[2], g.rs[2]);
-                        rho_unapply<1>(rho, MOP_RY, g.rc[0], g.rs[0]);
-                        put(g.slot0 + 4, make_double2(rho[15].y, -rho[15].x));
-                    }
-                }
-            } else if (slot_theta && g.slot0 >= 0) {
-                for (int k = 0; k < 5; ++k) put(g.slot0 + k, make_double2(0.0, 0.0));
+            if (TABLE) {
+                const GmRec& r = tab[base + lane];
+                const DevGrp d = dgrp[base + lane];
+                Gm g;
+                g.type = d.type; g.flags = d.flags; g.slot0 = d.slot0; g.jblock = d.jblock;
+#pragma unroll
+                for (int k = 0; k < 4; ++k) { g.rc[k] = r.rc[k]; g.rs[k] = r.rs[k]; }
+                walk_rho(g);
+            } else {
+                walk_rho(gm[lane]);
             }
         }
         RG_STAMP(4);
@@ -1196,7 +1257,8 @@
 hipError_t launch_rgrad(const DevSub3* subs, const DevGrp* grps, int entangler, const double* thetas, int T, const void* rpart,
                         int ntiles, int nsubs_total, void* partial, int nslots, int from, int to, int front, int batch, hipStream_t s,
                         const int* slot_theta, void* grads, void* mirror, GatherJob gather, int nparts, int chunk, int sparse_subs,
-                        const int* lane_parts, int conj_sub, const double* umat, int nsubs_run, const RgradSecond* second_plan) {
+                        const int* lane_parts, int conj_sub, const double* umat, int nsubs_run, const RgradSecond* second_plan,
+                        const GmRec* gtab, int gtab_ngrp) {
     if (nsubs_total < 1) return hipSuccess;
     if (nsubs_run < 0 || nsubs_run > nsubs_total) nsubs_run = nsubs_total;
     RgradSecond second;
@@ -1207,14 +1269,16 @@
     const int tiles_per_lane = ntiles;
     if (nparts <= 0) nparts = ntiles;
     ntiles = nparts;
-    if (nparts >= 32 && second.count == 0)
-        rgrad_kernel<4><<<dim3(nsubs_run + extra, batch), 256, 0, s>>>(subs, grps, entangler, thetas, T, static_cast<const cplx*>(rpart), ntiles,
-                                                                  nsubs_total, static_cast<cplx*>(partial), nslots, from, to, front, slot_theta,
-                                                                  static_cast<cplx*>(grads), static_cast<cplx*>(mirror), gather, tiles_per_lane, chunk, sparse_subs, lane_parts, conj_sub, umat, nsubs_run, second);
-    else
-        rgrad_kernel<1><<<dim3(nsubs_run + extra, batch), 64, 0, s>>>(subs, grps, entangler, thetas, T, static_cast<const cplx*>(rpart), ntiles,
-                                                                 nsubs_total, static_cast<cplx*>(partial), nslots, from, to, front, slot_theta,
-                                                                 static_cast<cplx*>(grads), static_cast<cplx*>(mirror), gather, tiles_per_lane, chunk, sparse_subs, lane_parts, conj_sub, umat, nsubs_run, second);
+    const GmRec* gtab2 = second.gtab;
+    if (!gtab || (second.count > 0 && !gtab2)) gtab = gtab2 = nullptr;
+    const dim3 grid(nsubs_run + extra, batch);
+    auto launch = [&](auto kernel, int threads) {
+        kernel<<<grid, threads, 0, s>>>(subs, grps, entangler, thetas, T, static_cast<const cplx*>(rpart), ntiles, nsubs_total, static_cast<cplx*>(partial),
+                                        nslots, from, to, front, slot_theta, static_cast<cplx*>(grads), static_cast<cplx*>(mirror), gather, tiles_per_lane,
+                                        chunk, sparse_subs, lane_parts, conj_sub, umat, nsubs_run, second, gtab, gtab_ngrp, gtab2, second.grps);
+    };
+    if (nparts >= 32 && second.count == 0) { if (gtab) launch(rgrad_kernel<4, true>, 256); else launch(rgrad_kernel<4, false>, 256); }
+    else { if (gtab) launch(rgrad_kernel<1, true>, 64); else launch(rgrad_kernel<1, false>, 64); }
     return hipGetLastError();
 }
 
diff --git a/aqc_research_amd/csrc/aqc_launch.h b/aqc_research_amd/csrc/aqc_launch.h
--- a/aqc_research_amd/csrc/aqc_launch.h
+++ b/aqc_research_amd/csrc/aqc_launch.h
@@ -123,6 +123,13 @@
 hipError_t launch_project_amps(const ProjArgs& a, const long long* gather, int ngather, const long long* supp, void* small, const void* vy, const void* z,
                                hipStream_t s);
 hipError_t launch_project(const ProjArgs& a, hipStream_t s);
+struct GmRec {
+    double2 c[4], t[4];
+    double ec, es;
+    double rc[4], rs[4];
+    double pad[6];
+};
+static_assert(sizeof(GmRec) == 256, "a decoded-group record is 256 bytes");
 struct UJob {
     const DevSub3* sub;
     const DevGrp* grps;
@@ -131,6 +138,8 @@
     int inverse, entangler;
     double* umat_mirror;
     int mirror_index, mirror_nsubs;
+    GmRec* gtab;
+    int gtab_ngrp;
 };
 hipError_t launch_ubuild(const UJob* jobs, int njobs, const double* thetas, int T, int batch, hipStream_t s, double* thetas_copy = nullptr);
 struct GatherJob {
@@ -142,6 +151,8 @@
     const double2* rpart;
     const int* lane_parts;
     const double* umat;
+    const GmRec* gtab;
+    int gtab_ngrp;
     int nparts, nsubs_total, count;
 };
 hipError_t launch_rgrad(const DevSub3* subs, const DevGrp* grps, int entangler, const double* thetas, int T, const void* rpart,
@@ -152,7 +163,8 @@
                         int sparse_subs = 0, const int* lane_parts = nullptr,
                         int conj_sub = -1, const double* umat = nullptr,
                         int nsubs_run = -1,
-                        const RgradSecond* second_plan = nullptr);
+                        const RgradSecond* second_plan = nullptr,
+                        const GmRec* gtab = nullptr, int gtab_ngrp = 0);
 constexpr int kMaxTileCands = 72;
 hipError_t launch_tile_items(const DevStage& stage, const long long* supp, int per_lane, const long long* extra, int nextra, int batch,
                              TileItem* items, int* nitems, int* lane_parts, int* prev_tiles, TileItem* clear_items, int* nclear, hipStream_t s);
diff --git a/aqc_research_amd/csrc/aqc_ws.h b/aqc_research_amd/csrc/aqc_ws.h
--- a/aqc_research_amd/csrc/aqc_ws.h
+++ b/aqc_research_amd/csrc/aqc_ws.h
@@ -68,6 +68,7 @@
     DevBuf<DevSub3> d_subs3;
     DevBuf<DevGrp> d_grps;
     DevBuf<double> d_umat;
+    DevBuf<GmRec> d_gtab;
     DevBuf<double2> d_rpart;
     int u_level = kUNone;
     DevPlan& operator=(const HostPlan& host) { HostPlan::operator=(host); return *this; }
@@ -239,6 +240,7 @@
     bool proj_vdag_enabled = true;
     long long proj_vdag_min_elems = 1ll << 24;
     bool proj_fused_enabled = true;
+    bool gm_table = true;
     bool proj_pairs_enabled = true;
     bool proj_y0_ready = false;
     bool z_from_y = false;
diff --git a/aqc_research_amd/csrc/aqc_ws_project.cpp b/aqc_research_amd/csrc/aqc_ws_project.cpp
--- a/aqc_research_amd/csrc/aqc_ws_project.cpp
+++ b/aqc_research_amd/csrc/aqc_ws_project.cpp
@@ -101,6 +101,7 @@
     if (upload_plan(pr.vsw) || upload_plan(pr.vinv)) return 1;
     const size_t nsubs = std::max<size_t>(pr.vsw.h_subs3.size(), 1);
     if (pr.vsw.d_umat.alloc(B * nsubs * 12 * 64) || pr.vinv.d_umat.alloc(B * nsubs * 12 * 64)) return 1;
+    if (ws->gm_table && pr.vsw.d_gtab.alloc(B * std::max<size_t>(pr.vsw.h_grps.size(), 1))) return 1;
     if (pr.vsw.d_rpart.alloc(B * nsubs * (2 * (size_t)pr.ntiles_v) * 256)) return 1;
     const size_t velems = B * (2ull << pr.nvp), vbytes = sizeof(double2) * velems;
     pr.vy_copies = pr.us > 8 && pr.us <= 10 && pr.cb <= 4 ? 1 << (pr.us - 8) : 1;
@@ -225,6 +226,7 @@
     RgradSecond r;
     memset(&r, 0, sizeof r);
     r.subs = v.d_subs3; r.grps = v.d_grps; r.rpart = v.d_rpart; r.lane_parts = pr.d_lane_parts; r.umat = v.d_umat;
+    r.gtab = v.d_gtab; r.gtab_ngrp = (int)v.h_grps.size();
     r.nparts = 2 * pr.ntiles_v;
     r.nsubs_total = r.count = (int)v.h_subs3.size();
     return r;
diff --git a/aqc_research_amd/csrc/aqc_ws_sweep.cpp b/aqc_research_amd/csrc/aqc_ws_sweep.cpp
--- a/aqc_research_amd/csrc/aqc_ws_sweep.cpp
+++ b/aqc_research_amd/csrc/aqc_ws_sweep.cpp
@@ -516,6 +516,8 @@
     }
     if (projected && !pair_virtual && run_projected_stages(ws)) return 1;
     sweep_state_after(ws, sparse);
+    if (p.d_gtab && p.u_level < (projected ? route_level(ws) : kUAll))
+        return fail("gradient walk over gate groups the U builder has not decoded for the thetas in use");
     ProfScope ps(ws, AQC_K_FINALIZE);
     RgradSecond vwalk;
     if (projected) vwalk = projected_rgrad_plan(ws);
@@ -526,7 +528,7 @@
                                          : GatherJob{nullptr, 0, nullptr, 0, nullptr, nullptr},
                         nparts, chunk,
                         sparse ? p.h_stages[0].nsubs : 0, sparse ? ws->d_sw_lane_parts : nullptr, r_only_sub, p.d_umat,
-                        projected ? p.h_stages[0].nsubs : -1, projected ? &vwalk : nullptr));
+                        projected ? p.h_stages[0].nsubs : -1, projected ? &vwalk : nullptr, p.d_gtab, (int)p.h_grps.size()));
 #ifdef AQC_TUNING
     if (env_int("AQC_STAMPS", 0) != 0) { HIP_OK(hipStreamSynchronize(ws->stream)); rgrad_print_stamps(nsubs); }
 #endif
```

Measured after the change: 1.185 million evals/s. About the same (-0.4%).
